# YichengDWu/NeuralGraphPDE.jl

Hardware: AMD Instinct MI355X
Metric: ODE-steps/sec (fwd+bwd) on 16k-node graph, 64-d feats (higher is better)
Workload: dtype f32; 1 GPU; C2: 16384-node / 131072-edge closest-pairs radius graph, 64-d feats, RHS = 2 x GCNConv(64=>64, relu, self-loops), Tsit5 fixed dt=1/50 x 50 steps, forward + discrete adjoint of sum(u(T)); rhs_evals_per_ode_step=6, parallelism=dp1 (independent trajectories, all-reduce of 8320-float grads)

## Files before the change

### include/ngpde.h

```cpp
#ifndef NGPDE_H
#define NGPDE_H

#include <stddef.h>
#include <stdint.h>

#ifdef __cplusplus
extern "C" {
#endif

#define NGPDE_VERSION_STRING "0.1.0"

typedef struct ngpde_graph ngpde_graph_t;
typedef struct ngpde_node ngpde_node_t;
typedef struct ngpde_node_gat ngpde_node_gat_t;
typedef struct ngpde_node_vmh ngpde_node_vmh_t;
typedef void *ngpde_stream_t;

typedef enum {
  NGPDE_OK = 0,
  NGPDE_ERR_INVALID_ARGUMENT = -1,
  NGPDE_ERR_DIMENSION_MISMATCH = -2,
  NGPDE_ERR_HIP = -3,
  NGPDE_ERR_UNSUPPORTED = -4,
  NGPDE_ERR_WORKSPACE = -5,
// ... 274 lines not shown

int32_t ngpde_gat_layer_supported(const ngpde_graph_t *g, int32_t din, int32_t heads, int32_t c);
size_t ngpde_gat_layer_workspace_bytes(const ngpde_graph_t *g, int32_t heads, int32_t c);
int32_t ngpde_gat_layer_forward(const ngpde_graph_t *g, int32_t din, int32_t heads, int32_t c, float negative_slope, int32_t act,
                                const float *x, const float *weight, const float *a, const float *bias, float *y,
                                float *save_alpha, float *save_z, ngpde_stream_t stream);
int32_t ngpde_gat_layer_backward(const ngpde_graph_t *g, int32_t din, int32_t heads, int32_t c, float negative_slope, int32_t act,
                                 const float *x, const float *weight, const float *a, const float *y_or_z, const float *save_alpha,
                                 const float *dy, float *dx, float *dweight, float *da, float *dbias, void *workspace,
                                 size_t workspace_bytes, ngpde_stream_t stream);

int32_t ngpde_bias_act_forward(int64_t n, int32_t d, int32_t act, const float *a, const float *addend, const float *bias, float *y,
                               float *save_z, ngpde_stream_t stream);
size_t ngpde_bias_act_workspace_bytes(int32_t d);
int32_t ngpde_bias_act_backward(int64_t n, int32_t d, int32_t act, const float *dy, const float *z, float *dz, float *dbias,
                                void *workspace, size_t workspace_bytes, ngpde_stream_t stream);

int32_t ngpde_edge_mlp_supported(const ngpde_graph_t *g, int32_t h1, int32_t n_tail, const int32_t *tail_dout);
int32_t ngpde_edge_mlp_forward(const ngpde_graph_t *g, int32_t h1, int32_t act1, const float *p_target,
                               const float *q_source, const float *e_term, int32_t n_tail, const int32_t *tail_dout,
                               const int32_t *tail_act, const float *const *tail_weight, const float *const *tail_bias,
                               int32_t aggr, float *out, float *const *save_z, ngpde_stream_t stream);
int32_t ngpde_edge_mlp_backward_supported(const ngpde_graph_t *g, int32_t h1, int32_t n_tail, const int32_t *tail_dout, int32_t aggr);
int32_t ngpde_edge_mlp_backward_needs_edge_buffer(const ngpde_graph_t *g, int32_t h1, int32_t act1, int32_t has_e_term, int32_t n_tail,
                                                   const int32_t *tail_dout, const int32_t *tail_act, int32_t aggr);
size_t ngpde_edge_mlp_backward_workspace_bytes(const ngpde_graph_t *g, int32_t h1, int32_t n_tail, const int32_t *tail_dout);
int32_t ngpde_edge_mlp_backward(const ngpde_graph_t *g, int32_t h1, int32_t act1, const float *p_target, const float *q_source,
                                const float *e_term, int32_t n_tail, const int32_t *tail_dout, const int32_t *tail_act,
                                const float *const *tail_weight, const float *const *tail_bias, int32_t aggr, const float *dout,
                                float *dp_target, float *dq_source, float *de_term, float *const *dtail_weight,
                                float *const *dtail_bias, void *workspace, size_t workspace_bytes, ngpde_stream_t stream);
int32_t ngpde_activation_forward(int64_t count, int32_t act, const float *z, float *a, ngpde_stream_t stream);

int32_t ngpde_spectral_weights(int64_t n_edges, int32_t n, const float *e, float *w, ngpde_stream_t stream);

int32_t ngpde_node_gcn2_create(const ngpde_graph_t *g, int32_t d, int32_t act, int32_t tableau,
                               int32_t n_steps, float dt, int32_t with_backward, ngpde_node_t **out);
int32_t ngpde_node_gcn2_create_batch(const ngpde_graph_t *member, int32_t members, int32_t d, int32_t act, int32_t tableau,
                                     int32_t n_steps, float dt, int32_t with_backward, ngpde_node_t **out);
int32_t ngpde_node_destroy(ngpde_node_t *plan);
size_t ngpde_node_tape_bytes(const ngpde_node_t *plan);
int32_t ngpde_node_gcn2_forward(ngpde_node_t *plan, const float *u0, const float *w1, const float *b1,
                                const float *w2, const float *b2, float *uT, ngpde_stream_t stream);
int32_t ngpde_node_gcn2_backward(ngpde_node_t *plan, const float *duT, float *du0, float *dw1,
                                 float *db1, float *dw2, float *db2, ngpde_stream_t stream);
int32_t ngpde_node_generation(const ngpde_node_t *plan, uint64_t *generation, int32_t *backward_pending);
int32_t ngpde_node_expect_generation(const ngpde_node_t *plan, uint64_t generation);
int32_t ngpde_node_launch_count(const ngpde_node_t *plan, int32_t *forward, int32_t *backward);
enum { NGPDE_NODE_PRESCALED = 1, NGPDE_NODE_SIGN_MASKS = 2,  NGPDE_NODE_PERSISTENT_FWD = 8,
       NGPDE_NODE_PERSISTENT_BWD = 16, NGPDE_NODE_TILE_PAIRS = 32 ,
       NGPDE_NODE_TILE_ROUNDS = 64 ,
       NGPDE_NODE_WIDENED = 128 ,
       NGPDE_NODE_HUB_GEOMETRY = 256 ,
       NGPDE_NODE_OWN_FIRST = 512  };
int32_t ngpde_node_flags(const ngpde_node_t *plan, int32_t *flags);
int32_t ngpde_batch_pad_host(int32_t n_members, const int64_t *sizes, int64_t *padded_offsets, int64_t *index, const int32_t *order,
                             int32_t *order_padded);
int32_t ngpde_hub_partition_host(int64_t n_nodes, const int32_t *rowptr_by_target, const int32_t *col_by_target,
                                 const int32_t *rowptr_by_source, const int32_t *col_by_source, int32_t *order, int32_t *tile_rows);
int32_t ngpde_node_fault(ngpde_node_t *plan, ngpde_stream_t stream, int32_t *fault);
int32_t ngpde_node_pipeline_stats(ngpde_node_t *plan, ngpde_stream_t stream, int64_t *ahead_forward, int64_t *ahead_backward,
                                  int64_t *slot_phases);
int32_t ngpde_node_gat_supported(const ngpde_graph_t *g, int32_t din, int32_t heads, int32_t c);
int32_t ngpde_node_gat_create(const ngpde_graph_t *g, int32_t heads, int32_t c, float negative_slope, int32_t act, int32_t tableau,
                              int32_t n_steps, double dt, int32_t with_backward, ngpde_node_gat_t **out);
int32_t ngpde_node_gat_create_batch(const ngpde_graph_t *g, int32_t members, int32_t heads, int32_t c, float negative_slope,
                                    int32_t act, int32_t tableau, int32_t n_steps, double dt, int32_t with_backward,
                                    ngpde_node_gat_t **out);
int32_t ngpde_node_gat_destroy(ngpde_node_gat_t *plan);
size_t ngpde_node_gat_tape_bytes(const ngpde_node_gat_t *plan);
int32_t ngpde_node_gat_fault(ngpde_node_gat_t *plan, ngpde_stream_t stream, int32_t *fault);
int32_t ngpde_node_gat_forward(ngpde_node_gat_t *plan, const float *u0, const float *weight, const float *a, const float *bias,
                               float *uT, ngpde_stream_t stream);
int32_t ngpde_node_gat_backward(ngpde_node_gat_t *plan, const float *weight, const float *a, const float *duT, float *du0,
                                float *dweight, float *da, float *dbias, ngpde_stream_t stream);
int32_t ngpde_node_vmh_supported(const ngpde_graph_t *g, int32_t hd, int32_t pd, int32_t n_phi, const int32_t *phi_dims, const int32_t *phi_acts,
                                 int32_t n_gamma, const int32_t *gamma_dims, const int32_t *gamma_acts, int32_t aggr);
int32_t ngpde_node_vmh_create(const ngpde_graph_t *g, int32_t hd, int32_t pd, const float *pos, int32_t n_phi, const int32_t *phi_dims,
                              const int32_t *phi_acts, int32_t n_gamma, const int32_t *gamma_dims, const int32_t *gamma_acts, int32_t aggr,
                              int32_t tableau, int32_t n_steps, double dt, int32_t with_backward, ngpde_node_vmh_t **out);
int32_t ngpde_node_vmh_destroy(ngpde_node_vmh_t *plan);
size_t ngpde_node_vmh_tape_bytes(const ngpde_node_vmh_t *plan);
size_t ngpde_release_cached_memory(void);
int32_t ngpde_node_vmh_fault(ngpde_node_vmh_t *plan, ngpde_stream_t stream, int32_t *fault);
int32_t ngpde_node_vmh_forward(ngpde_node_vmh_t *plan, const float *u0, const float *const *phi_weight, const float *const *phi_bias,
                               const float *const *gamma_weight, const float *const *gamma_bias, float *uT, ngpde_stream_t stream);
int32_t ngpde_node_vmh_backward(ngpde_node_vmh_t *plan, const float *const *phi_weight, const float *const *gamma_weight, const float *duT,
                                float *du0, float *const *dphi_weight, float *const *dphi_bias, float *const *dgamma_weight,
                                float *const *dgamma_bias, ngpde_stream_t stream);
int32_t ngpde_node_vmh_forward_saveat(ngpde_node_vmh_t *plan, const float *u0, const float *const *phi_weight, const float *const *phi_bias,
                                      const float *const *gamma_weight, const float *const *gamma_bias, int32_t save_every,
                                      int32_t save_start, float *usave, ngpde_stream_t stream);
int32_t ngpde_node_vmh_backward_saveat(ngpde_node_vmh_t *plan, const float *const *phi_weight, const float *const *gamma_weight,
                                       int32_t save_every, int32_t save_start, const float *dusave, float *du0, float *const *dphi_weight,
                                       float *const *dphi_bias, float *const *dgamma_weight, float *const *dgamma_bias,
                                       ngpde_stream_t stream);

int32_t ngpde_node_profile(ngpde_node_t *plan, int32_t stride, float *out_us, int32_t *out_count,
                           ngpde_stream_t stream);

int32_t ngpde_rk_stage_combine(int64_t count, float c_self, const float *base, int32_t n_terms, const float *const *terms,
                               const float *coefs, float *out, ngpde_stream_t stream);

int32_t ngpde_accumulate_many(int32_t n_arrays, float *const *acc, const float *const *g, const int64_t *counts, ngpde_stream_t stream);

size_t ngpde_rk_error_norm_workspace_bytes(int64_t count);
int32_t ngpde_rk_error_norm(int64_t count, int32_t n_terms, const float *const *terms, const float *coefs, const float *u_prev,
                            const float *u_new, double abstol, double reltol, void *workspace, double *out ,
                            ngpde_stream_t stream);

typedef enum { NGPDE_RK_REJECT = 0, NGPDE_RK_ACCEPT = 1, NGPDE_RK_DONE = 2 } ngpde_rk_action_t;
typedef struct ngpde_rk_control {
  double t0, t, t_end;
  double dt;
  double dtmax, dtmin;
// ... 144 lines not shown
```

### neuralgraphpde.jl_amd/_lib.py

```python
from __future__ import annotations

import ctypes as C
import os

_HERE = os.path.dirname(os.path.abspath(__file__))
LIB_PATH = os.path.join(_HERE, "libngpde_hip.so")


class NgpdeError(RuntimeError):

    def __init__(self, code, msg):
        super().__init__(f"[ngpde status {code}] {msg}")
        self.code = code
        self.msg = msg


class DimensionMismatch(NgpdeError, ValueError):
    """Mirrors Julia's DimensionMismatch (status NGPDE_ERR_DIMENSION_MISMATCH)."""


class ArgumentError(NgpdeError, ValueError):
    """Mirrors Julia's ArgumentError / AssertionError (status NGPDE_ERR_INVALID_ARGUMENT)."""


# ... 184 lines not shown
    "ngpde_rk_control_init": (_i32, [C.POINTER(RkControl), C.c_double, C.c_double, C.c_double, C.c_double, C.c_double, _i64]),
    "ngpde_rk_control_trial_dt": (_i32, [C.POINTER(RkControl), C.c_double, C.c_double, C.POINTER(C.c_double)]),
    "ngpde_rk_control_initial_dt": (_i32, [C.POINTER(RkControl), C.c_double, C.c_double, C.c_double]),
    "ngpde_rk_control_step": (_i32, [C.POINTER(RkControl), C.c_double, C.POINTER(_i32)]),
    "ngpde_rk_tsit5_interp_coefs": (_i32, [C.c_double, C.c_double, C.POINTER(C.c_double)]),
    "ngpde_rk_dense_output": (_i32, [_i64, _vp, _i32, _vp, _i32, _vp, _vp, _vp]),
    "ngpde_rk_dense_output_pullback": (_i32, [_i64, _i32, _vp, _i32, _vp, _vp, _vp, _vp]),
    "ngpde_gno_message_supported": (_i32, [_i32, _i32]),
    "ngpde_gno_message_backward_from_nodes": (_i32, [_vp, _i32, _i32, _i32, _i32, _vp, _vp, _vp, _vp, _vp, _vp, _vp, _vp]),
    "ngpde_gno_message_forward": (_i32, [_vp, _i32, _i32, _i32, _vp, _vp, _vp, _vp, _vp, _vp, _vp, _vp]),
    "ngpde_ode_create": (_i32, [_vp, C.POINTER(OdeDesc), C.POINTER(_vp), C.POINTER(_i32)]),
    "ngpde_ode_destroy": (_i32, [_vp]),
    "ngpde_ode_tape_bytes": (_sz, [_vp]),
    "ngpde_ode_fault": (_i32, [_vp, _vp, C.POINTER(_i32)]),
    "ngpde_ode_forward": (_i32, [_vp, _vp, C.POINTER(OdeParams), _i32, _i32, _vp, _vp]),
    "ngpde_ode_backward": (_i32, [_vp, C.POINTER(OdeParams), _i32, _i32, _vp, _vp, C.POINTER(OdeGrads), _vp]),
    "ngpde_gno_gform_supported": (_i32, [_i32, _i32]),
    "ngpde_gno_gform_preferred": (_i32, [_i64, _i64, _i32, _i32, _i32, _i32]),
    "ngpde_gno_gform_splits": (_i32, [_i64, _i32, _i32, _i32]),
    "ngpde_gno_gform_aggregate": (_i32, [_vp, _i32, _i32, _i32, _i32, _vp, _vp, _vp, _vp, _vp, _vp, _vp, _vp]),
    "ngpde_gno_gform_transform": (_i32, [_i64, _i32, _i32, _i32, _i32, _vp, _vp, _vp, _vp, _vp, _vp, _vp, _vp, _vp, _vp, _i32, _vp]),
    "ngpde_gat_layer_supported": (_i32, [_vp, _i32, _i32, _i32]),
    "ngpde_gat_layer_workspace_bytes": (_sz, [_vp, _i32, _i32]),
    "ngpde_gat_layer_forward": (_i32, [_vp, _i32, _i32, _i32, _f32, _i32, _vp, _vp, _vp, _vp, _vp, _vp, _vp, _vp]),
    "ngpde_gat_layer_backward": (_i32, [_vp, _i32, _i32, _i32, _f32, _i32, _vp, _vp, _vp, _vp, _vp, _vp, _vp, _vp, _vp, _vp, _vp, _sz, _vp]),
    "ngpde_bias_act_forward": (_i32, [_i64, _i32, _i32, _vp, _vp, _vp, _vp, _vp, _vp]),
    "ngpde_bias_act_workspace_bytes": (_sz, [_i32]),
    "ngpde_bias_act_backward": (_i32, [_i64, _i32, _i32, _vp, _vp, _vp, _vp, _vp, _sz, _vp]),
    "ngpde_edge_mlp_supported": (_i32, [_vp, _i32, _i32, _vp]),
    "ngpde_edge_mlp_forward": (_i32, [_vp, _i32, _i32, _vp, _vp, _vp, _i32, _vp, _vp, _vp, _vp, _i32, _vp, _vp, _vp]),
    "ngpde_edge_mlp_backward_supported": (_i32, [_vp, _i32, _i32, _vp, _i32]),
    "ngpde_edge_mlp_backward_needs_edge_buffer": (_i32, [_vp, _i32, _i32, _i32, _i32, _vp, _vp, _i32]),
    "ngpde_edge_mlp_backward_workspace_bytes": (_sz, [_vp, _i32, _i32, _vp]),
    "ngpde_edge_mlp_backward": (_i32, [_vp, _i32, _i32, _vp, _vp, _vp, _i32, _vp, _vp, _vp, _vp, _i32, _vp, _vp, _vp, _vp, _vp, _vp,
                                        _vp, _sz, _vp]),
    "ngpde_activation_forward": (_i32, [_i64, _i32, _vp, _vp, _vp]),
    "ngpde_spectral_weights": (_i32, [_i64, _i32, _vp, _vp, _vp]),
    "ngpde_node_gcn2_create": (_i32, [_vp, _i32, _i32, _i32, _i32, _f32, _i32, C.POINTER(_vp)]),
    "ngpde_node_gcn2_create_batch": (_i32, [_vp, _i32, _i32, _i32, _i32, _i32, _f32, _i32, C.POINTER(_vp)]),
    "ngpde_node_destroy": (_i32, [_vp]),
    "ngpde_node_tape_bytes": (_sz, [_vp]),
    "ngpde_node_gcn2_forward": (_i32, [_vp, _vp, _vp, _vp, _vp, _vp, _vp, _vp]),
    "ngpde_node_gcn2_backward": (_i32, [_vp, _vp, _vp, _vp, _vp, _vp, _vp, _vp]),
    "ngpde_node_launch_count": (_i32, [_vp, C.POINTER(_i32), C.POINTER(_i32)]),
    "ngpde_node_flags": (_i32, [_vp, C.POINTER(_i32)]),
    "ngpde_hub_partition_host": (_i32, [_i64, _vp, _vp, _vp, _vp, _vp, _vp]),
    "ngpde_batch_pad_host": (_i32, [_i32, _vp, _vp, _vp, _vp, _vp]),
    "ngpde_node_fault": (_i32, [_vp, _vp, C.POINTER(_i32)]),
    "ngpde_row_blocks_gather": (_i32, [_i32, _i32, _vp, _i32, _vp, _vp, _vp, _vp, _vp, _i32, _vp, _vp, _vp]),
    "ngpde_row_blocks_scatter": (_i32, [_i32, _i32, _vp, _i32, _vp, _vp, _vp, _vp, _vp, _i32, _vp, _vp, _vp]),
    "ngpde_transpose": (_i32, [_i32, _i32, _vp, _vp, _vp]),
    "ngpde_rows_scale": (_i32, [_i64, _i32, _vp, _vp, _vp, _vp]),
    "ngpde_node_pipeline_stats": (_i32, [_vp, _vp, C.POINTER(_i64), C.POINTER(_i64), C.POINTER(_i64)]),
    "ngpde_node_generation": (_i32, [_vp, C.POINTER(C.c_uint64), C.POINTER(_i32)]),
    "ngpde_node_expect_generation": (_i32, [_vp, C.c_uint64]),
    "ngpde_node_profile": (_i32, [_vp, _i32, C.POINTER(_f32), C.POINTER(_i32), _vp]),
    "ngpde_node_gat_supported": (_i32, [_vp, _i32, _i32, _i32]),
    "ngpde_node_gat_create": (_i32, [_vp, _i32, _i32, _f32, _i32, _i32, _i32, C.c_double, _i32, C.POINTER(_vp)]),
    "ngpde_node_gat_create_batch": (_i32, [_vp, _i32, _i32, _i32, _f32, _i32, _i32, _i32, C.c_double, _i32, C.POINTER(_vp)]),
    "ngpde_node_gat_destroy": (_i32, [_vp]),
    "ngpde_node_gat_tape_bytes": (_sz, [_vp]),
    "ngpde_node_gat_fault": (_i32, [_vp, _vp, C.POINTER(_i32)]),
    "ngpde_node_gat_forward": (_i32, [_vp, _vp, _vp, _vp, _vp, _vp, _vp]),
    "ngpde_node_gat_backward": (_i32, [_vp, _vp, _vp, _vp, _vp, _vp, _vp, _vp, _vp]),
}

_lib = None


def load():
    global _lib
    if _lib is not None:
        return _lib
    if not os.path.exists(LIB_PATH):
        raise ImportError(
            f"{LIB_PATH} is missing: build it with `python -c 'import __graft_entry__ as g; g.build()'` "
            "or `make -C neuralgraphpde.jl_amd/csrc`.  There is no CPU fallback for the hot path.")
    import torch
    lib = C.CDLL(LIB_PATH, mode=C.RTLD_GLOBAL)
    for name, (res, args) in SIGNATURES.items():
        try:
            fn = getattr(lib, name)
        except AttributeError as e:
            raise ImportError(f"{LIB_PATH} does not export {name}; rebuild the library") from e
        fn.restype = res
        fn.argtypes = args
    _lib = lib
    return lib


def check(status):
    if status == OK:
        return
    msg = load().ngpde_last_error().decode("utf-8", "replace")
    if status == ERR_DIMENSION_MISMATCH:
        raise DimensionMismatch(status, msg)
    if status == ERR_INVALID_ARGUMENT:
        raise ArgumentError(status, msg)
    raise NgpdeError(status, msg)


def ptr(t):
    if t is None:
        return None
    if hasattr(t, "data_ptr"):
        return t.data_ptr()
# ... 42 lines not shown
```

### neuralgraphpde.jl_amd/csrc/common.h

```cpp
#pragma once

#include <hip/hip_runtime.h>

#include <cstdarg>
#include <cstdint>
#include <cstdio>
#include <mutex>
#include <string>
#include <vector>

#include "../../include/ngpde.h"

namespace ngpde {

std::string &last_error();
int32_t fail(int32_t code, const char *fmt, ...);

#define NGPDE_LAUNCH_CHECK(name)                                                                    \
  do {                                                                                              \
    hipError_t _le = hipGetLastError();                                                             \
    if (_le != hipSuccess)                                                                          \
      return ::ngpde::fail(NGPDE_ERR_HIP, "%s launch failed: %s", name, hipGetErrorString(_le));    \
  } while (0)

// ... 85 lines not shown
  const float *wt = nullptr;
  const float *bias = nullptr;
  float *y = nullptr;
  float *save_agg = nullptr;
  float *save_z = nullptr;
  uint8_t *save_mask = nullptr;
  bool pre = false;
  const OwnFirst *of = nullptr;
  bool has_comb = false;
  Comb comb;
  float *comb_out = nullptr;
  hipEvent_t ev_start = nullptr, ev_stop = nullptr;
};
bool fused_supported(int din, int dout);
bool fused_prescaled_supported(const ngpde_graph *g, int d);
int32_t launch_fused_fwd(const FusedFwdArgs &a, hipStream_t stream);

struct FusedBwdArgs {
  const ngpde_graph *g = nullptr;
  int d = 0, act = 0;
  bool aggregate = false;
  const float *g_in = nullptr;
  bool has_comb = false;
  Comb comb;
  float *store_t = nullptr;
  float *store_v = nullptr;
  float v_scale = 1.f;
  bool do_dense = true;
  const float *z = nullptr;
  const uint8_t *mask = nullptr;
  bool pre = false;
  const float *saved_agg = nullptr;
  const float *wt = nullptr;
  float *g_out = nullptr;
  float *slab_dw = nullptr;
  float *slab_db = nullptr;
  hipEvent_t ev_start = nullptr, ev_stop = nullptr;
};
int fused_tile_rows();
int fused_num_blocks(int64_t n_nodes);
size_t fused_mask_bytes(int64_t n_nodes, int d);
int fused_num_slabs(int64_t n_nodes, int d);
int32_t launch_fused_bwd(const FusedBwdArgs &a, hipStream_t stream);
int32_t launch_reduce_slabs(const float *slab, int n_slabs, int len, int ct, float *out, hipStream_t stream);
int32_t launch_zero(void *ptr, size_t bytes, hipStream_t stream);
struct OwnFirst {
  uint8_t *slots = nullptr;
  int4 *sched = nullptr;
  float *slot_w = nullptr;
  uint8_t *pre = nullptr;
};
int32_t own_first_tables_build(const ngpde_graph *g, OwnFirst *of, hipStream_t stream);
void own_first_tables_free(OwnFirst *of);

struct NodePersist {
  int n_tiles = 0;
  int pair_wgs = 0;
  int *nbr = nullptr;
  unsigned *sync = nullptr;
  size_t sync_bytes = 0;
  unsigned *fault = nullptr;
  volatile unsigned *fault_host = nullptr;
  int *stats = nullptr;
  float *coef = nullptr;
  bool hub = false;
  struct HubLists {
    int32_t *halo = nullptr;
    uint8_t *slots = nullptr;
    int2 *rows = nullptr;
    int4 *info = nullptr;
    uint8_t *longs = nullptr;
    float *w = nullptr;
    int4 *sched = nullptr;
  } hub_lists[2];
};
struct NodePersistFwd {
  const ngpde_graph *g = nullptr;
  const NodePersist *ps = nullptr;
  int n_steps = 0, S = 0, act = 0, n_members = 1;
  const float *u_in = nullptr;
  float *u_out = nullptr, *bufA = nullptr, *bufB = nullptr;
  const float *w1 = nullptr, *b1 = nullptr, *w2 = nullptr, *b2 = nullptr;
  float *tape = nullptr;
  uint8_t *masks = nullptr;
  float *ztape = nullptr;
  size_t row_elems = 0, mask_bytes = 0;
  bool interleave = false;
  bool pair = false;
  int k_tiles = 0;
  float *state = nullptr;
  hipEvent_t ev_start = nullptr, ev_stop = nullptr;
  bool no_latch = false;
  const OwnFirst *of = nullptr;
};
struct NodePersistBwd {
  const ngpde_graph *g = nullptr;
  const NodePersist *ps = nullptr;
  int n_steps = 0, S = 0, n_members = 1, act = NGPDE_ACT_RELU;
  float *lam = nullptr, *g1 = nullptr, *g2 = nullptr;
  const float *w1 = nullptr, *w2 = nullptr, *tape = nullptr, *ztape = nullptr;
  const uint8_t *masks = nullptr;
  size_t row_elems = 0, mask_bytes = 0;
  float *slab_dw1 = nullptr, *slab_db1 = nullptr, *slab_dw2 = nullptr, *slab_db2 = nullptr;
  bool interleave = false;
  bool pair = false;
  int k_tiles = 0;
  float *ubar = nullptr;
  hipEvent_t ev_start = nullptr, ev_stop = nullptr;
  bool no_latch = false;
};
const unsigned *node_persistent_abort_word(const NodePersist *ps);
bool node_persistent_interleave_env();
bool node_persistent_disabled_env();
bool node_persistent_supported(const ngpde_graph *g, int d, int act, bool with_bwd);
int node_persistent_mode(const ngpde_graph *g, int d, int act, bool with_bwd);
bool node_persistent_hub_possible(const ngpde_graph *g, int d);
int node_persistent_rounds(const ngpde_graph *g);
int32_t node_persistent_setup(const ngpde_graph *g, const float *coef_host , NodePersist *ps, bool pair = false, bool hub = false);
bool node_wait_lists_fit(const ngpde_graph *g);
void node_persistent_free(NodePersist *ps);
int32_t launch_node_fwd_persistent(const NodePersistFwd &a, hipStream_t stream);
int32_t launch_node_bwd_persistent(const NodePersistBwd &a, hipStream_t stream);
struct PersistentTurn {
  int dev = -1;
  bool held = false;
  hipStream_t stream = nullptr;
  const NodePersist *ps = nullptr;
  int32_t enter(const NodePersist &p, hipStream_t s);
  int32_t latch();
  int32_t leave();
  ~PersistentTurn();
  PersistentTurn() = default;
  PersistentTurn(const PersistentTurn &) = delete;
  PersistentTurn &operator=(const PersistentTurn &) = delete;
};
struct GatNodeFwd {
  const ngpde_graph *g = nullptr;
  const NodePersist *ps = nullptr;
  int heads = 0, act = 0, n_steps = 0, S = 0;
  float slope = 0.2f;
  bool taped = false;
  const float *u_in = nullptr, *wt = nullptr, *a = nullptr, *bias = nullptr;
  float *u_out = nullptr, *xs = nullptr, *yz = nullptr, *alpha = nullptr, *kbuf = nullptr;
  const float *cf = nullptr;
  int n_members = 1;
  size_t xs_stride = 0, yz_stride = 0, alpha_stride = 0;
  hipEvent_t ev_start = nullptr, ev_stop = nullptr;
};
struct GatNodeBwd {
  const ngpde_graph *g = nullptr;
  const NodePersist *ps = nullptr;
  int heads = 0, act = 0, n_steps = 0, S = 0;
  float slope = 0.2f;
  const float *wt = nullptr, *a = nullptr, *xs = nullptr, *yz = nullptr, *alpha = nullptr, *duT = nullptr;
  float *lam = nullptr, *ubar = nullptr, *dzbuf = nullptr, *dscore = nullptr, *dal = nullptr;
  float *slab_db = nullptr, *slab_dw = nullptr, *slab_u = nullptr;
  const int *xpad = nullptr;
  const float *cb = nullptr;
  float *dwt = nullptr, *da = nullptr, *db = nullptr;
  int n_members = 1;
  size_t xs_stride = 0, yz_stride = 0, alpha_stride = 0;
  hipEvent_t ev_start = nullptr, ev_stop = nullptr;
// ... 214 lines not shown
```

### neuralgraphpde.jl_amd/csrc/node.hip

```cpp
#include <cstdlib>
#include <new>
#include <vector>

#include "common.h"

using namespace ngpde;

namespace {

struct Tableau {
  int S;
  std::vector<std::vector<double>> a;
  std::vector<double> b;
};

Tableau make_tableau(int which) {
  Tableau t;
  if (which == NGPDE_TABLEAU_EULER) {
    t.S = 1;
    t.a = {{}};
    t.b = {1.0};
    return t;
  }
  t.S = 6;
// ... 125 lines not shown
    }
  }
}

int32_t copy_block(float *dst, int dpitch, const float *src, int spitch, int w, int h, hipStream_t stream) {
  NGPDE_HIP_CHECK(hipMemcpy2DAsync(dst, (size_t)dpitch * sizeof(float), src, (size_t)spitch * sizeof(float), (size_t)w * sizeof(float),
                                   (size_t)h, hipMemcpyDeviceToDevice, stream));
  return NGPDE_OK;
}

bool act_needs_z(int act) {
  return !(act == NGPDE_ACT_IDENTITY || act == NGPDE_ACT_RELU || act == NGPDE_ACT_LEAKYRELU);
}

}

struct ngpde_node {
  const ngpde_graph *g = nullptr;
  int d = 0, act = 0, n_steps = 0;
  int du = 0;
  float dt = 0.f;
  bool with_bwd = false, needs_z = false;
  Tableau tb;
  int64_t n = 0;
  size_t row_elems = 0;
  int members = 1;
  size_t all_elems = 0;
  int nb = 0;
  int slots = 0;

  float *u = nullptr, *ustage = nullptr, *u0keep = nullptr;
  float *w1 = nullptr, *b1 = nullptr, *w2 = nullptr, *b2 = nullptr;
  float *tape = nullptr;
  size_t tape_bytes = 0;
  bool mask_mode = false;
  bool pre = false;
  float *ybuf = nullptr;
  uint8_t *masks = nullptr;
  size_t mask_bytes = 0;
  float *lam = nullptr, *g1 = nullptr, *g2 = nullptr;
  std::vector<float *> ubar;
  float *slabs = nullptr;
  size_t slab_bytes = 0;
  float *slab_dw1 = nullptr, *slab_db1 = nullptr, *slab_dw2 = nullptr, *slab_db2 = nullptr;
  float *dw1 = nullptr, *db1 = nullptr, *dw2 = nullptr, *db2 = nullptr;

  bool persistent = false;
  bool hub = false;
  bool ztape_mode = false;
  float *ztape = nullptr;
  NodePersist persist;
  OwnFirst of;
  bool has_of = false;
  float *pbuf = nullptr;
  bool interleave = false;
  bool pair = false;
  int ktiles = 0;
  float *kstate = nullptr;
  float *pubar = nullptr;

  hipStream_t cap_stream = nullptr;
  hipGraph_t fwd_graph = nullptr, bwd_graph = nullptr;
  hipGraphExec_t fwd_exec = nullptr, bwd_exec = nullptr;
  bool forward_done = false;
  uint64_t generation = 0;
  bool backward_pending = false;
  int fwd_launches = 0, bwd_launches = 0;

  float *slot(int step, int stage, int k) const {
    const int s = with_bwd ? step : 0;
    if (mask_mode) {
      if (k == 1 || k == 3) return ybuf + ((size_t)stage * 2 + (k == 3 ? 1 : 0)) * row_elems;
      return tape + ((size_t)(s * tb.S + stage) * 2 + (k == 2 ? 1 : 0)) * row_elems;
    }
    return tape + ((size_t)(s * tb.S + stage) * slots + k) * row_elems;
  }
  uint8_t *mask_slot(int step, int stage, int layer) const {
    return masks + ((size_t)(step * tb.S + stage) * 2 + (layer - 1)) * mask_bytes;
  }
};

namespace {

struct Prof {
  int stride = 1, counter = 0;
  std::vector<hipEvent_t> ev0, ev1;
  std::vector<int> role;
  bool want(int r, hipEvent_t *a, hipEvent_t *b) {
    if ((counter++ % stride) != 0) return false;
    hipEvent_t e0 = nullptr, e1 = nullptr;
    if (hipEventCreate(&e0) != hipSuccess || hipEventCreate(&e1) != hipSuccess) return false;
    ev0.push_back(e0); ev1.push_back(e1); role.push_back(r);
    *a = e0; *b = e1;
    return true;
  }
  ~Prof() {
    for (hipEvent_t e : ev0) (void)hipEventDestroy(e);
    for (hipEvent_t e : ev1) (void)hipEventDestroy(e);
  }
};

int32_t dev_alloc(float **p, size_t elems) {
  *p = nullptr;
  NGPDE_HIP_CHECK(hipMalloc((void **)p, std::max<size_t>(elems, 1) * sizeof(float)));
  return NGPDE_OK;
}
// ... 97 lines not shown
        for (int j = i + 1; j < S; ++j) {
          if (tb.a[j][i - 1] == 0.0) continue;
          e.comb.ptr[e.comb.n] = p->ubar[j];
          e.comb.coef[e.comb.n++] = (float)(p->dt * tb.a[j][i - 1]);
        }
        e.comb.coef_self = (float)(p->dt * tb.a[i][i - 1]);
        fill_dense(p, e, 2, n, i - 1);
      } else {
        e.comb.ptr[e.comb.n] = p->lam;
        e.comb.coef[e.comb.n++] = 1.0f;
        for (int j = 1; j < S; ++j) {
          e.comb.ptr[e.comb.n] = p->ubar[j];
          e.comb.coef[e.comb.n++] = 1.0f;
        }
        e.comb.coef_self = 1.0f;
        e.store_v = p->lam;
        if (n > 0) {
          e.v_scale = (float)(p->dt * tb.b[S - 1]);
          fill_dense(p, e, 2, n - 1, S - 1);
        } else {
          e.do_dense = false;
          e.pre = p->pre;
        }
      }
      if (prof && e.do_dense) prof->want(3, &e.ev_start, &e.ev_stop);
      if ((st = launch_fused_bwd(e, stream))) return st;
      count += 2;
    }
  }
  const int dd = p->d * p->d;
  const int ns = fused_num_slabs(p->n, p->d);
  if ((st = launch_reduce_slabs(p->slab_dw1, ns, dd, p->d / 16, p->dw1, stream))) return st;
  if ((st = launch_reduce_slabs(p->slab_db1, ns, p->d, 0, p->db1, stream))) return st;
  if ((st = launch_reduce_slabs(p->slab_dw2, ns, dd, p->d / 16, p->dw2, stream))) return st;
  if ((st = launch_reduce_slabs(p->slab_db2, ns, p->d, 0, p->db2, stream))) return st;
  count += 4;
  if (launches) *launches = count;
  return NGPDE_OK;
}

int32_t enqueue_forward_persistent(ngpde_node *p, hipStream_t stream, hipEvent_t ev0 = nullptr, hipEvent_t ev1 = nullptr, bool fold_latch = false) {
  NodePersistFwd a;
  a.no_latch = fold_latch;
  a.g = p->g; a.ps = &p->persist; a.n_steps = p->n_steps; a.S = p->tb.S; a.act = p->act; a.n_members = p->members;
  a.u_in = p->u; a.u_out = p->u;
  a.bufA = p->ustage; a.bufB = p->pbuf;
  a.w1 = p->w1; a.b1 = p->b1; a.w2 = p->w2; a.b2 = p->b2;
  a.row_elems = p->row_elems;
  if (p->with_bwd) {
    a.tape = p->tape; a.masks = p->masks; a.mask_bytes = p->mask_bytes; a.ztape = p->ztape;
  }
  a.interleave = p->interleave; a.pair = p->pair; a.k_tiles = p->ktiles; a.state = p->kstate;
  a.of = p->has_of ? &p->of : nullptr;
  a.ev_start = ev0; a.ev_stop = ev1;
  return launch_node_fwd_persistent(a, stream);
}

int32_t enqueue_backward_persistent(ngpde_node *p, hipStream_t stream, hipEvent_t ev0 = nullptr, hipEvent_t ev1 = nullptr,
                                    float *const *out = nullptr) {
  NodePersistBwd a;
  a.no_latch = true;
  a.g = p->g; a.ps = &p->persist; a.n_steps = p->n_steps; a.S = p->tb.S; a.n_members = p->members; a.act = p->act;
  a.lam = p->lam; a.g1 = p->g1; a.g2 = p->g2; a.w1 = p->w1; a.w2 = p->w2;
  a.tape = p->tape; a.masks = p->masks; a.row_elems = p->row_elems; a.mask_bytes = p->mask_bytes; a.ztape = p->ztape;
  a.slab_dw1 = p->slab_dw1; a.slab_db1 = p->slab_db1; a.slab_dw2 = p->slab_dw2; a.slab_db2 = p->slab_db2;
  a.interleave = p->interleave; a.pair = p->pair; a.ubar = p->pubar; a.k_tiles = p->ktiles;
  a.ev_start = ev0; a.ev_stop = ev1;
  int32_t st;
  if ((st = launch_node_bwd_persistent(a, stream))) return st;
  const int dd = p->d * p->d;
  Reduce4 r;
  r.n_slabs = (p->pair || p->ktiles) ? p->persist.pair_wgs : p->persist.n_tiles;
  r.slab[0] = p->slab_dw1; r.slab[1] = p->slab_db1; r.slab[2] = p->slab_dw2; r.slab[3] = p->slab_db2;
  r.len[0] = r.len[2] = dd; r.len[1] = r.len[3] = p->d;
  r.ct[0] = r.ct[2] = p->d / 16; r.ct[1] = r.ct[3] = 0;
  if (out) {
    for (int j = 0; j < 4; ++j) r.out[j] = out[j];
    r.du = p->du;
  } else {
    r.out[0] = p->dw1; r.out[1] = p->db1; r.out[2] = p->dw2; r.out[3] = p->db2;
    r.du = p->d;
  }
  r.abort_word = node_persistent_abort_word(&p->persist); r.fault = p->persist.fault;
  hipLaunchKernelGGL(reduce4_slabs_kernel, dim3((dd + 63) / 64, 4), dim3(1024), 0, stream, r);
  NGPDE_LAUNCH_CHECK("reduce4_slabs_kernel");
  return NGPDE_OK;
}

int32_t capture(ngpde_node *p, bool backward) {
  hipGraph_t graph = nullptr;
  NGPDE_HIP_CHECK(hipStreamBeginCapture(p->cap_stream, hipStreamCaptureModeRelaxed));
  int count = 0;
  int32_t st = backward ? enqueue_backward(p, p->cap_stream, &count) : enqueue_forward(p, p->cap_stream, &count);
  hipError_t e = hipStreamEndCapture(p->cap_stream, &graph);
  if (st) {
    if (graph) (void)hipGraphDestroy(graph);
    return st;
  }
  if (e != hipSuccess) {
    if (graph) (void)hipGraphDestroy(graph);
    return fail(NGPDE_ERR_HIP, "hipStreamEndCapture failed: %s", hipGetErrorString(e));
  }
  hipGraphExec_t exec = nullptr;
  e = hipGraphInstantiate(&exec, graph, nullptr, nullptr, 0);
  if (e != hipSuccess) {
    (void)hipGraphDestroy(graph);
    return fail(NGPDE_ERR_HIP, "hipGraphInstantiate failed: %s", hipGetErrorString(e));
  }
  if (backward) {
    p->bwd_graph = graph; p->bwd_exec = exec; p->bwd_launches = count;
  } else {
    p->fwd_graph = graph; p->fwd_exec = exec; p->fwd_launches = count;
  }
  return NGPDE_OK;
}

}

extern "C" {

int32_t ngpde_node_destroy(ngpde_node_t *p) {
  NGPDE_RANGE();
  if (!p) return NGPDE_OK;
  if (p->fwd_exec) (void)hipGraphExecDestroy(p->fwd_exec);
  if (p->bwd_exec) (void)hipGraphExecDestroy(p->bwd_exec);
  if (p->fwd_graph) (void)hipGraphDestroy(p->fwd_graph);
  if (p->bwd_graph) (void)hipGraphDestroy(p->bwd_graph);
  if (p->cap_stream) (void)hipStreamDestroy(p->cap_stream);
  float *bufs[] = {p->u0keep, p->u, p->ustage, p->w1, p->b1, p->w2, p->b2, p->tape, p->lam, p->g1, p->g2, p->slabs,
                   p->dw1, p->db1, p->dw2, p->db2};
  for (float *b : bufs)
    if (b) (void)hipFree(b);
  for (float *b : p->ubar)
    if (b) (void)hipFree(b);
  if (p->ybuf) (void)hipFree(p->ybuf);
  if (p->masks) (void)hipFree(p->masks);
  if (p->pbuf) (void)hipFree(p->pbuf);
  if (p->pubar) (void)hipFree(p->pubar);
  if (p->kstate) (void)hipFree(p->kstate);
  node_persistent_free(&p->persist);
  own_first_tables_free(&p->of);
  delete p;
  return NGPDE_OK;
}

int32_t ngpde_node_gcn2_create(const ngpde_graph_t *g, int32_t d, int32_t act, int32_t tableau, int32_t n_steps,
                               float dt, int32_t with_backward, ngpde_node_t **out) {
  NGPDE_RANGE();
  return ngpde_node_gcn2_create_batch(g, 1, d, act, tableau, n_steps, dt, with_backward, out);
}

static int32_t node_create(const ngpde_graph_t *g, int32_t members, int32_t d, int32_t du, int32_t act, int32_t tableau,
                           int32_t n_steps, float dt, int32_t with_backward, ngpde_node_t **out) {
  NGPDE_REQUIRE(out != nullptr, NGPDE_ERR_INVALID_ARGUMENT, "ngpde_node_gcn2_create: out is NULL");
  NGPDE_REQUIRE(members >= 1, NGPDE_ERR_INVALID_ARGUMENT, "ngpde_node_gcn2_create_batch: members must be >= 1");
  *out = nullptr;
  NGPDE_REQUIRE(g != nullptr, NGPDE_ERR_INVALID_ARGUMENT, "ngpde_node_gcn2_create: graph is NULL");
  NGPDE_REQUIRE(g->has_norm, NGPDE_ERR_STATE, "ngpde_node_gcn2_create: GCN normalisation not set");
  NGPDE_REQUIRE(fused_supported(d, d), NGPDE_ERR_UNSUPPORTED,
                "ngpde_node_gcn2_create: d must be one of 16, 32, 64, 128 (got %d)", d);
  NGPDE_REQUIRE(act >= NGPDE_ACT_IDENTITY && act <= NGPDE_ACT_SOFTPLUS, NGPDE_ERR_INVALID_ARGUMENT,
                "ngpde_node_gcn2_create: unknown activation code %d", act);
  NGPDE_REQUIRE(tableau == NGPDE_TABLEAU_EULER || tableau == NGPDE_TABLEAU_TSIT5, NGPDE_ERR_INVALID_ARGUMENT,
                "ngpde_node_gcn2_create: unknown tableau %d", tableau);
  NGPDE_REQUIRE(n_steps >= 1, NGPDE_ERR_INVALID_ARGUMENT, "ngpde_node_gcn2_create: n_steps must be >= 1");
  NGPDE_REQUIRE(g->n_nodes >= 1, NGPDE_ERR_INVALID_ARGUMENT, "ngpde_node_gcn2_create: empty graph");
  ngpde_node *p = new (std::nothrow) ngpde_node();
  NGPDE_REQUIRE(p != nullptr, NGPDE_ERR_INVALID_ARGUMENT, "out of host memory");
  p->g = g; p->d = d; p->du = du; p->act = act; p->n_steps = n_steps; p->dt = dt;
  p->with_bwd = with_backward != 0;
  p->needs_z = p->with_bwd && act_needs_z(act);
  p->tb = make_tableau(tableau);
  p->n = g->n_nodes;
  p->members = members;
  p->row_elems = (size_t)p->n * d;
  p->all_elems = (size_t)members * p->row_elems;
  p->nb = fused_num_blocks(p->n);
  p->mask_mode = p->with_bwd && act == NGPDE_ACT_RELU && std::getenv("NGPDE_NO_MASK") == nullptr;
  p->pre = fused_prescaled_supported(g, d) && std::getenv("NGPDE_NO_PRESCALE") == nullptr;
  int pmode = p->pre ? node_persistent_mode(g, d, act, p->with_bwd) : 0;
  bool hub = !p->pre && pmode == 0 && std::getenv("NGPDE_NO_PRESCALE") == nullptr && node_persistent_hub_possible(g, d) &&
             (!p->with_bwd || p->mask_mode || act != NGPDE_ACT_RELU);
  if (hub) {
    pmode = 4;
    p->pre = true;
  }
  p->pair = pmode == 2 && members == 1 && (!p->with_bwd || p->mask_mode);
  p->ktiles = (pmode == 3 && members == 1) ? node_persistent_rounds(g) : 0;
  bool want_persist = (pmode == 1 && (!p->with_bwd || p->mask_mode || (act != NGPDE_ACT_RELU && members == 1))) || p->pair || p->ktiles > 0 || hub;
  const int S = p->tb.S;
  int32_t st = NGPDE_OK;
  if (want_persist) {
    p->persistent = true;
    float coef[90] = {0};
    const Tableau &tb = p->tb;
    for (int i = 0; i < S; ++i) {
      const std::vector<double> &row = (i == S - 1) ? tb.b : tb.a[i + 1];
      for (int j = 0; j < i; ++j) coef[i * 6 + j] = (float)(dt * row[j]);
      coef[36 + i] = (float)(dt * row[i]);
      coef[42 + i] = (float)(dt * tb.b[i]);
    }
    for (int i = 1; i < S; ++i) {
      for (int j = i + 1; j < S; ++j) coef[48 + i * 6 + j] = (float)(dt * tb.a[j][i - 1]);
      coef[84 + i] = (float)(dt * tb.a[i][i - 1]);
    }
    st = node_persistent_setup(g, coef, &p->persist, p->pair, hub);
    if (st == NGPDE_ERR_UNSUPPORTED) {
      st = NGPDE_OK;
      p->persistent = false;
    }
    if (p->persistent && p->ktiles > 0) p->persist.pair_wgs = (p->persist.n_tiles + p->ktiles - 1) / p->ktiles;
  }
  if (!p->persistent) {
    p->pair = false;
    p->ktiles = 0;
  }
  if (hub && !p->persistent) {
    p->pre = false;
    hub = false;
    node_persistent_free(&p->persist);
  }
  p->hub = hub;
  int dev_ = 0, cus_ = 0;
  const bool one_wave = hipGetDevice(&dev_) == hipSuccess && hipDeviceGetAttribute(&cus_, hipDeviceAttributeMultiprocessorCount, dev_) == hipSuccess &&
                        p->nb <= 2 * cus_;
  if (st == NGPDE_OK && p->pre && !hub && one_wave) {
    const char *nof = std::getenv("NGPDE_NO_OWN_FIRST");
    if (!(nof && nof[0] == '1')) {
      st = own_first_tables_build(g, &p->of, nullptr);
      p->has_of = st == NGPDE_OK;
    }
  }
  p->ztape_mode = p->with_bwd && !p->mask_mode && p->persistent;
  p->slots = p->mask_mode ? 2 : (p->ztape_mode ? 4 : (p->with_bwd ? (p->needs_z ? 6 : 4) : 4));
  p->mask_bytes = p->mask_mode ? fused_mask_bytes(p->n, d) : 0;
  p->interleave = members > 1 && !hub && node_persistent_interleave_env();
  const size_t xslots = p->interleave ? 2 : 1;
  auto A = [&](float **ptr, size_t elems) {
    if (st == NGPDE_OK) st = dev_alloc(ptr, elems);
  };
  A(&p->u, p->all_elems);
  A(&p->ustage, xslots * p->row_elems);
  A(&p->u0keep, (size_t)members * p->n * du);
  A(&p->w1, (size_t)d * d); A(&p->b1, d); A(&p->w2, (size_t)d * d); A(&p->b2, d);
  if (st == NGPDE_OK && du != d) {
    for (float *w : {p->w1, p->w2})
      if (hipMemset(w, 0, (size_t)d * d * sizeof(float)) != hipSuccess) st = fail(NGPDE_ERR_HIP, "hipMemset failed");
    for (float *b : {p->b1, p->b2})
      if (hipMemset(b, 0, (size_t)d * sizeof(float)) != hipSuccess) st = fail(NGPDE_ERR_HIP, "hipMemset failed");
  }
  const size_t tape_elems = (size_t)(p->with_bwd ? n_steps : 1) * S * p->slots * p->all_elems;
  p->tape_bytes = tape_elems * sizeof(float);
  A(&p->tape, tape_elems);
  if (p->mask_mode) {
    A(&p->ybuf, (size_t)S * 2 * p->row_elems);
    if (st == NGPDE_OK) {
      const size_t mb = (size_t)members * n_steps * S * 2 * p->mask_bytes;
      if (hipMalloc((void **)&p->masks, std::max<size_t>(mb, 1)) != hipSuccess) st = fail(NGPDE_ERR_HIP, "hipMalloc of the sign-bit masks failed");
      else p->tape_bytes += mb + (size_t)S * 2 * p->row_elems * sizeof(float);
    }
  }
  if (p->with_bwd) {
    A(&p->lam, p->all_elems); A(&p->g1, xslots * p->row_elems); A(&p->g2, xslots * p->row_elems);
    if (p->interleave || p->pair || p->ktiles) A(&p->pubar, 2 * 5 * p->row_elems);
    p->ubar.assign(S, nullptr);
    for (int j = 1; j < S; ++j) A(&p->ubar[j], p->row_elems);
    const size_t dd = (size_t)d * d;
    const size_t per = (size_t)p->nb * (dd + d);
    p->slab_bytes = 2 * per * sizeof(float);
    A(&p->slabs, 2 * per);
    if (st == NGPDE_OK) {
      p->slab_dw1 = p->slabs;
      p->slab_db1 = p->slab_dw1 + (size_t)p->nb * dd;
      p->slab_dw2 = p->slab_db1 + (size_t)p->nb * d;
      p->slab_db2 = p->slab_dw2 + (size_t)p->nb * dd;
    }
    A(&p->dw1, dd); A(&p->db1, d); A(&p->dw2, dd); A(&p->db2, d);
  }
  if (st == NGPDE_OK && p->persistent) A(&p->pbuf, xslots * p->row_elems);
  if (st == NGPDE_OK && p->ktiles) A(&p->kstate, 7 * p->row_elems);
  if (st == NGPDE_OK && p->ztape_mode) p->ztape = p->tape + (size_t)n_steps * S * 2 * p->all_elems;
  if (st == NGPDE_OK && members > 1 && !p->persistent)
    st = fail(NGPDE_ERR_UNSUPPORTED, "ngpde_node_gcn2_create_batch: the member-by-member solve exists for the persistent plan only "
                                     "(d = 64, relu, unweighted, at most two 32-row tiles per CU); batch the graphs into one handle instead");
  if (st == NGPDE_OK && !p->persistent) {
    hipError_t e = hipStreamCreateWithFlags(&p->cap_stream, hipStreamNonBlocking);
    if (e != hipSuccess) st = fail(NGPDE_ERR_HIP, "hipStreamCreate failed: %s", hipGetErrorString(e));
    if (st == NGPDE_OK) st = capture(p, false);
    if (st == NGPDE_OK && p->with_bwd) st = capture(p, true);
  }
  if (p->persistent) {
    p->fwd_launches = 2;
    p->bwd_launches = p->with_bwd ? 3 : 0;
  }
  if (st != NGPDE_OK) {
    std::string keep = last_error();
    ngpde_node_destroy(p);
    last_error() = keep;
    return st;
  }
  *out = p;
  return NGPDE_OK;
}

int32_t ngpde_node_gcn2_create_batch(const ngpde_graph_t *g, int32_t members, int32_t d, int32_t act, int32_t tableau,
                                     int32_t n_steps, float dt, int32_t with_backward, ngpde_node_t **out) {
  NGPDE_RANGE();
  const char *nw = std::getenv("NGPDE_NO_WIDEN");
  if (out && g && (d == 16 || d == 32) && !(nw && nw[0] == '1') && g->has_norm && g->n_nodes >= 1 &&
      (node_persistent_mode(g, 64, act, with_backward != 0) != 0 || node_persistent_hub_possible(g, 64))) {
    ngpde_node_t *w = nullptr;
    if (node_create(g, members, 64, d, act, tableau, n_steps, dt, with_backward, &w) == NGPDE_OK) {
      if (w->persistent) {
        *out = w;
        return NGPDE_OK;
      }
      ngpde_node_destroy(w);
    }
  }
  return node_create(g, members, d, d, act, tableau, n_steps, dt, with_backward, out);
}

size_t ngpde_node_tape_bytes(const ngpde_node_t *p) { return p ? p->tape_bytes : 0; }

int32_t ngpde_node_launch_count(const ngpde_node_t *p, int32_t *forward, int32_t *backward) {
  NGPDE_RANGE();
  NGPDE_REQUIRE(p != nullptr, NGPDE_ERR_INVALID_ARGUMENT, "ngpde_node_launch_count: plan is NULL");
  if (forward) *forward = p->fwd_launches;
  if (backward) *backward = p->bwd_launches;
  return NGPDE_OK;
}

int32_t ngpde_node_flags(const ngpde_node_t *p, int32_t *flags) {
  NGPDE_RANGE();
  NGPDE_REQUIRE(p != nullptr && flags != nullptr, NGPDE_ERR_INVALID_ARGUMENT, "ngpde_node_flags: NULL argument");
  *flags = (p->pre ? NGPDE_NODE_PRESCALED : 0) | (p->mask_mode ? NGPDE_NODE_SIGN_MASKS : 0) |
           (p->persistent ? NGPDE_NODE_PERSISTENT_FWD : 0) | (p->persistent && p->with_bwd ? NGPDE_NODE_PERSISTENT_BWD : 0) |
           (p->pair ? NGPDE_NODE_TILE_PAIRS : 0) | (p->ktiles ? NGPDE_NODE_TILE_ROUNDS : 0) | (p->du != p->d ? NGPDE_NODE_WIDENED : 0) |
           (p->hub ? NGPDE_NODE_HUB_GEOMETRY : 0) | (p->has_of ? NGPDE_NODE_OWN_FIRST : 0);
  return NGPDE_OK;
}

int32_t ngpde_node_fault(ngpde_node_t *p, ngpde_stream_t stream_, int32_t *fault) {
  NGPDE_RANGE();
  NGPDE_REQUIRE(p != nullptr && fault != nullptr, NGPDE_ERR_INVALID_ARGUMENT, "ngpde_node_fault: NULL argument");
  *fault = 0;
  if (!p->persist.fault_host) return NGPDE_OK;
  NGPDE_HIP_CHECK(hipStreamSynchronize((hipStream_t)stream_));
  *fault = *p->persist.fault_host ? 1 : 0;
  return NGPDE_OK;
}

int32_t ngpde_node_pipeline_stats(ngpde_node_t *p, ngpde_stream_t stream_, int64_t *ahead_forward, int64_t *ahead_backward,
                                  int64_t *slot_phases) {
  NGPDE_RANGE();
  NGPDE_REQUIRE(p != nullptr, NGPDE_ERR_INVALID_ARGUMENT, "ngpde_node_pipeline_stats: plan is NULL");
  if (ahead_forward) *ahead_forward = 0;
  if (ahead_backward) *ahead_backward = 0;
  if (slot_phases) *slot_phases = 0;
  if (!p->persist.stats) return NGPDE_OK;
  const int nt = p->persist.n_tiles;
  std::vector<int> h((size_t)nt * 2);
  NGPDE_HIP_CHECK(hipMemcpyAsync(h.data(), p->persist.stats, h.size() * sizeof(int), hipMemcpyDeviceToHost, (hipStream_t)stream_));
  NGPDE_HIP_CHECK(hipStreamSynchronize((hipStream_t)stream_));
  int64_t f = 0, b = 0;
  for (int t = 0; t < nt; ++t) f += h[2 * t], b += h[2 * t + 1];
  if (ahead_forward) *ahead_forward = f;
  if (ahead_backward) *ahead_backward = b;
  if (slot_phases) *slot_phases = (int64_t)nt * p->members * p->n_steps * p->tb.S * 2;
  return NGPDE_OK;
}

int32_t ngpde_node_gcn2_forward(ngpde_node_t *p, const float *u0, const float *w1, const float *b1, const float *w2,
                                const float *b2, float *uT, ngpde_stream_t stream_) {
  NGPDE_RANGE();
  NGPDE_REQUIRE(p != nullptr, NGPDE_ERR_INVALID_ARGUMENT, "ngpde_node_gcn2_forward: plan is NULL");
  NGPDE_REQUIRE(u0 && w1 && w2 && uT, NGPDE_ERR_INVALID_ARGUMENT, "ngpde_node_gcn2_forward: NULL argument");
  NGPDE_REQUIRE(!(p->persist.fault_host && *p->persist.fault_host), NGPDE_ERR_STATE,
                "ngpde_node_gcn2_forward: an earlier persistent launch of this plan gave up waiting for its neighbours (its outputs are NaN): "
                "another kernel held the device's compute units, or two persistent solves of different processes shared the device; "
                "create a new plan (NGPDE_NO_PERSISTENT=1 selects the replayed plan)");
  hipStream_t stream = (hipStream_t)stream_;
  const size_t user_bytes = (size_t)p->members * p->n * p->du * sizeof(float);
  if (p->pre) {
    RowsExtra x;
    x.keep = reinterpret_cast<float4 *>(p->u0keep);
    int32_t st = launch_scale_rows_width(u0, p->du, p->g->c, p->u, p->d, p->n, false, stream, p->members, x);
    if (st) return st;
  } else {
    NGPDE_HIP_CHECK(hipMemcpyAsync(p->u, u0, p->all_elems * sizeof(float), hipMemcpyDeviceToDevice, stream));
    NGPDE_HIP_CHECK(hipMemcpyAsync(p->u0keep, u0, user_bytes, hipMemcpyDeviceToDevice, stream));
  }
  {
    int32_t st = launch_pack_params(w1, b1, w2, b2, p->du, p->d, p->w1, p->b1, p->w2, p->b2, stream);
    if (st) return st;
  }
  const bool fold_latch = p->persistent && p->pre;
  if (p->persistent) {
    int32_t st = enqueue_forward_persistent(p, stream, nullptr, nullptr, fold_latch);
    if (st) return st;
  } else {
    NGPDE_HIP_CHECK(hipGraphLaunch(p->fwd_exec, stream));
  }
  if (p->pre) {
    RowsExtra x;
    if (fold_latch) { x.abort_word = node_persistent_abort_word(&p->persist); x.fault = p->persist.fault; }
    int32_t st = launch_scale_rows_width(p->u, p->d, p->g->c, uT, p->du, p->n, true, stream, p->members, x);
    if (st) return st;
  } else {
    NGPDE_HIP_CHECK(hipMemcpyAsync(uT, p->u, p->all_elems * sizeof(float), hipMemcpyDeviceToDevice, stream));
  }
  p->forward_done = true;
  ++p->generation;
  p->backward_pending = p->with_bwd;
  return NGPDE_OK;
}

int32_t ngpde_node_generation(const ngpde_node_t *p, uint64_t *generation, int32_t *backward_pending) {
  NGPDE_RANGE();
  NGPDE_REQUIRE(p != nullptr, NGPDE_ERR_INVALID_ARGUMENT, "ngpde_node_generation: plan is NULL");
  if (generation) *generation = p->generation;
  if (backward_pending) *backward_pending = p->backward_pending ? 1 : 0;
// ... 611 lines not shown
```

### neuralgraphpde.jl_amd/csrc/node_persistent.hip

```cpp

#include <algorithm>
#include <cstdlib>
#include <cstring>
#include <mutex>
#include <type_traits>

#include "common.h"
#include "persistent_gcn_tile.h"
#include "stamps.h"

namespace ngpde {

namespace {


template <int ACT, bool TAPE, bool WGT = false, bool HUB = false>
__global__ __launch_bounds__(kThreads, HUB ? 2 : 4) void node_fwd_persistent_kernel(const PFwdK p) {
  static_assert(!(HUB && WGT), "hub geometry: its own weight lists (HubCtx::hw), not the WGT form");
  constexpr int XH = HUB ? kHubXhF : kXhF, MF = HUB ? kHubMetaF : kMetaF;
  __shared__ __attribute__((aligned(16))) float lds[XH + 2 * kTileF + (WGT ? kWF + kSlotWF : 2 * kWF) + 2 * PD + MF + 48 + 4];
  static_assert(!HUB || sizeof(lds) <= 160 * 1024 - 64, "one workgroup per CU");
  float *ldsXh = lds, *ldsT = lds + XH, *ldsZ = ldsT + kTileF, *ldsW1 = ldsZ + kTileF, *ldsW2 = WGT ? ldsW1 : ldsW1 + kWF;
  float *ldsSW = ldsW2 + kWF, *ldsB = WGT ? ldsSW + kSlotWF : ldsSW;
  float *ldsMeta = ldsB + 2 * PD, *ldsC = ldsMeta + MF;
  int *s_ok = reinterpret_cast<int *>(ldsC + 48);
  typename std::conditional<HUB, HubCtx, TileCtx>::type c;
  if constexpr (HUB) hub_ctx_init(p.m, c, ldsMeta);
  else tile_ctx_init(p.m, c, ldsMeta);
  coef_to_lds(ldsC, p.cf, 42, c.tid);
  const int act = ACT >= 0 ? ACT : p.act;
  float4 *Xh4 = reinterpret_cast<float4 *>(ldsXh);
  float bw1[16];
  if constexpr (WGT) {
    reinterpret_cast<float2 *>(ldsSW)[c.tid] = reinterpret_cast<const float2 *>(p.m.slot_w + (size_t)c.tile * kSlotWF)[c.tid];
    c.lds_w = ldsSW;
    const int i16 = c.lane & 15, kq = c.lane >> 4, ct = c.wave_u / PG::RT;
#pragma unroll
    for (int kb = 0; kb < 4; ++kb)
#pragma unroll
      for (int r = 0; r < 4; ++r) bw1[4 * kb + r] = p.w1[(16 * kb + 4 * kq + r) * PD + 16 * ct + i16];
  } else {
    load_weight_lds(p.w1, ldsW1, c.tid, true);
  }
  load_weight_lds(p.w2, ldsW2, c.tid, true);
  biases_to_lds(ldsB, p.b1, p.b2, c.tid);
  if (!HUB) zero_halo_row(ldsXh, c.grp == 0, c.q);
  if (c.tid == 0) *s_ok = 1;
  const unsigned own = own_row_offset(c);
  __syncthreads();
  int of_pre = 0;
  if constexpr (!HUB && !WGT) {
    if (p.m.of_pre) of_pre = __builtin_amdgcn_readfirstlane((int)p.m.of_pre[(size_t)c.tile * 8 + c.wave_u]);
  }
  const float4 bias1 = reinterpret_cast<const float4 *>(ldsB)[c.q], bias2 = reinterpret_cast<const float4 *>(ldsB + PD)[c.q];
  bool ok = true;
  int ph = 0;
  for (int mb = 0; mb < p.n_members; ++mb) {
  const float *u_in = p.u_in + (size_t)mb * p.row_elems;
  const size_t ev0 = (size_t)mb * p.n_steps * p.S * 2;
  float4 u = f4_sel(c.valid && ok, ld4_g(u_in, own), f4_zero());
  float4 k0 = f4_zero(), k1 = f4_zero(), k2 = f4_zero(), k3 = f4_zero(), k4 = f4_zero(), k5 = f4_zero();
  Xh4[c.grp * PG::LPR + c.q] = u;
  if constexpr (!HUB && !WGT) __syncthreads();
  for (int n = 0; n < p.n_steps && ok; ++n) {
    for (int i = 0; i < p.S && ok; ++i) {
#pragma unroll
      for (int layer = 0; layer < 2; ++layer) {
        ++ph;
        const float *X = layer == 0 ? ((n == 0 && i == 0) ? u_in : p.bufA) : p.bufB;
        NGPDE_PHASE_STAMP(p.m.stamps, ph, 0);
        float4 agg;
        if constexpr (HUB) {
          unsigned sw[8];
          hub_slot_words(c, sw);
          if (!hub_wait(p.m, c, ph, s_ok)) { ok = false; break; }
          NGPDE_PHASE_STAMP(p.m.stamps, ph, 1);
          hub_gather_foreign(c, X, ldsXh);
          NGPDE_PHASE_STAMP(p.m.stamps, ph, 2);
          agg = hub_aggregate(c, sw, ldsXh, ldsZ);
        } else if constexpr (!WGT) {
          unsigned sw[8], swf[8];
          tile_slot_words(c, sw);
          tile_slot_words_from(c, of_pre, swf);
          unsigned goff[2];
          tile_gather_offsets(c, goff);
          const float4 self = Xh4[c.grp * PG::LPR + c.q];
          float4 a = tile_aggregate_rounds(c, sw, ldsXh, f4_zero(), of_pre);
          tile_wait_arrive(p.m, c, ph, s_ok, p.m.flags);
          NGPDE_PHASE_STAMP(p.m.stamps, ph, 1);
          if (!tile_gather_foreign_checked(c, X, ldsXh, goff, s_ok)) { ok = false; break; }
          NGPDE_PHASE_STAMP(p.m.stamps, ph, 2);
          a = tile_aggregate_rounds(c, swf, ldsXh, a, ((c.wmax + 3) >> 2) - of_pre);
          agg = f4_add(a, self);
        } else {
          unsigned sw[8];
          tile_slot_words(c, sw);
          if (!tile_wait(p.m, c, ph, s_ok)) { ok = false; break; }
          NGPDE_PHASE_STAMP(p.m.stamps, ph, 1);
          tile_gather_foreign(c, X, ldsXh);
          NGPDE_PHASE_STAMP(p.m.stamps, ph, 2);
          agg = tile_aggregate_weighted(c, ldsXh);
        }
        float4 acc = f4_scale(c.ci, agg);
        tile_row_store(ldsT, c, acc);
        const size_t ev = ev0 + (size_t)(n * p.S + i) * 2 + layer;
        __syncthreads();
        NGPDE_PHASE_STAMP(p.m.stamps, ph, 3);
        if (WGT && layer == 0) mfma_rows_times_bfrag64(ldsT, bw1, ldsZ, c.wave_u, c.lane);
        else mfma_rows_times_bt<PD>(ldsT, layer == 0 ? ldsW1 : ldsW2, ldsZ, c.wave_u, c.lane);
        __syncthreads();
        NGPDE_PHASE_STAMP(p.m.stamps, ph, 4);
        const float4 z = fwd_preact(ldsZ, c, layer == 0 ? bias1 : bias2);
        const uint8_t sign_bits = relu_sign_bits(z);
        float4 yv = fwd_output(c, act, z);
        if (layer == 0) {
          if (c.valid) store_sc1(p.bufB, own, yv);
          Xh4[c.grp * PG::LPR + c.q] = yv;
        } else {
          k0 = f4_sel(i == 0, yv, k0); k1 = f4_sel(i == 1, yv, k1); k2 = f4_sel(i == 2, yv, k2);
          k3 = f4_sel(i == 3, yv, k3); k4 = f4_sel(i == 4, yv, k4); k5 = f4_sel(i == 5, yv, k5);
          const float4 v = rk_combine<false>(RkCoefInPlace{ldsC, i}, i, yv, u, k0, k1, k2, k3, k4);
          if (i == p.S - 1) u = v;
          if (c.valid) store_sc1(p.bufA, own, v);
          Xh4[c.grp * PG::LPR + c.q] = v;
        }
        NGPDE_PHASE_STAMP(p.m.stamps, ph, 5);
        tile_publish(p.m, c, ph);
        NGPDE_PHASE_STAMP(p.m.stamps, ph, 6);
        if constexpr (TAPE && ACT == NGPDE_ACT_RELU) stu8_g(p.masks + ev * p.mask_bytes + (size_t)c.tile * kThreads, (unsigned)c.tid, sign_bits);
        else if (TAPE && c.valid) st4_stream_g(p.ztape + ev * p.row_elems, own, z);
        if (TAPE && c.valid) st4_stream_g(p.tape + ev * p.row_elems, own, tile_row(ldsT, c));
      }
    }
  }
  if (c.valid) st4_g(p.u_out + (size_t)mb * p.row_elems, own, f4_sel(ok, u, f4_nan()));
  }
}


template <int ACT, bool TAPE>
__global__ __launch_bounds__(kThreads, 4) void node_fwd_persistentK_kernel(const PFwdK p) {
  constexpr int kMS = meta_stride<true>(), kMT = meta_tiles<true>();
  __shared__ __attribute__((aligned(16))) float lds[kXhF + 2 * kTileF + kWF + 2 * PD + kMT * kMS + 48 + 4];
  static_assert(sizeof(lds) <= 80 * 1024 - 64, "two workgroups per CU");
  float *ldsXh = lds, *ldsT = lds + kXhF, *ldsZ = ldsT + kTileF, *ldsW = ldsZ + kTileF, *ldsB = ldsW + kWF;
  float *ldsMeta = ldsB + 2 * PD, *ldsC = ldsMeta + kMT * kMS;
  int *s_ok = reinterpret_cast<int *>(ldsC + 48);
  const int tid = threadIdx.x, q = tid & 15;
  coef_to_lds(ldsC, p.cf, 42, tid);
  const int act = ACT >= 0 ? ACT : p.act;
  biases_to_lds(ldsB, p.b1, p.b2, tid);
  zero_halo_row(ldsXh, tid < PG::LPR, tid & 15);
  if (tid == 0) *s_ok = 1;
  const int W = p.pair_wgs, K = min(p.k_tiles, kMT);
  const int t0 = xcd_tile(blockIdx.x, W);
  const unsigned rowb = (unsigned)(p.row_elems * sizeof(float));
  tile_round_tables<true>(p.m, t0, W, K, ldsMeta);
  const int KT = tile_round_count(p.m, t0, W, K);
  __syncthreads();
  const float4 bias1 = reinterpret_cast<const float4 *>(ldsB)[q], bias2 = reinterpret_cast<const float4 *>(ldsB + PD)[q];
  bool ok = true;
  int ph = 0;
  for (int n = 0; n < p.n_steps && ok; ++n) {
    for (int i = 0; i < p.S && ok; ++i) {
#pragma unroll 1
      for (int layer = 0; layer < 2 && ok; ++layer) {
        ++ph;
        const float *X = layer == 0 ? ((n == 0 && i == 0) ? p.u_in : p.bufA) : p.bufB;
        const size_t ev = (size_t)(n * p.S + i) * 2 + layer;
        const bool last_phase = (n == p.n_steps - 1 && i == p.S - 1 && layer == 1);
        load_weight_lds(layer == 0 ? p.w1 : p.w2, ldsW, tid, true);
        for (int s = 0; s < K; ++s) {
          const int tile = t0 + s * W;
          if (tile >= p.m.n_tiles) break;
          TileCtx c;
          tile_ctx_from_lds<true>(c, tile, ldsMeta + s * kMS);
          const unsigned own = own_row_offset(c);
          if (!tile_wait(p.m, c, ph, s_ok)) { ok = false; break; }
          halo_fill_all(c, X, ldsXh);
          float4 su = f4_zero(), sk0 = f4_zero(), sk1 = f4_zero(), sk2 = f4_zero(), sk3 = f4_zero(), sk4 = f4_zero();
          if (layer == 1) {
            su = (n == 0) ? f4_sel(c.valid, ld4_g(p.u_in, own), f4_zero()) : ld4_g(p.state, own);
            sk0 = i > 0 ? ld4_g(p.state, own + rowb) : f4_zero(); sk1 = i > 1 ? ld4_g(p.state, own + 2 * rowb) : f4_zero();
            sk2 = i > 2 ? ld4_g(p.state, own + 3 * rowb) : f4_zero(); sk3 = i > 3 ? ld4_g(p.state, own + 4 * rowb) : f4_zero();
// ... 285 lines not shown
  int pend_ph = 0;
  const int NP = p.n_steps * p.S * 2;
  for (int mb = 0; mb < p.n_members && ok; mb += 2) {
    const bool two = PAIR ? has1 : mb + 1 < p.n_members;
    const float *u_in0 = p.u_in + (size_t)mb * p.row_elems, *u_in1 = u_in0 + ((two && !PAIR) ? p.row_elems : 0);
    const size_t ev00 = (size_t)mb * NP, ev01 = PAIR ? ev00 : ev00 + NP;
    const size_t boff1 = PAIR ? 0 : p.row_elems;
    unsigned *flags1 = p.m.flags + (PAIR ? 0 : p.flag_stride);
    FSlot s0, s1;
    s0.u = f4_sel(c.valid, ld4_g(u_in0, own), f4_zero());
    s1.u = f4_sel(c1.valid && two, ld4_g(u_in1, own1), f4_zero());
    s0.k0 = s0.k1 = s0.k2 = s0.k3 = s0.k4 = s0.k5 = f4_zero();
    s1.k0 = s1.k1 = s1.k2 = s1.k3 = s1.k4 = s1.k5 = f4_zero();
    s0.xown = s0.u;
    s1.xown = s1.u;
    int n = 0, i = 0;
    for (int P = 0; P < NP && ok; P += 2) {
#pragma unroll
      for (int layer = 0; layer < 2; ++layer) {
        ++ph;
        const float *ldsW = layer == 0 ? ldsW1 : ldsW2, *ldsBias = layer == 0 ? ldsB : ldsB + PD;
        const float *X0 = layer == 0 ? (P == 0 ? u_in0 : p.bufA) : p.bufB;
        const float *X1 = layer == 0 ? (P == 0 ? u_in1 : p.bufA + boff1) : p.bufB + boff1;
        FNext nx0, nx1;
        nx0.exists = two; nx0.ph = ph; nx0.X = X1; nx0.flags = flags1;
        nx1.exists = P + layer + 1 < NP; nx1.ph = ph + 1; nx1.X = layer == 0 ? p.bufB : p.bufA; nx1.flags = p.m.flags;
        if (!fwd_slot_phase<ACT, TAPE, PAIR>(p, c, c1, s0, s1, 0, ph, n, i, layer, X0, ev00, act, own, pre, n_ahead, pend_flags, pend_ph, nx0, ldsXh,
                                             ldsT, ldsZ, ldsW, ldsBias, ldsC, s_ok, s_pre)) { ok = false; break; }
        if (two && !fwd_slot_phase<ACT, TAPE, PAIR>(p, c1, c, s1, s0, 1, ph, n, i, layer, X1, ev01, act, own1, pre, n_ahead, pend_flags, pend_ph, nx1,
                                                    ldsXh, ldsT, ldsZ, ldsW, ldsBias, ldsC, s_ok, s_pre)) { ok = false; break; }
      }
      if (++i == p.S) i = 0, ++n;
    }
    wait_vmcnt0();
    __syncthreads();
    if (ok && pend_flags && c.tid == 0) __hip_atomic_store(pend_flags, (unsigned)pend_ph, __ATOMIC_RELAXED, __HIP_MEMORY_SCOPE_AGENT);
    pend_flags = nullptr;
    if (c.valid) st4_g(p.u_out + (size_t)mb * p.row_elems, own, f4_sel(ok, s0.u, f4_nan()));
    if (two && c1.valid) st4_g(p.u_out + (PAIR ? 0 : (size_t)(mb + 1) * p.row_elems), own1, f4_sel(ok, s1.u, f4_nan()));
    if (PAIR) break;
  }
  if (!ok) {
    poison_members(p.u_out, p.n_members, p.row_elems, c.valid, own);
    poison_members(p.u_out, p.n_members, p.row_elems, PAIR && has1 && c1.valid, own1);
  }
  if (c.tid == 0 && p.m.stats) p.m.stats[2 * c.tile] = n_ahead;
}


template <int ACT, bool WGT = false, bool HUB = false>
__global__ __launch_bounds__(kThreads, HUB ? 2 : 4) void node_bwd_persistent_kernel(const PBwdK p) {
  static_assert(!(HUB && WGT), "hub geometry: its own weight lists (HubCtx::hw), not the WGT form");
  constexpr bool RELU = (ACT == NGPDE_ACT_RELU);
  using Aux = typename std::conditional<RELU, unsigned, float4>::type;
  constexpr int XH = HUB ? kHubXhF : kXhF, MF = HUB ? kHubMetaF : kMetaF;
  __shared__ __attribute__((aligned(16))) float lds[XH + 2 * kTileF + (WGT ? PD * PD + kWF + kSlotWF : 2 * kWF) + MF + 48 + 4];
  static_assert(sizeof(lds) <= (HUB ? 160 : 80) * 1024 - 64, "two workgroups per CU (hub geometry: one)");
  float *ldsXh = lds, *ldsG = lds, *ldsDZ = lds + XH, *ldsX = ldsDZ + kTileF, *ldsW1 = ldsX + kTileF, *ldsW2 = ldsW1 + (WGT ? PD * PD : kWF);
  float *ldsSW = ldsW2 + kWF;
  float *ldsMeta = WGT ? ldsSW + kSlotWF : ldsSW, *ldsC = ldsMeta + MF;
  int *s_ok = reinterpret_cast<int *>(ldsC + 48);
  typename std::conditional<HUB, HubCtx, TileCtx>::type c;
  if constexpr (HUB) hub_ctx_init(p.m, c, ldsMeta);
  else tile_ctx_init(p.m, c, ldsMeta);
  coef_to_lds(ldsC, p.cb, 48, c.tid);
  float4 *Xh4 = reinterpret_cast<float4 *>(ldsXh);
  if constexpr (WGT) {
    reinterpret_cast<float2 *>(ldsSW)[c.tid] = reinterpret_cast<const float2 *>(p.m.slot_w + (size_t)c.tile * kSlotWF)[c.tid];
    c.lds_w = ldsSW;
#pragma unroll
    for (int k = 0; k < PG::W4; ++k) {
      const int idx = c.tid + k * kThreads;
      if (idx < PD * PD / 4) {
        const int wi = (idx * 4) / PD, w4 = ((idx * 4) % PD) / 4;
        *reinterpret_cast<float4 *>(&ldsW1[wi * PD + 4 * (w4 ^ (wi & 15))]) = reinterpret_cast<const float4 *>(p.w1)[idx];
      }
    }
  } else {
    load_weight_lds(p.w1, ldsW1, c.tid, false);
  }
  load_weight_lds(p.w2, ldsW2, c.tid, false);
  if (!HUB) zero_halo_row(ldsXh, c.grp == 0, c.q);
  if (c.tid == 0) *s_ok = 1;
  const unsigned own = own_row_offset(c);
  f32x4 dw1[PG::DWT], dw2[PG::DWT];
#pragma unroll
  for (int mm = 0; mm < PG::DWT; ++mm) dw1[mm] = dw2[mm] = (f32x4){0.f, 0.f, 0.f, 0.f};
  float db1 = 0.f, db2 = 0.f;
  const int dbc = c.tid / PG::DBP, dbpart = c.tid % PG::DBP;
  const int S = p.S;
  __syncthreads();

  auto tape_row = [&](size_t ev) { return ld4_stream_g(p.tape + ev * p.row_elems, own); };
  auto mask_of = [&](size_t ev) -> Aux {
    if constexpr (RELU) return ldu8_g(p.masks + ev * p.mask_bytes + (size_t)c.tile * kThreads, (unsigned)c.tid);
    else return ld4_stream_g(p.ztape + ev * p.row_elems, own);
  };
  Aux mk_n{};
  float4 xrow_n = f4_zero();
  unsigned f_next = 0;
  auto dense = [&](int ph, const float *ldsW, f32x4 (&dwl)[PG::DWT], float &dbl, float4 kbar, Aux mk, float4 xrow, float *gout, bool pf, size_t ev_n) {
    const float4 dz = adjoint_dz<RELU>(c, p.act, kbar, mk);
    tile_row_store(ldsDZ, c, dz);
    __syncthreads();
    NGPDE_PHASE_STAMP(p.m.stamps, ph, 3);
    if (WGT && ldsW == ldsW1) mfma_rows_times_bswz64(ldsDZ, ldsW, ldsG, c.wave_u, c.lane);
    else mfma_rows_times_bt<PD>(ldsDZ, ldsW, ldsG, c.wave_u, c.lane);
    __syncthreads();
    NGPDE_PHASE_STAMP(p.m.stamps, ph, 4);
    const float4 gv = adjoint_g_row(ldsG, c);
    if (c.valid) store_sc1(gout, own, gv);
    adjoint_x_store(ldsX, c, xrow);
    NGPDE_PHASE_STAMP(p.m.stamps, ph, 5);
    tile_publish(p.m, c, ph);
    NGPDE_PHASE_STAMP(p.m.stamps, ph, 6);
    Xh4[c.grp * PG::LPR + c.q] = gv;
    if constexpr (!HUB) {
      if (c.wave_u == 0) f_next = poll_issue(p.m, c, p.m.flags);
    }
    if (pf) {
      mk_n = mask_of(ev_n);
      xrow_n = tape_row(ev_n);
    }
    param_grad_products(ldsX, ldsDZ, c.wave_u, c.lane, dbc, dbpart, dwl, dbl);
    NGPDE_PHASE_STAMP(p.m.stamps, ph, 7);
  };

  bool ok = true;
  int ph = 0;
  for (int mb = 0; mb < p.n_members; ++mb) {
  float *lam_g = p.lam + (size_t)mb * p.row_elems;
  const size_t ev0 = (size_t)mb * p.n_steps * S * 2;
  float4 lam = f4_sel(c.valid && ok, ld4_g(lam_g, own), f4_zero());
  float4 ub1 = f4_zero(), ub2 = f4_zero(), ub3 = f4_zero(), ub4 = f4_zero(), ub5 = f4_zero();
  if (ok) {
    ++ph;
    const size_t ev = ev0 + (size_t)((p.n_steps - 1) * S + (S - 1)) * 2 + 1;
    dense(ph, ldsW2, dw2, db2, adjoint_kbar_last(ldsC, S, lam), mask_of(ev), tape_row(ev), p.g2, true,
          ev0 + (size_t)((p.n_steps - 1) * S + (S - 1)) * 2);
  }
  for (int n = p.n_steps - 1; n >= 0 && ok; --n) {
    for (int i = S - 1; i >= 0 && ok; --i) {
      {
        ++ph;
        NGPDE_PHASE_STAMP(p.m.stamps, ph, 0);
        const Aux mk = mk_n;
        const float4 xrow = xrow_n;
        const bool last_next = (i == 0 && n == 0);
        const size_t ev_next = ev0 + ((i >= 1) ? (size_t)(n * S + i - 1) * 2 + 1 : (size_t)((max(n, 1) - 1) * S + (S - 1)) * 2 + 1);
        float4 t;
        if constexpr (HUB) {
          unsigned sw[8];
          hub_slot_words(c, sw);
          if (!hub_wait(p.m, c, ph, s_ok)) { ok = false; break; }
          NGPDE_PHASE_STAMP(p.m.stamps, ph, 1);
          hub_gather_foreign(c, p.g2, ldsXh);
          NGPDE_PHASE_STAMP(p.m.stamps, ph, 2);
          t = hub_aggregate(c, sw, ldsXh, ldsDZ);
        } else if constexpr (WGT) {
          if (!tile_wait_primed(p.m, c, ph, s_ok, p.m.flags, f_next)) { ok = false; break; }
          NGPDE_PHASE_STAMP(p.m.stamps, ph, 1);
          tile_gather_foreign(c, p.g2, ldsXh);
          NGPDE_PHASE_STAMP(p.m.stamps, ph, 2);
          t = tile_aggregate_weighted(c, ldsXh);
        } else {
          unsigned sw[8], goff[2];
          tile_slot_words(c, sw);
          if constexpr (RELU) tile_gather_offsets(c, goff);
          if constexpr (RELU) {
            tile_wait_primed_arrive(p.m, c, ph, s_ok, p.m.flags, f_next);
            NGPDE_PHASE_STAMP(p.m.stamps, ph, 1);
            if (!tile_gather_foreign_checked(c, p.g2, ldsXh, goff, s_ok)) { ok = false; break; }
          } else {
            if (!tile_wait_primed(p.m, c, ph, s_ok, p.m.flags, f_next)) { ok = false; break; }
            NGPDE_PHASE_STAMP(p.m.stamps, ph, 1);
            tile_gather_foreign(c, p.g2, ldsXh);
          }
          NGPDE_PHASE_STAMP(p.m.stamps, ph, 2);
          float4 self;
          if constexpr (RELU) self = Xh4[c.grp * PG::LPR + c.q];
          t = tile_aggregate_rounds_rolling(c, sw, ldsXh, f4_zero(), (c.wmax + 3) >> 2);
          if constexpr (!RELU) self = Xh4[c.grp * PG::LPR + c.q];
          t = f4_add(t, self);
        }
        dense(ph, ldsW1, dw1, db1, t, mk, xrow, p.g1, !last_next, ev_next);
      }
      {
        ++ph;
        const bool last = (i == 0 && n == 0);
        NGPDE_PHASE_STAMP(p.m.stamps, ph, 0);
        const Aux mk = mk_n;
        const float4 xrow = xrow_n;
        const size_t ev_next = ev0 + (size_t)(i >= 1 ? n * S + i - 1 : (max(n, 1) - 1) * S + (S - 1)) * 2;
        float4 t;
        if constexpr (HUB) {
          unsigned sw[8];
          hub_slot_words(c, sw);
          if (!hub_wait(p.m, c, ph, s_ok)) { ok = false; break; }
          NGPDE_PHASE_STAMP(p.m.stamps, ph, 1);
          hub_gather_foreign(c, p.g1, ldsXh);
          NGPDE_PHASE_STAMP(p.m.stamps, ph, 2);
          t = hub_aggregate(c, sw, ldsXh, ldsDZ);
        } else if constexpr (WGT) {
          if (!tile_wait_primed(p.m, c, ph, s_ok, p.m.flags, f_next)) { ok = false; break; }
          NGPDE_PHASE_STAMP(p.m.stamps, ph, 1);
          tile_gather_foreign(c, p.g1, ldsXh);
          NGPDE_PHASE_STAMP(p.m.stamps, ph, 2);
          t = tile_aggregate_weighted(c, ldsXh);
        } else {
          unsigned sw[8], goff[2];
          tile_slot_words(c, sw);
          if constexpr (RELU) tile_gather_offsets(c, goff);
          if constexpr (RELU) {
            tile_wait_primed_arrive(p.m, c, ph, s_ok, p.m.flags, f_next);
            NGPDE_PHASE_STAMP(p.m.stamps, ph, 1);
            if (!tile_gather_foreign_checked(c, p.g1, ldsXh, goff, s_ok)) { ok = false; break; }
          } else {
            if (!tile_wait_primed(p.m, c, ph, s_ok, p.m.flags, f_next)) { ok = false; break; }
            NGPDE_PHASE_STAMP(p.m.stamps, ph, 1);
            tile_gather_foreign(c, p.g1, ldsXh);
          }
          NGPDE_PHASE_STAMP(p.m.stamps, ph, 2);
          float4 self;
          if constexpr (RELU) self = Xh4[c.grp * PG::LPR + c.q];
          t = tile_aggregate_rounds_rolling(c, sw, ldsXh, f4_zero(), (c.wmax + 3) >> 2);
          if constexpr (!RELU) self = Xh4[c.grp * PG::LPR + c.q];
          t = f4_add(t, self);
        }
        float4 kbar;
        if (i >= 1) {
          ub1 = f4_sel(i == 1, t, ub1); ub2 = f4_sel(i == 2, t, ub2); ub3 = f4_sel(i == 3, t, ub3);
          ub4 = f4_sel(i == 4, t, ub4); ub5 = f4_sel(i == 5, t, ub5);
          kbar = adjoint_kbar_stage(ldsC, i, t, lam, ub2, ub3, ub4, ub5);
        } else {
          const float4 v = adjoint_lambda_update(t, lam, ub1, ub2, ub3, ub4, ub5);
          lam = v;
          kbar = adjoint_kbar_last(ldsC, S, v);
        }
        if (last) break;
        dense(ph, ldsW2, dw2, db2, kbar, mk, xrow, p.g2, true, ev_next);
      }
    }
  }
  if (c.valid) st4_g(lam_g, own, f4_sel(ok, lam, f4_nan()));
  }
  write_slab(dw1, db1, p.slab_dw1, p.slab_db1, c.wave_u, c.lane, dbc, dbpart, ok);
  write_slab(dw2, db2, p.slab_dw2, p.slab_db2, c.wave_u, c.lane, dbc, dbpart, ok);
}


struct BNext {
  bool gather;
  int ph;
  const float *X;
  const unsigned *flags;
  bool tape;
  size_t ev;
};

template <bool PAIR>
__global__ __launch_bounds__(kThreads, 4) void node_bwd_persistent2_kernel(const PBwdK p) {
  __shared__ __attribute__((aligned(16))) float lds[kXhF + 2 * kTileF + 2 * kWF + (PAIR ? 2 : 1) * kMetaF + 48 + 4];
  float *ldsXh = lds, *ldsG = lds, *ldsDZ = lds + kXhF, *ldsX = ldsDZ + kTileF, *ldsW1 = ldsX + kTileF, *ldsW2 = ldsW1 + kWF;
  float *ldsMeta = ldsW2 + kWF, *ldsC = ldsMeta + (PAIR ? 2 : 1) * kMetaF;
  int *s_ok = reinterpret_cast<int *>(ldsC + 48), *s_pre = s_ok + 1;
  TileCtx c, c1s;
  tile_ctx_init(p.m, c, ldsMeta, PAIR ? xcd_tile(blockIdx.x, p.pair_wgs) : -1);
  const bool has1 = !PAIR || c.tile + p.pair_wgs < p.m.n_tiles;
  if (PAIR) tile_ctx_init(p.m, c1s, ldsMeta + kMetaF, has1 ? c.tile + p.pair_wgs : c.tile);
  const TileCtx &c1 = PAIR ? c1s : c;
  coef_to_lds(ldsC, p.cb, 48, c.tid);
  load_weight_lds(p.w1, ldsW1, c.tid, false);
  load_weight_lds(p.w2, ldsW2, c.tid, false);
  zero_halo_row(ldsXh, c.grp == 0, c.q);
  if (c.tid == 0) *s_ok = 1, *s_pre = 0;
  const unsigned own = own_row_offset(c);
  const unsigned own1 = row_offset(c1.node, c.q);
  f32x4 dw1[PG::DWT], dw2[PG::DWT];
#pragma unroll
// ... 869 lines not shown
  pre = max(pre, __shfl_xor(pre, 1));
  pre = max(pre, __shfl_xor(pre, 2));
  int fits = (4 * pre + nf <= kSlotWidth) ? 1 : 0;
  fits = min(fits, __shfl_xor(fits, 1));
  fits = min(fits, __shfl_xor(fits, 2));
  if (!fits) pre = 0;
  if (row) {
    uint8_t *ob = o_slots + pos * kSlotWidth;
    float *ow = o_w ? o_w + pos * kSlotWidth : nullptr;
    const float *iw = slot_w ? slot_w + pos * kSlotWidth : nullptr;
    if (fits) {
      int k = 0;
      for (int j = 0; j < deg; ++j)
        if (b[j] < kTileRows) { ob[k] = b[j]; if (ow) ow[k] = iw[j]; ++k; }
      for (; k < 4 * pre; ++k) { ob[k] = (uint8_t)kHaloCap; if (ow) ow[k] = 0.f; }
      for (int j = 0; j < deg; ++j)
        if (b[j] >= kTileRows) { ob[k] = b[j]; if (ow) ow[k] = iw[j]; ++k; }
      const int len = k;
      for (; k < kSlotWidth; ++k) { ob[k] = (uint8_t)kHaloCap; if (ow) ow[k] = 0.f; }
      if (sc.x >= 0) sc.z = len;
    } else {
      for (int j = 0; j < kSlotWidth; ++j) { ob[j] = b[j]; if (ow) ow[j] = iw[j]; }
    }
    o_sched[pos] = sc;
    if ((r & 3) == 0) o_pre[(size_t)tile * 8 + (r >> 2)] = (uint8_t)pre;
  }
}
}

int32_t own_first_tables_build(const ngpde_graph *g, OwnFirst *of, hipStream_t stream) {
  const int nt = g->n_sched / kTileRows;
  const Csr &c = g->by_t;
  if (c.halo_ok && c.slots && c.sched) {
    NGPDE_HIP_CHECK(hipMalloc((void **)&of->slots, (size_t)g->n_sched * kSlotWidth));
    NGPDE_HIP_CHECK(hipMalloc((void **)&of->sched, (size_t)g->n_sched * sizeof(int4)));
    NGPDE_HIP_CHECK(hipMalloc((void **)&of->pre, (size_t)nt * 8));
    if (c.slot_w) NGPDE_HIP_CHECK(hipMalloc((void **)&of->slot_w, (size_t)g->n_sched * kSlotWidth * sizeof(float)));
    hipLaunchKernelGGL(own_first_tables_kernel, dim3(nt), dim3(64), 0, stream, nt, c.slots, c.sched, c.slot_w, of->slots, of->sched,
                       of->slot_w, of->pre);
    NGPDE_LAUNCH_CHECK("own_first_tables_kernel");
  }
  NGPDE_HIP_CHECK(hipStreamSynchronize(stream));
  return NGPDE_OK;
}

void own_first_tables_free(OwnFirst *of) {
  if (of->slots) (void)hipFree(of->slots);
  if (of->sched) (void)hipFree(of->sched);
  if (of->slot_w) (void)hipFree(of->slot_w);
  if (of->pre) (void)hipFree(of->pre);
  *of = OwnFirst();
}

int32_t node_persistent_setup(const ngpde_graph *g, const float *coef_host, NodePersist *ps, bool pair, bool hub) {
  std::vector<int> lists;
  const int nt = g->n_sched / kTileRows;
  ps->hub = false;
  if (hub) {
    NGPDE_REQUIRE(!pair && nt <= kHubNbr, NGPDE_ERR_UNSUPPORTED, "persistent solver, hub geometry: at most %d tiles, one per workgroup", kHubNbr);
    std::vector<int32_t> rp[2], cl[2];
    NGPDE_REQUIRE(host_csr(g, g->by_t, rp[0], cl[0]) && host_csr(g, g->by_s, rp[1], cl[1]), NGPDE_ERR_HIP, "download of the CSR lists failed");
    std::vector<int32_t> order = hub_partition(g->n_nodes, rp, cl, true);
    if ((int64_t)order.size() != g->n_nodes) order = hub_partition(g->n_nodes, rp, cl, false);
    NGPDE_REQUIRE((int64_t)order.size() == g->n_nodes, NGPDE_ERR_UNSUPPORTED,
                  "persistent solver, hub geometry: no partition into 32-row tiles of at most %d referenced rows each (a node of more than %d distinct in+out neighbours, or tiles that do not close)",
                  kHubHalo, kHubHalo - kTileRows);
    std::vector<float> wcsr[2];
    if (g->w_coo && g->n_edges > 0) {
      std::vector<float> wc((size_t)g->n_edges);
      NGPDE_HIP_CHECK(hipMemcpy(wc.data(), g->w_coo, wc.size() * sizeof(float), hipMemcpyDeviceToHost));
      const Csr *cs[2] = {&g->by_t, &g->by_s};
      for (int dir = 0; dir < 2; ++dir) {
        std::vector<int32_t> eid = cs[dir]->h_eid;
        if (eid.empty()) {
          eid.resize((size_t)g->n_edges);
          NGPDE_HIP_CHECK(hipMemcpy(eid.data(), cs[dir]->eid, eid.size() * sizeof(int32_t), hipMemcpyDeviceToHost));
        }
        wcsr[dir].resize((size_t)g->n_edges);
        for (int64_t e = 0; e < g->n_edges; ++e) wcsr[dir][(size_t)e] = wc[(size_t)eid[(size_t)e]];
      }
    }
    HubHost hh[2];
    NGPDE_REQUIRE(build_hub_lists(g->n_nodes, nt, rp[0], cl[0], order, hh[0], wcsr[0].empty() ? nullptr : wcsr[0].data()) &&
                      build_hub_lists(g->n_nodes, nt, rp[1], cl[1], order, hh[1], wcsr[1].empty() ? nullptr : wcsr[1].data()),
                  NGPDE_ERR_UNSUPPORTED,
                  "persistent solver, hub geometry: a tile references more than %d distinct rows or holds more than %d entries", kHubHalo, kHubList);
    std::vector<float> cnode((size_t)g->n_nodes);
    NGPDE_HIP_CHECK(hipMemcpy(cnode.data(), g->c, cnode.size() * sizeof(float), hipMemcpyDeviceToHost));
    std::vector<int4> hsched((size_t)nt * kTileRows, make_int4(-1, 0, 0, 0));
    for (int64_t pos = 0; pos < g->n_nodes; ++pos) {
      int4 e = make_int4(order[pos], 0, 0, 0);
      std::memcpy(&e.w, &cnode[order[pos]], 4);
      hsched[(size_t)pos] = e;
    }
    std::vector<int32_t> tile_of((size_t)g->n_nodes, 0);
    for (int64_t pos = 0; pos < g->n_nodes; ++pos) tile_of[order[pos]] = (int32_t)(pos / kTileRows);
    std::vector<std::vector<int>> nb(nt);
    for (const HubHost &h : hh)
      for (int t = 0; t < nt; ++t)
        for (int k = kTileRows; k < h.info[t].x; ++k) {
          const int u = tile_of[h.halo[(size_t)t * kHubHalo + k]];
          if (u == t) continue;
          nb[t].push_back(u);
          nb[u].push_back(t);
        }
    lists.assign((size_t)nt * kHubNbr, -1);
// ... 38 lines not shown
  NGPDE_HIP_CHECK(hipMemset(ps->sync, 0, ps->sync_bytes));
  NGPDE_HIP_CHECK(hipMalloc((void **)&ps->coef, 90 * sizeof(float)));
  NGPDE_HIP_CHECK(hipMemcpy(ps->coef, coef_host, 90 * sizeof(float), hipMemcpyHostToDevice));
  NGPDE_HIP_CHECK(hipHostMalloc((void **)&ps->fault_host, 128, hipHostMallocMapped));
  *ps->fault_host = 0u;
  NGPDE_HIP_CHECK(hipHostGetDevicePointer((void **)&ps->fault, const_cast<unsigned *>(ps->fault_host), 0));
  NGPDE_HIP_CHECK(hipMalloc((void **)&ps->stats, (size_t)nt * 2 * sizeof(int)));
  NGPDE_HIP_CHECK(hipMemset(ps->stats, 0, (size_t)nt * 2 * sizeof(int)));
  return NGPDE_OK;
}

void node_persistent_free(NodePersist *ps) {
  if (ps->nbr) (void)hipFree(ps->nbr);
  if (ps->sync) (void)hipFree(ps->sync);
  if (ps->fault_host) (void)hipHostFree(const_cast<unsigned *>(ps->fault_host));
  ps->fault_host = nullptr;
  if (ps->coef) (void)hipFree(ps->coef);
  if (ps->stats) (void)hipFree(ps->stats);
  ps->stats = nullptr;
  for (NodePersist::HubLists &L : ps->hub_lists) {
    if (L.halo) (void)hipFree(L.halo);
    if (L.slots) (void)hipFree(L.slots);
    if (L.rows) (void)hipFree(L.rows);
    if (L.info) (void)hipFree(L.info);
    if (L.longs) (void)hipFree(L.longs);
    if (L.sched) (void)hipFree(L.sched);
    if (L.w) (void)hipFree(L.w);
    L = NodePersist::HubLists();
  }
  ps->hub = false;
  ps->nbr = nullptr; ps->sync = nullptr; ps->fault = nullptr; ps->coef = nullptr;
}

namespace {
__global__ void set_word_kernel(unsigned *w, unsigned v) {
  if (threadIdx.x == 0) *w = v;
}
__global__ void latch_fault_kernel(const unsigned *abort_word, unsigned *fault) {
  if (threadIdx.x == 0 && *abort_word != 0) *fault = 1u;
}
}
const unsigned *node_persistent_abort_word(const NodePersist *ps) { return ps->sync ? sync_abort_word(ps->sync, ps->n_tiles) : nullptr; }
namespace {
TileMeta make_meta(const Csr &c, const NodePersist &ps, int dir, const OwnFirst *of = nullptr) {
  TileMeta m;
  m.halo = c.halo; m.slots = c.slots; m.sched = c.sched; m.tile_info = c.tile_info; m.nbr = ps.nbr; m.slot_w = c.slot_w;
  m.of_pre = nullptr;
  if (of && of->slots && !ps.hub) {
    m.slots = of->slots; m.sched = of->sched; m.of_pre = of->pre;
    if (m.slot_w) m.slot_w = of->slot_w;
  }
  const NodePersist::HubLists &L = ps.hub_lists[dir];
  m.hub_halo = L.halo; m.hub_slots = L.slots; m.hub_rows = L.rows; m.hub_info = L.info; m.hub_long = L.longs; m.hub_sched = L.sched;
  m.hub_w = L.w;
  if (ps.hub) m.slot_w = nullptr;
  m.flags = ps.sync; m.abort_word = sync_abort_word(ps.sync, ps.n_tiles); m.n_tiles = ps.n_tiles;
  m.stats = ps.stats;
  NGPDE_STAMP_SET(m, kStampPersistent, 0);
  return m;
}
}

namespace {
struct Turnstile {
  std::mutex mu;
  hipEvent_t last[16] = {};
  bool used[16] = {};
};
Turnstile &turnstile() {
  static Turnstile t;
  return t;
}
}

int32_t PersistentTurn::enter(const NodePersist &p, hipStream_t s) {
  ps = &p;
  stream = s;
  NGPDE_HIP_CHECK(hipGetDevice(&dev));
  if (dev >= 0 && dev < 16) {
    Turnstile &t = turnstile();
    t.mu.lock();
    held = true;
    hipStreamCaptureStatus cs = hipStreamCaptureStatusNone;
    if (hipStreamIsCapturing(stream, &cs) != hipSuccess) cs = hipStreamCaptureStatusNone;
    if (cs == hipStreamCaptureStatusNone && t.used[dev]) NGPDE_HIP_CHECK(hipStreamWaitEvent(stream, t.last[dev], 0));
  }
  int32_t st;
  if ((st = launch_zero(p.sync, p.sync_bytes, stream))) return st;
  const char *fa = std::getenv("NGPDE_DEBUG_FORCE_ABORT");
  if (fa && fa[0] == '1') hipLaunchKernelGGL(set_word_kernel, dim3(1), dim3(64), 0, stream, sync_abort_word(p.sync, p.n_tiles), 1u);
  return NGPDE_OK;
}
int32_t PersistentTurn::latch() {
  hipLaunchKernelGGL(latch_fault_kernel, dim3(1), dim3(64), 0, stream, sync_abort_word(ps->sync, ps->n_tiles), ps->fault);
  NGPDE_LAUNCH_CHECK("latch_fault_kernel");
  return NGPDE_OK;
}
int32_t PersistentTurn::leave() {
  if (!held) return NGPDE_OK;
  Turnstile &t = turnstile();
  int32_t st = NGPDE_OK;
  hipStreamCaptureStatus cs = hipStreamCaptureStatusNone;
  if (hipStreamIsCapturing(stream, &cs) != hipSuccess) cs = hipStreamCaptureStatusNone;
  if (cs == hipStreamCaptureStatusNone) {
    if (!t.last[dev] && hipEventCreateWithFlags(&t.last[dev], hipEventDisableTiming) != hipSuccess) st = fail(NGPDE_ERR_HIP, "hipEventCreate failed");
    if (st == NGPDE_OK && hipEventRecord(t.last[dev], stream) != hipSuccess) st = fail(NGPDE_ERR_HIP, "hipEventRecord failed");
// ... 17 lines not shown
  PersistentTurn turn;
  if ((st = turn.enter(ps, stream))) return st;
  PFwdK k;
  k.m = make_meta(g->by_t, ps, 0, a.of);
  k.n_steps = a.n_steps; k.S = a.S; k.act = a.act; k.n_members = a.n_members;
  k.u_in = a.u_in; k.u_out = a.u_out; k.bufA = a.bufA; k.bufB = a.bufB;
  k.w1 = a.w1; k.b1 = a.b1; k.w2 = a.w2; k.b2 = a.b2;
  k.tape = a.tape; k.masks = a.masks; k.row_elems = a.row_elems; k.mask_bytes = a.mask_bytes;
  k.flag_stride = sync_slot_stride(ps.n_tiles);
  k.pair_wgs = a.pair ? ps.pair_wgs : 0;
  k.cf = ps.coef;
  NGPDE_REQUIRE(!a.pair || (ps.pair_wgs > 0 && !a.interleave && a.n_members == 1), NGPDE_ERR_STATE, "tile-pair launch without its setup");
  k.k_tiles = a.k_tiles; k.state = a.state;
  const auto launch = [&](auto kernel, dim3 grid) { launch_timed(kernel, grid, dim3(kThreads), 0, stream, a.ev_start, a.ev_stop, k); };
  if (a.k_tiles > 0) {
    NGPDE_REQUIRE(ps.pair_wgs > 0 && a.n_members == 1 && a.state, NGPDE_ERR_STATE, "tile-round launch without its setup");
    NGPDE_REQUIRE(a.k_tiles <= kMaxTileRounds, NGPDE_ERR_STATE, "tile rounds: at most %d tiles per workgroup", kMaxTileRounds);
    k.pair_wgs = ps.pair_wgs; k.ztape = a.ztape;
    if ((st = launch_zero(a.state + a.row_elems, 6 * a.row_elems * sizeof(float), stream))) return st;
    const dim3 gridk(ps.pair_wgs);
    NGPDE_REQUIRE(!k.m.slot_w || a.k_tiles <= kMaxTileRoundsW, NGPDE_ERR_STATE, "weighted tile rounds: at most %d tiles per workgroup", kMaxTileRoundsW);
#define NGPDE_PFK_LAUNCH(AA, TT) \
    launch(k.m.slot_w ? node_fwd_persistentK_kernel<AA, TT> : node_fwd_persistentKP_kernel<AA, TT>, gridk);
    if (a.tape && a.act == NGPDE_ACT_RELU) { NGPDE_PFK_LAUNCH(NGPDE_ACT_RELU, true) }
    else if (a.tape) { NGPDE_PFK_LAUNCH(-1, true) }
    else if (a.act == NGPDE_ACT_RELU) { NGPDE_PFK_LAUNCH(NGPDE_ACT_RELU, false) }
    else { NGPDE_PFK_LAUNCH(-1, false) }
#undef NGPDE_PFK_LAUNCH
    NGPDE_LAUNCH_CHECK("node_fwd_persistentK_kernel");
    if (!a.no_latch && (st = turn.latch())) return st;
    return turn.leave();
  }
  NGPDE_REQUIRE(!k.m.slot_w || (!a.pair && !a.interleave && a.n_members == 1), NGPDE_ERR_STATE,
                "weighted graphs: one tile per workgroup or tile rounds, one member");
  const dim3 grid(a.pair ? ps.pair_wgs : ps.n_tiles);
  if (ps.hub) {
    NGPDE_REQUIRE(!a.pair && !a.interleave, NGPDE_ERR_STATE, "hub geometry: one tile per workgroup, the members of a batch one after the other");
    k.ztape = a.ztape;
    NGPDE_REQUIRE(!a.tape || (a.act == NGPDE_ACT_RELU ? a.masks != nullptr : a.ztape != nullptr), NGPDE_ERR_INVALID_ARGUMENT,
                  "persistent forward with a tape needs the sign-bit masks (relu) or the pre-activation tape");
    if (a.tape && a.act == NGPDE_ACT_RELU) launch(node_fwd_persistent_kernel<NGPDE_ACT_RELU, true, false, true>, grid);
    else if (a.tape) launch(node_fwd_persistent_kernel<-1, true, false, true>, grid);
    else if (a.act == NGPDE_ACT_RELU) launch(node_fwd_persistent_kernel<NGPDE_ACT_RELU, false, false, true>, grid);
    else launch(node_fwd_persistent_kernel<-1, false, false, true>, grid);
    NGPDE_LAUNCH_CHECK("node_fwd_persistent_kernel (hub geometry)");
    if (!a.no_latch && (st = turn.latch())) return st;
    return turn.leave();
  }
#define NGPDE_PF_LAUNCH(AA, TT)                                                                                  \
  launch(k.m.slot_w ? node_fwd_persistent_kernel<AA, TT, true>                                                   \
         : a.pair ? node_fwd_persistent2_kernel<AA, TT, true>                                                    \
         : a.interleave ? node_fwd_persistent2_kernel<AA, TT, false> : node_fwd_persistent_kernel<AA, TT>, grid);
  k.ztape = a.ztape;
  if (a.tape && a.act == NGPDE_ACT_RELU) {
    NGPDE_REQUIRE(a.masks != nullptr, NGPDE_ERR_INVALID_ARGUMENT, "persistent forward with a relu tape needs the sign-bit masks");
    NGPDE_PF_LAUNCH(NGPDE_ACT_RELU, true)
  } else if (a.tape) {
    NGPDE_REQUIRE(a.ztape != nullptr && !a.interleave && !a.pair, NGPDE_ERR_INVALID_ARGUMENT,
                  "persistent forward with a tape: activations other than relu keep the pre-activations (one member at a time)");
    NGPDE_PF_LAUNCH(-1, true)
  } else if (a.act == NGPDE_ACT_RELU) {
    NGPDE_PF_LAUNCH(NGPDE_ACT_RELU, false)
  } else {
    NGPDE_PF_LAUNCH(-1, false)
  }
#undef NGPDE_PF_LAUNCH
  NGPDE_LAUNCH_CHECK("node_fwd_persistent_kernel");
  if (!a.no_latch && (st = turn.latch())) return st;
  return turn.leave();
}

int32_t launch_node_bwd_persistent(const NodePersistBwd &a, hipStream_t stream) {
  const ngpde_graph *g = a.g;
  const NodePersist &ps = *a.ps;
  int32_t st;
  PersistentTurn turn;
  if ((st = turn.enter(ps, stream))) return st;
  PBwdK k;
  k.m = make_meta(g->by_s, ps, 1);
  k.n_steps = a.n_steps; k.S = a.S; k.n_members = a.n_members; k.act = a.act; k.ztape = a.ztape;
  k.lam = a.lam; k.g1 = a.g1; k.g2 = a.g2; k.w1 = a.w1; k.w2 = a.w2;
  k.tape = a.tape; k.masks = a.masks; k.row_elems = a.row_elems; k.mask_bytes = a.mask_bytes;
  k.slab_dw1 = a.slab_dw1; k.slab_db1 = a.slab_db1; k.slab_dw2 = a.slab_dw2; k.slab_db2 = a.slab_db2;
  k.cb = ps.coef + 42;
  k.flag_stride = sync_slot_stride(ps.n_tiles);
  k.pair_wgs = a.pair ? ps.pair_wgs : 0;
  k.ubar = a.ubar;
  NGPDE_REQUIRE(!a.pair || (ps.pair_wgs > 0 && !a.interleave && a.n_members == 1 && a.act == NGPDE_ACT_RELU), NGPDE_ERR_STATE,
                "tile-pair launch without its setup");
  k.k_tiles = a.k_tiles;
  const auto launch = [&](auto kernel, dim3 grid) { launch_timed(kernel, grid, dim3(kThreads), 0, stream, a.ev_start, a.ev_stop, k); };
  if (a.k_tiles > 0) {
    NGPDE_REQUIRE(ps.pair_wgs > 0 && a.n_members == 1 && a.ubar, NGPDE_ERR_STATE, "tile-round launch without its setup");
    NGPDE_REQUIRE(a.k_tiles <= kMaxTileRounds, NGPDE_ERR_STATE, "tile rounds: at most %d tiles per workgroup", kMaxTileRounds);
    NGPDE_REQUIRE(a.act == NGPDE_ACT_RELU || a.ztape, NGPDE_ERR_INVALID_ARGUMENT, "persistent adjoint: activations other than relu need the saved pre-activations");
    k.pair_wgs = ps.pair_wgs;
    if ((st = launch_zero(a.ubar, 5 * a.row_elems * sizeof(float), stream))) return st;
    const dim3 gridk(ps.pair_wgs);
    NGPDE_REQUIRE(!k.m.slot_w || a.k_tiles <= kMaxTileRoundsW, NGPDE_ERR_STATE, "weighted tile rounds: at most %d tiles per workgroup", kMaxTileRoundsW);
    if (a.act == NGPDE_ACT_RELU) launch(k.m.slot_w ? node_bwd_persistentK_kernel<NGPDE_ACT_RELU> : node_bwd_persistentKP_kernel<NGPDE_ACT_RELU>, gridk);
    else launch(k.m.slot_w ? node_bwd_persistentK_kernel<-1> : node_bwd_persistentKP_kernel<-1>, gridk);
    NGPDE_LAUNCH_CHECK("node_bwd_persistentK_kernel");
    if (!a.no_latch && (st = turn.latch())) return st;
    return turn.leave();
  }
  NGPDE_REQUIRE(!k.m.slot_w || (!a.pair && !a.interleave && a.n_members == 1), NGPDE_ERR_STATE,
                "weighted graphs: one tile per workgroup or tile rounds, one member");
  const dim3 grid(a.pair ? ps.pair_wgs : ps.n_tiles);
  if (ps.hub) {
    NGPDE_REQUIRE(!a.pair && !a.interleave, NGPDE_ERR_STATE, "hub geometry: one tile per workgroup, the members of a batch one after the other");
    NGPDE_REQUIRE(a.act == NGPDE_ACT_RELU || a.ztape, NGPDE_ERR_INVALID_ARGUMENT, "persistent adjoint: activations other than relu need the saved pre-activations");
    launch(a.act == NGPDE_ACT_RELU ? node_bwd_persistent_kernel<NGPDE_ACT_RELU, false, true> : node_bwd_persistent_kernel<-1, false, true>, grid);
  } else if (k.m.slot_w) {
    NGPDE_REQUIRE(a.act == NGPDE_ACT_RELU || a.ztape, NGPDE_ERR_INVALID_ARGUMENT, "persistent adjoint: activations other than relu need the saved pre-activations");
    launch(a.act == NGPDE_ACT_RELU ? node_bwd_persistent_kernel<NGPDE_ACT_RELU, true> : node_bwd_persistent_kernel<-1, true>, grid);
  } else if (a.pair) {
    NGPDE_REQUIRE(a.ubar != nullptr, NGPDE_ERR_INVALID_ARGUMENT, "tile-pair persistent adjoint without its stage-adjoint scratch");
    launch(node_bwd_persistent2_kernel<true>, grid);
  } else if (a.interleave) {
    NGPDE_REQUIRE(a.ubar != nullptr, NGPDE_ERR_INVALID_ARGUMENT, "interleaved persistent adjoint without its stage-adjoint scratch");
    launch(node_bwd_persistent2_kernel<false>, grid);
  } else if (a.act != NGPDE_ACT_RELU) {
    NGPDE_REQUIRE(a.ztape != nullptr, NGPDE_ERR_INVALID_ARGUMENT, "persistent adjoint: activations other than relu need the saved pre-activations");
    launch(node_bwd_persistent_kernel<-1>, grid);
  } else {
    launch(node_bwd_persistent_kernel<NGPDE_ACT_RELU>, grid);
  }
  NGPDE_LAUNCH_CHECK("node_bwd_persistent_kernel");
  if (!a.no_latch && (st = turn.latch())) return st;
  return turn.leave();
}

}
```

### neuralgraphpde.jl_amd/csrc/persistent_gcn_tile.h

```cpp
#pragma once

#include "common.h"
#include "device_utils.h"
#include "gcn_tile.h"
#include "persistent_mem.h"
#include "persistent_sync.h"
#include "stamps.h"

namespace ngpde {

namespace {

constexpr int PD = 64;
using PG = Geo<PD>;
static_assert(PG::R == 1 && PG::GROUPS == kTM && PG::LPR == 16, "one 16-lane group per tile row");
constexpr int kXhF = (kHaloCap + 1) * PD;
constexpr int kTileF = kTM * PG::TS;
constexpr int kWF = PD * PG::TS;
constexpr int kMaxTileRounds = 8;

struct TileCtx {
  int tid, lane, wave_u, grp, q, tile, node, hcount, wmax, my_nbr;
  bool valid;
  float ci;
  const unsigned *lds_slots;
  const int *lds_hnode;
  const float *lds_w;
};
constexpr int kMetaF = kTM * 8 + 2 * kTM;

struct TileMeta {
  const int2 *halo;
  const uint8_t *slots;
  const int4 *sched;
  const int2 *tile_info;
  const int *nbr;
  const float *slot_w;
  unsigned *flags, *abort_word;
  int n_tiles;
  const uint8_t *of_pre;
  int *stats;
  const int *hub_halo;
  const uint8_t *hub_slots;
  const int2 *hub_rows;
  const int4 *hub_info;
  const int4 *hub_sched;
  const uint8_t *hub_long;
  const float *hub_w;
  NGPDE_STAMP_FIELD
};

__device__ __forceinline__ void tile_ctx_init(const TileMeta &m, TileCtx &c, float *lds_meta, int tile = -1) {
  c.tid = threadIdx.x;
  c.lane = c.tid & 63;
  c.wave_u = __builtin_amdgcn_readfirstlane(c.tid >> 6);
  c.grp = c.tid >> 4;
  c.q = c.tid & 15;
  c.tile = tile >= 0 ? tile : xcd_tile(blockIdx.x, m.n_tiles);
  const size_t pos = (size_t)c.tile * kTM + c.grp;
  const int4 sc = m.sched[pos];
  c.valid = sc.x >= 0;
  c.node = max(sc.x, 0);
  c.ci = c.valid ? __int_as_float(sc.w) : 0.f;
  unsigned *ls = reinterpret_cast<unsigned *>(lds_meta);
  int *lh = reinterpret_cast<int *>(lds_meta + kTM * 8);
  if (c.q < 8) ls[c.grp * 8 + c.q] = reinterpret_cast<const unsigned *>(m.slots)[pos * 8 + c.q];
  if (c.q >= 8 && c.q < 10) lh[c.grp + 32 * (c.q - 8)] = m.halo[(size_t)c.tile * kHaloCap + c.grp + 32 * (c.q - 7)].x;
  c.lds_slots = ls;
  c.lds_hnode = lh;
  c.hcount = __builtin_amdgcn_readfirstlane(m.tile_info[c.tile].x);
  int wm = c.valid ? sc.z : 0;
  wm = max(wm, __shfl_xor(wm, 16));
  wm = max(wm, __shfl_xor(wm, 32));
  c.wmax = __builtin_amdgcn_readfirstlane(wm);
  c.my_nbr = m.nbr[(size_t)c.tile * kNbrStride + c.lane];
}

constexpr int kMetaKF = kMetaF + kTM * 4 + kNbrStride + 4;
constexpr int kMaxTileRoundsW = 3;
constexpr int kSlotWF = kTM * kSlotWidth;
template <bool WGT> constexpr int meta_stride() { return kMetaKF + (WGT ? kSlotWF : 0); }
template <bool WGT> constexpr int meta_tiles() { return WGT ? kMaxTileRoundsW : kMaxTileRounds; }
template <bool WGT = false>
__device__ __forceinline__ void tile_tables_to_lds(const TileMeta &m, int tile, float *base) {
  const int tid = threadIdx.x, grp = tid >> 4, q = tid & 15;
  const size_t pos = (size_t)tile * kTM + grp;
  unsigned *ls = reinterpret_cast<unsigned *>(base);
  int *lh = reinterpret_cast<int *>(base + kTM * 8);
  int4 *lsc = reinterpret_cast<int4 *>(base + kMetaF);
  int *ln = reinterpret_cast<int *>(base + kMetaF + kTM * 4);
  if (q < 8) ls[grp * 8 + q] = reinterpret_cast<const unsigned *>(m.slots)[pos * 8 + q];
  if (q >= 8 && q < 10) lh[grp + 32 * (q - 8)] = m.halo[(size_t)tile * kHaloCap + grp + 32 * (q - 7)].x;
  if (q == 10) lsc[grp] = m.sched[pos];
  if (tid < kNbrStride) ln[tid] = m.nbr[(size_t)tile * kNbrStride + tid];
  if (tid == kNbrStride) ln[kNbrStride] = m.tile_info[tile].x;
  if constexpr (WGT) {
    float2 *lw = reinterpret_cast<float2 *>(base + kMetaKF);
    lw[tid] = reinterpret_cast<const float2 *>(m.slot_w + (size_t)tile * kSlotWF)[tid];
  }
}
template <bool WGT = false>
__device__ __forceinline__ void tile_ctx_from_lds(TileCtx &c, int tile, const float *base) {
  c.tid = threadIdx.x;
  c.lane = c.tid & 63;
  c.wave_u = __builtin_amdgcn_readfirstlane(c.tid >> 6);
  c.grp = c.tid >> 4;
  c.q = c.tid & 15;
  c.tile = tile;
  const int4 sc = reinterpret_cast<const int4 *>(base + kMetaF)[c.grp];
  const int *ln = reinterpret_cast<const int *>(base + kMetaF + kTM * 4);
  c.valid = sc.x >= 0;
  c.node = max(sc.x, 0);
  c.ci = c.valid ? __int_as_float(sc.w) : 0.f;
  c.lds_slots = reinterpret_cast<const unsigned *>(base);
  c.lds_hnode = reinterpret_cast<const int *>(base + kTM * 8);
  c.hcount = __builtin_amdgcn_readfirstlane(ln[kNbrStride]);
  int wm = c.valid ? sc.z : 0;
  wm = max(wm, __shfl_xor(wm, 16));
  wm = max(wm, __shfl_xor(wm, 32));
  c.wmax = __builtin_amdgcn_readfirstlane(wm);
  c.my_nbr = ln[c.lane];
  c.lds_w = WGT ? base + kMetaKF : nullptr;
}

__device__ __forceinline__ void tile_wait_arrive(const TileMeta &m, const TileCtx &c, int ph, int *s_ok, const unsigned *flags) {
  if (ph <= 1) return;
  if (c.wave_u == 0) {
    const unsigned *const a[1] = {watch_first(m.abort_word, flags, c.lane, c.my_nbr)};
    flag_poll<1>(a, m.abort_word, c.lane, (unsigned)(ph - 1), s_ok);
  }
  __syncthreads();
}
__device__ __forceinline__ bool tile_wait(const TileMeta &m, const TileCtx &c, int ph, int *s_ok, const unsigned *flags) {
  if (ph <= 1) return true;
  tile_wait_arrive(m, c, ph, s_ok, flags);
  return *s_ok != 0;
}
__device__ __forceinline__ bool tile_wait(const TileMeta &m, const TileCtx &c, int ph, int *s_ok) { return tile_wait(m, c, ph, s_ok, m.flags); }
__device__ __forceinline__ void tile_wait_primed_arrive(const TileMeta &m, const TileCtx &c, int ph, int *s_ok, const unsigned *flags, unsigned f) {
  if (c.wave_u == 0) {
    const unsigned need = (unsigned)(ph - 1);
    const unsigned *addr = watch_first(m.abort_word, flags, c.lane, c.my_nbr);
    const unsigned long long t0 = __builtin_amdgcn_s_memrealtime();
    bool ok = true;
    for (unsigned it = 1;; ++it) {
      if (__any((int)(c.lane == 63 && f != 0))) { ok = false; break; }
      if (__all((int)(c.lane == 63 || f >= need))) break;
      if ((it & 1023u) == 0 && __builtin_amdgcn_s_memrealtime() - t0 > kWaitTicks) {
        if (c.lane == 0) __hip_atomic_store(m.abort_word, 1u, __ATOMIC_RELAXED, __HIP_MEMORY_SCOPE_AGENT);
        ok = false;
        break;
      }
      __builtin_amdgcn_s_sleep(1);
      f = (c.lane == 63) ? 0u : need;
      if (addr) f = __hip_atomic_load(addr, __ATOMIC_RELAXED, __HIP_MEMORY_SCOPE_AGENT);
    }
    if (c.lane == 0) *s_ok = ok ? 1 : 0;
  }
  __syncthreads();
}
__device__ __forceinline__ bool tile_wait_primed(const TileMeta &m, const TileCtx &c, int ph, int *s_ok, const unsigned *flags, unsigned f) {
  tile_wait_primed_arrive(m, c, ph, s_ok, flags, f);
  return *s_ok != 0;
}

__device__ __forceinline__ void tile_publish(const TileCtx &c, int ph, unsigned *flags) { flag_publish(flags, c.tid, (unsigned)ph, c.tile); }
__device__ __forceinline__ void tile_publish(const TileMeta &m, const TileCtx &c, int ph) { tile_publish(c, ph, m.flags); }

__device__ __forceinline__ void tile_gather_foreign(const TileCtx &c, const float *X, float *ldsXh) {
  float4 *Xh4 = reinterpret_cast<float4 *>(ldsXh);
#pragma unroll
  for (int k = 0; k < 2; ++k) {
    if (4 * c.wave_u + 32 * (k + 1) < c.hcount) {
      const unsigned off = (unsigned)c.lds_hnode[c.grp + 32 * k] * (unsigned)(PD * 4) + (unsigned)(c.q * 16);
      __builtin_amdgcn_global_load_lds((const __attribute__((address_space(1))) void *)(reinterpret_cast<const char *>(X) + off),
                                       (__attribute__((address_space(3))) void *)(Xh4 + (c.grp + 32 * (k + 1)) * PG::LPR + c.q), 16, 0, 16);
    }
  }
  wait_vmcnt0();
  __syncthreads();
}

__device__ __forceinline__ void tile_gather_offsets(const TileCtx &c, unsigned (&off)[2]) {
#pragma unroll
  for (int k = 0; k < 2; ++k) off[k] = (unsigned)c.lds_hnode[c.grp + 32 * k] * (unsigned)(PD * 4) + (unsigned)(c.q * 16);
}
__device__ __forceinline__ bool tile_gather_foreign_checked(const TileCtx &c, const float *X, float *ldsXh, const unsigned (&off)[2], const int *s_ok) {
  float4 *Xh4 = reinterpret_cast<float4 *>(ldsXh);
#pragma unroll
  for (int k = 0; k < 2; ++k) {
    if (4 * c.wave_u + 32 * (k + 1) < c.hcount) {
      __builtin_amdgcn_global_load_lds((const __attribute__((address_space(1))) void *)(reinterpret_cast<const char *>(X) + off[k]),
                                       (__attribute__((address_space(3))) void *)(Xh4 + (c.grp + 32 * (k + 1)) * PG::LPR + c.q), 16, 0, 16);
    }
  }
  const int verdict = *s_ok;
  wait_vmcnt0();
  __syncthreads();
  return verdict != 0;
}

__device__ __forceinline__ void tile_slot_words(const TileCtx &c, unsigned (&w)[8]) {
  const uint4 a = reinterpret_cast<const uint4 *>(c.lds_slots)[c.grp * 2], b = reinterpret_cast<const uint4 *>(c.lds_slots)[c.grp * 2 + 1];
  w[0] = a.x; w[1] = a.y; w[2] = a.z; w[3] = a.w; w[4] = b.x; w[5] = b.y; w[6] = b.z; w[7] = b.w;
}

__device__ __forceinline__ void tile_round_rows(const float4 *Xh4, unsigned w, int q, float4 (&v)[4]) {
#pragma unroll
  for (int jb = 0; jb < 4; ++jb) v[jb] = Xh4[((w >> (8 * jb)) & 0xff) * PG::LPR + q];
}
__device__ __forceinline__ float4 tile_aggregate_rounds(const TileCtx &c, const unsigned (&w)[8], const float *ldsXh, float4 a, int n) {
  const float4 *Xh4 = reinterpret_cast<const float4 *>(ldsXh);
  if (n <= 0) return a;
  float4 v[4];
  tile_round_rows(Xh4, w[0], c.q, v);
#pragma unroll
  for (int jw = 0; jw < 8; ++jw) {
    if (jw == 7 || jw + 1 >= n) {
      a = f4_add(a, f4_add(f4_add(v[0], v[1]), f4_add(v[2], v[3])));
      break;
    }
    float4 nx[4];
    tile_round_rows(Xh4, w[jw + 1], c.q, nx);
    __builtin_amdgcn_sched_barrier(0);
    a = f4_add(a, f4_add(f4_add(v[0], v[1]), f4_add(v[2], v[3])));
#pragma unroll
    for (int jb = 0; jb < 4; ++jb) v[jb] = nx[jb];
  }
  return a;
}
__device__ __forceinline__ float4 tile_aggregate_rounds_rolling(const TileCtx &c, const unsigned (&w)[8], const float *ldsXh, float4 a, int n) {
  const float4 *Xh4 = reinterpret_cast<const float4 *>(ldsXh);
  if (n <= 0) return a;
  auto row = [&](unsigned wd, int jb) { return Xh4[((wd >> (8 * jb)) & 0xff) * PG::LPR + c.q]; };
  float4 v0 = row(w[0], 0), v1 = row(w[0], 1), v2 = row(w[0], 2), v3 = row(w[0], 3);
#pragma unroll
  for (int jw = 0; jw < 8; ++jw) {
    if (jw == 7 || jw + 1 >= n) {
      a = f4_add(a, f4_add(f4_add(v0, v1), f4_add(v2, v3)));
      break;
    }
    const float4 p = f4_add(v0, v1);
    __builtin_amdgcn_sched_barrier(0);
    v0 = row(w[jw + 1], 0); v1 = row(w[jw + 1], 1);
    __builtin_amdgcn_sched_barrier(0);
    const float4 s2 = f4_add(v2, v3);
    __builtin_amdgcn_sched_barrier(0);
    v2 = row(w[jw + 1], 2); v3 = row(w[jw + 1], 3);
    __builtin_amdgcn_sched_barrier(0);
    a = f4_add(a, f4_add(p, s2));
  }
  return a;
}

__device__ __forceinline__ float4 tile_aggregate(const TileCtx &c, const unsigned (&sw)[8], const float *ldsXh) {
  const float4 *Xh4 = reinterpret_cast<const float4 *>(ldsXh);
  float4 a = f4_zero();
#pragma unroll
  for (int jw = 0; jw < 8; ++jw) {
    if (jw * 4 < c.wmax) {
      const unsigned w = sw[jw];
      float4 v[4];
#pragma unroll
      for (int jb = 0; jb < 4; ++jb) v[jb] = Xh4[((w >> (8 * jb)) & 0xff) * PG::LPR + c.q];
      a = f4_add(a, f4_add(f4_add(v[0], v[1]), f4_add(v[2], v[3])));
    }
  }
  return f4_add(a, Xh4[c.grp * PG::LPR + c.q]);
}
__device__ __forceinline__ float4 tile_aggregate_lean(const TileCtx &c, const float *ldsXh) {
  const float4 *Xh4 = reinterpret_cast<const float4 *>(ldsXh);
  float4 a = f4_zero();
#pragma unroll 1
  for (int jw = 0; jw * 4 < c.wmax; ++jw) {
    const unsigned w = c.lds_slots[c.grp * 8 + jw];
    float4 v[4];
#pragma unroll
    for (int jb = 0; jb < 4; ++jb) v[jb] = Xh4[((w >> (8 * jb)) & 0xff) * PG::LPR + c.q];
    a = f4_add(a, f4_add(f4_add(v[0], v[1]), f4_add(v[2], v[3])));
  }
  return f4_add(a, Xh4[c.grp * PG::LPR + c.q]);
}

__device__ __forceinline__ float4 tile_aggregate_weighted(const TileCtx &c, const float *ldsXh) {
  const float4 *Xh4 = reinterpret_cast<const float4 *>(ldsXh);
  float4 a = f4_zero();
#pragma unroll 1
  for (int jw = 0; jw * 4 < c.wmax; ++jw) {
    const unsigned w = c.lds_slots[c.grp * 8 + jw];
    const float4 wv = *reinterpret_cast<const float4 *>(c.lds_w + c.grp * kSlotWidth + 4 * jw);
    float4 v[4];
#pragma unroll
    for (int jb = 0; jb < 4; ++jb) v[jb] = Xh4[((w >> (8 * jb)) & 0xff) * PG::LPR + c.q];
    a = f4_fma(wv.x, v[0], a); a = f4_fma(wv.y, v[1], a); a = f4_fma(wv.z, v[2], a); a = f4_fma(wv.w, v[3], a);
  }
  return f4_add(a, Xh4[c.grp * PG::LPR + c.q]);
}


__device__ __forceinline__ void tile_slot_words_from(const TileCtx &c, int r0, unsigned (&w)[8]) {
#pragma unroll
  for (int k = 0; k < 8; ++k) w[k] = c.lds_slots[c.grp * 8 + min(r0 + k, 7)];
}
constexpr int kHubHalo = 256;
constexpr int kHubList = 4096;
constexpr int kHubNbr = 256;
constexpr int kHubXhF = kHubHalo * PD;
constexpr int kHubMetaF = kHubList / 4 + (kHubHalo - kTM) + 2 * kTM + kTM / 4 + kHubList;

struct HubCtx : TileCtx {
  const uint8_t *hs;
  const int2 *hrows;
  const uint8_t *hlong;
  const float *hw;
  int start, len;
  int n_long;
  int nb1, nb2, nb3;
};

__device__ __forceinline__ void hub_ctx_init(const TileMeta &m, HubCtx &c, float *lds_meta) {
  c.tid = threadIdx.x;
  c.lane = c.tid & 63;
  c.wave_u = __builtin_amdgcn_readfirstlane(c.tid >> 6);
  c.grp = c.tid >> 4;
  c.q = c.tid & 15;
  c.tile = xcd_tile(blockIdx.x, m.n_tiles);
  const size_t pos = (size_t)c.tile * kTM + c.grp;
  const int4 sc = m.hub_sched[pos];
  c.valid = sc.x >= 0;
  c.node = max(sc.x, 0);
  c.ci = c.valid ? __int_as_float(sc.w) : 0.f;
  const int4 info = m.hub_info[c.tile];
  uint4 *ls = reinterpret_cast<uint4 *>(lds_meta);
  int *lh = reinterpret_cast<int *>(lds_meta + kHubList / 4);
  int2 *lr = reinterpret_cast<int2 *>(lds_meta + kHubList / 4 + (kHubHalo - kTM));
  unsigned *ll = reinterpret_cast<unsigned *>(lds_meta + kHubList / 4 + (kHubHalo - kTM) + 2 * kTM);
  if (c.tid * 16 < info.y) ls[c.tid] = reinterpret_cast<const uint4 *>(m.hub_slots + (size_t)c.tile * kHubList)[c.tid];
  if (c.tid < kHubHalo - kTM) lh[c.tid] = m.hub_halo[(size_t)c.tile * kHubHalo + kTM + c.tid];
  if (c.tid >= 256 && c.tid < 256 + kTM) lr[c.tid - 256] = m.hub_rows[(size_t)c.tile * kTM + (c.tid - 256)];
  if (c.tid >= 320 && c.tid < 320 + kTM / 4) ll[c.tid - 320] = reinterpret_cast<const unsigned *>(m.hub_long + (size_t)c.tile * kTM)[c.tid - 320];
  c.hs = reinterpret_cast<const uint8_t *>(ls);
  c.lds_hnode = lh;
  c.lds_slots = nullptr;
  c.lds_w = nullptr;
  c.hrows = lr;
  c.hlong = reinterpret_cast<const uint8_t *>(ll);
  c.hw = nullptr;
  if (m.hub_w) {
    float4 *lw = reinterpret_cast<float4 *>(lds_meta + kHubList / 4 + (kHubHalo - kTM) + 2 * kTM + kTM / 4);
    const float4 *gw = reinterpret_cast<const float4 *>(m.hub_w + (size_t)c.tile * kHubList);
#pragma unroll
    for (int k = 0; k < kHubList / 4 / kThreads; ++k)
      if ((c.tid + k * kThreads) * 4 < info.y) lw[c.tid + k * kThreads] = gw[c.tid + k * kThreads];
    c.hw = reinterpret_cast<const float *>(lw);
  }
  c.hcount = __builtin_amdgcn_readfirstlane(info.x);
  c.n_long = __builtin_amdgcn_readfirstlane(info.z);
  const int2 mine = m.hub_rows[pos];
  c.start = mine.x;
  c.len = (c.valid && mine.y <= kSlotWidth) ? mine.y : 0;
  int wm = c.len;
  wm = max(wm, __shfl_xor(wm, 16));
  wm = max(wm, __shfl_xor(wm, 32));
  c.wmax = __builtin_amdgcn_readfirstlane(wm);
  const int *nb = m.nbr + (size_t)c.tile * kHubNbr;
  c.my_nbr = nb[c.lane]; c.nb1 = nb[c.lane + 64]; c.nb2 = nb[c.lane + 128]; c.nb3 = nb[c.lane + 192];
}

__device__ __forceinline__ bool hub_wait(const TileMeta &m, const HubCtx &c, int ph, int *s_ok) {
  if (ph <= 1) return true;
  if (c.wave_u == 0) {
    const unsigned need = (unsigned)(ph - 1);
    const unsigned *a0 = (c.lane == 63) ? m.abort_word : (c.my_nbr >= 0 ? m.flags + kFlagLine * c.my_nbr : nullptr);
    const unsigned *a1 = c.nb1 >= 0 ? m.flags + kFlagLine * c.nb1 : nullptr, *a2 = c.nb2 >= 0 ? m.flags + kFlagLine * c.nb2 : nullptr,
                   *a3 = c.nb3 >= 0 ? m.flags + kFlagLine * c.nb3 : nullptr;
    const unsigned long long t0 = __builtin_amdgcn_s_memrealtime();
    bool ok = true;
// ... 136 lines not shown
  }
}
__device__ __forceinline__ void halo_fill_all(const TileCtx &c, const float *X, float *__restrict__ halo) {
  float4 *Xh4 = reinterpret_cast<float4 *>(halo);
#pragma unroll
  for (int k = 0; k < 3; ++k) {
    if (k == 0 || 4 * c.wave_u + 32 * k < c.hcount) {
      const unsigned row = k == 0 ? (unsigned)c.node : (unsigned)c.lds_hnode[c.grp + 32 * (k - 1)];
      const unsigned off = row * (unsigned)(PD * 4) + (unsigned)(c.q * 16);
      __builtin_amdgcn_global_load_lds((const __attribute__((address_space(1))) void *)(reinterpret_cast<const char *>(X) + off),
                                       (__attribute__((address_space(3))) void *)(Xh4 + (c.grp + 32 * k) * PG::LPR + c.q), 16, 0, 16);
    }
  }
}

struct PFwdK {
  TileMeta m;
  int n_steps, S, act;
  int n_members;
  const float *u_in;
  float *u_out;
  float *bufA, *bufB;
  const float *w1, *b1, *w2, *b2;
  float *tape;
  uint8_t *masks;
  float *ztape;
  size_t row_elems, mask_bytes;
  size_t flag_stride;
  int pair_wgs;
  int k_tiles;
  float *state;
  const float *cf;
};

struct PBwdK {
  TileMeta m;
  int n_steps, S, n_members, act;
  const float *ztape;
  float *lam;
  float *g1, *g2;
  const float *w1, *w2;
  const float *tape;
  const uint8_t *masks;
  size_t row_elems, mask_bytes;
  float *slab_dw1, *slab_db1, *slab_dw2, *slab_db2;
  int pair_wgs;
  int k_tiles;
  size_t flag_stride;
  float *ubar;
  const float *cb;
};


__device__ __forceinline__ float4 tile_row(const float *tile, const TileCtx &c) { return *reinterpret_cast<const float4 *>(&tile[c.grp * PG::TS + 4 * c.q]); }
__device__ __forceinline__ void tile_row_store(float *tile, const TileCtx &c, float4 v) { *reinterpret_cast<float4 *>(&tile[c.grp * PG::TS + 4 * c.q]) = v; }

__device__ __forceinline__ unsigned row_offset(int node, int q) { return (unsigned)node * (unsigned)(PD * 4) + (unsigned)(q * 16); }
__device__ __forceinline__ unsigned own_row_offset(const TileCtx c) { return row_offset(c.node, c.q); }

__device__ __forceinline__ void coef_to_lds(float *ldsC, const float *table, int n, int tid) {
  if (tid < n) ldsC[tid] = table[tid];
}
__device__ __forceinline__ void biases_to_lds(float *ldsB, const float *b1, const float *b2, int tid) {
  if (tid < PD) ldsB[tid] = b1 ? b1[tid] : 0.f;
  else if (tid < 2 * PD) ldsB[tid] = b2 ? b2[tid - PD] : 0.f;
}
__device__ __forceinline__ void zero_halo_row(float *ldsXh, bool first_group, int q) {
  if (first_group) reinterpret_cast<float4 *>(ldsXh)[kHaloCap * PG::LPR + q] = f4_zero();
}
template <bool WEIGHTED>
__device__ __forceinline__ void tile_round_tables(const TileMeta &m, int t0, int W, int K, float *ldsMeta) {
  for (int s = 0; s < K && t0 + s * W < m.n_tiles; ++s) tile_tables_to_lds<WEIGHTED>(m, t0 + s * W, ldsMeta + s * meta_stride<WEIGHTED>());
}
__device__ __forceinline__ int tile_round_count(const TileMeta &m, int t0, int W, int K) {
  int n = 0;
  for (int s = 0; s < K && t0 + s * W < m.n_tiles; ++s) n = s + 1;
  return n;
}

__device__ __forceinline__ void poison_tile_rounds(const TileMeta &m, float *out, int t0, int W, int n, int tid) {
  for (int s = 0; s < n; ++s) {
    const int4 sc = m.sched[(size_t)(t0 + s * W) * kTM + (tid >> 4)];
    if (sc.x >= 0) st4_g(out, row_offset(sc.x, tid & 15), f4_nan());
  }
}
__device__ __forceinline__ void poison_members(float *out, int n_members, size_t row_elems, bool valid, unsigned own) {
  for (int mb = 0; mb < n_members; ++mb)
    if (valid) st4_g(out + (size_t)mb * row_elems, own, f4_nan());
}

__device__ __forceinline__ float4 fwd_preact(const float *ldsZ, const TileCtx &c, float4 bias) { return f4_add(tile_row(ldsZ, c), bias); }
__device__ __forceinline__ uint8_t relu_sign_bits(float4 z) {
  return (uint8_t)((z.x > 0.f ? 1 : 0) | (z.y > 0.f ? 2 : 0) | (z.z > 0.f ? 4 : 0) | (z.w > 0.f ? 8 : 0));
}
__device__ __forceinline__ float4 fwd_output(const TileCtx &c, int act, float4 z) { return f4_sel(c.valid, f4_scale(c.ci, f4_act(act, z)), f4_zero()); }

struct RkCoef {
  float s, c0, c1, c2, c3, c4;
  __device__ __forceinline__ float self() const { return s; }
  __device__ __forceinline__ float k0() const { return c0; }
  __device__ __forceinline__ float k1() const { return c1; }
  __device__ __forceinline__ float k2() const { return c2; }
  __device__ __forceinline__ float k3() const { return c3; }
  __device__ __forceinline__ float k4() const { return c4; }
};
__device__ __forceinline__ RkCoef rk_coef(const float *ldsC, int i) {
  return RkCoef{ldsC[36 + i], ldsC[i * 6 + 0], ldsC[i * 6 + 1], ldsC[i * 6 + 2], ldsC[i * 6 + 3], ldsC[i * 6 + 4]};
}
struct RkCoefInPlace {
  const float *ldsC;
  int i;
  __device__ __forceinline__ float self() const { return ldsC[36 + i]; }
  __device__ __forceinline__ float k0() const { return ldsC[i * 6 + 0]; }
  __device__ __forceinline__ float k1() const { return ldsC[i * 6 + 1]; }
  __device__ __forceinline__ float k2() const { return ldsC[i * 6 + 2]; }
  __device__ __forceinline__ float k3() const { return ldsC[i * 6 + 3]; }
  __device__ __forceinline__ float k4() const { return ldsC[i * 6 + 4]; }
};
template <bool KI_IS_YV>
__device__ __forceinline__ float4 rk_stage_row(int i, int j, float4 yv, float4 kj) {
  if constexpr (KI_IS_YV) return f4_sel(i == j, yv, kj);
  else return kj;
}
template <bool KI_IS_YV, class Coef>
__device__ __forceinline__ float4 rk_combine(Coef cf, int i, float4 yv, float4 u, float4 k0, float4 k1, float4 k2, float4 k3, float4 k4) {
  float4 v = f4_scale(cf.self(), yv);
  v = f4_fma(1.0f, u, v);
  v = f4_fma(cf.k0(), rk_stage_row<KI_IS_YV>(i, 0, yv, k0), v); v = f4_fma(cf.k1(), rk_stage_row<KI_IS_YV>(i, 1, yv, k1), v);
  v = f4_fma(cf.k2(), rk_stage_row<KI_IS_YV>(i, 2, yv, k2), v); v = f4_fma(cf.k3(), rk_stage_row<KI_IS_YV>(i, 3, yv, k3), v);
  v = f4_fma(cf.k4(), rk_stage_row<KI_IS_YV>(i, 4, yv, k4), v);
  return v;
}

template <bool RELU, class Aux>
__device__ __forceinline__ float4 adjoint_dz(const TileCtx &c, int act, float4 kbar, Aux mk) {
  kbar = f4_scale(c.ci, kbar);
  if constexpr (RELU) {
    return c.valid ? make_float4((mk & 1u) ? kbar.x : 0.f, (mk & 2u) ? kbar.y : 0.f, (mk & 4u) ? kbar.z : 0.f, (mk & 8u) ? kbar.w : 0.f)
                   : f4_zero();
  } else {
    return f4_sel(c.valid, f4_mul(kbar, f4_dact(act, mk)), f4_zero());
  }
}
__device__ __forceinline__ float4 adjoint_kbar_last(const float *ldsC, int S, float4 lam) { return f4_scale(ldsC[S - 1], lam); }
__device__ __forceinline__ void adjoint_x_store(float *ldsX, const TileCtx &c, float4 xrow) { tile_row_store(ldsX, c, f4_sel(c.valid, xrow, f4_zero())); }
__device__ __forceinline__ float4 adjoint_g_row(const float *ldsG, const TileCtx &c) { return f4_sel(c.valid, f4_scale(c.ci, tile_row(ldsG, c)), f4_zero()); }

__device__ __forceinline__ void param_grad_products(const float *tX, const float *tDZ, int wave_u, int lane, int dbc, int dbpart,
                                                    f32x4 (&dwl)[PG::DWT], float &dbl) {
  constexpr int NT = PG::CT * PG::CT;
  const int i16 = lane & 15, kq = lane >> 4;
#pragma unroll
  for (int mm = 0; mm < PG::DWT; ++mm) {
    const int tt = wave_u + PG::WAVES * mm;
    if (tt < NT) {
      const int mt = tt / PG::CT, nt = tt % PG::CT;
#pragma unroll
      for (int kh = 0; kh < 2; ++kh) {
        float a[kTM / 8], b[kTM / 8];
#pragma unroll
        for (int ks = 0; ks < kTM / 8; ++ks) {
          a[ks] = tX[(4 * (ks + 4 * kh) + kq) * PG::TS + mt * 16 + i16];
          b[ks] = tDZ[(4 * (ks + 4 * kh) + kq) * PG::TS + nt * 16 + i16];
        }
#pragma unroll
        for (int ks = 0; ks < kTM / 8; ++ks) dwl[mm] = mfma16(a[ks], b[ks], dwl[mm]);
      }
    }
  }
  float sdb = 0.f;
#pragma unroll
  for (int nn = dbpart; nn < kTM; nn += PG::DBP) sdb += tDZ[nn * PG::TS + dbc];
#pragma unroll
  for (int o = 1; o < PG::DBP; o <<= 1) sdb += __shfl_xor(sdb, o);
  dbl += sdb;
}
__device__ __forceinline__ void param_grad_products_beside_dma(const float *__restrict__ tX, const float *__restrict__ tDZ, int wave_u, int lane, int dbc,
                                                               int dbpart, f32x4 (&dwl)[PG::DWT], float &dbl) {
  param_grad_products(tX, tDZ, wave_u, lane, dbc, dbpart, dwl, dbl);
}

__device__ __forceinline__ float4 adjoint_kbar_stage(const float *ldsC, int i, float4 t, float4 lam, float4 ub2, float4 ub3, float4 ub4, float4 ub5) {
  float4 v = f4_scale(ldsC[42 + i], t);
  v = f4_fma(ldsC[i - 1], lam, v);
  v = f4_fma(ldsC[6 + i * 6 + 2], ub2, v); v = f4_fma(ldsC[6 + i * 6 + 3], ub3, v);
  v = f4_fma(ldsC[6 + i * 6 + 4], ub4, v); v = f4_fma(ldsC[6 + i * 6 + 5], ub5, v);
  return v;
}
__device__ __forceinline__ float4 adjoint_lambda_update(float4 t, float4 lam, float4 ub1, float4 ub2, float4 ub3, float4 ub4, float4 ub5) {
  float4 v = f4_scale(1.0f, t);
  v = f4_fma(1.0f, lam, v);
  v = f4_fma(1.0f, ub1, v); v = f4_fma(1.0f, ub2, v); v = f4_fma(1.0f, ub3, v);
  v = f4_fma(1.0f, ub4, v); v = f4_fma(1.0f, ub5, v);
  return v;
}

__device__ __forceinline__ void write_slab(const f32x4 (&dwl)[PG::DWT], float dbl, float *slab_dw, float *slab_db, int wave_u, int lane,
                                           int dbc, int dbpart, bool ok) {
  float4 *slab4 = reinterpret_cast<float4 *>(slab_dw + (size_t)blockIdx.x * PD * PD);
// ... 12 lines not shown
```

### neuralgraphpde.jl_amd/plans.py

```python
from __future__ import annotations

import ctypes as C
import weakref

import torch

from . import _lib

class _Token:
    __slots__ = ("__weakref__",)


class _RowsIndexFn(torch.autograd.Function):

    @staticmethod
    def forward(ctx, x, index, n_rows, scatter):
        x = x.contiguous()
        outer = 1 if x.dim() == 1 else x.shape[0]
        n_idx = int(index.numel())
        out = torch.empty((n_rows if scatter else n_idx,) if x.dim() == 1 else (outer, n_rows if scatter else n_idx), dtype=torch.float32, device=x.device)
        _lib.check(_lib.load().ngpde_rows_index(outer, n_rows, n_idx, 1, _lib.ptr(index), _lib.ptr(x), _lib.ptr(out), int(scatter), _lib.current_stream()))
        ctx.meta = (index, n_rows, scatter)
        return out

# ... 58 lines not shown


class _Recent(dict):

    def put(self, key, value, limit):
        self[key] = value
        while len(self) > limit:
            del self[next(iter(self))]
        return value


class _PlanPool(_Recent):

    def acquire(self, key, with_backward, make, limits):
        pool = self.get(key)
        if pool is None:
            pool = self.put(key, [], limits.max_plans)
        else:
            self[key] = self.pop(key)
        for plan in pool:
            if not (with_backward and plan.busy()):
                return plan
        if len(pool) >= limits.max_outstanding:
            raise _lib.NgpdeError(_lib.ERR_STATE, f"NeuralODE: {len(pool)} solves await their backward pass on this graph; "
                                                  "each holds a tape -- run backward (or raise NeuralODE.max_outstanding)")
        try:
            pool.append(make())
        finally:
            if not pool:
                self.pop(key, None)
        return pool[-1]


class _Plan(_ResidentPlan):
    _entries = "ngpde_node"

    def __init__(self, handle, d, act, tableau, n_steps, dt, with_backward, members=1):
        super().__init__(handle, members)
        out = C.c_void_p()
        _lib.check(self.lib.ngpde_node_gcn2_create_batch(handle.ptr, self.members, d, act, _lib.TABLEAU[tableau], n_steps, dt,
                                                         int(with_backward), C.byref(out)))
        self.ptr = out

    def launch_count(self):
        f, b = C.c_int32(), C.c_int32()
        _lib.check(self.lib.ngpde_node_launch_count(self.ptr, C.byref(f), C.byref(b)))
        return f.value, b.value

    def flags(self):
        f = C.c_int32()
        _lib.check(self.lib.ngpde_node_flags(self.ptr, C.byref(f)))
        return {name for bit, name in _FLAG_NAMES if f.value & bit}

    def generation(self):
        gen, pend = C.c_uint64(), C.c_int32()
        _lib.check(self.lib.ngpde_node_generation(self.ptr, C.byref(gen), C.byref(pend)))
        return gen.value, bool(pend.value)

    def _backward_pending(self):
        return self.generation()[1]


class _NodeGCN2Fn(torch.autograd.Function):
    @staticmethod
    def forward(ctx, u, w1t, b1, w2t, b2, plan):
        lib = _lib.load()
        u, w1t, w2t = u.contiguous(), w1t.contiguous(), w2t.contiguous()
        uT = torch.empty_like(u)
        _lib.check(lib.ngpde_node_gcn2_forward(plan.ptr, _lib.ptr(u), _lib.ptr(w1t), _lib.ptr(b1), _lib.ptr(w2t),
                                               _lib.ptr(b2), _lib.ptr(uT), _lib.current_stream()))
        ctx.plan = plan
        ctx.token = plan.claim()
        ctx.generation = plan.generation()[0]
        ctx.shapes = (u.shape, w1t.shape, None if b1 is None else b1.shape, None if b2 is None else b2.shape)
        ctx.dev = u.device
        return uT

    @staticmethod
    def backward(ctx, duT):
        lib = _lib.load()
        us, ws, b1s, b2s = ctx.shapes
        mk = lambda s: None if s is None else torch.empty(s, dtype=torch.float32, device=ctx.dev)
        du0, dw1, dw2, db1, db2 = mk(us), mk(ws), mk(ws), mk(b1s), mk(b2s)
        duT = duT.contiguous()
        _lib.check(lib.ngpde_node_expect_generation(ctx.plan.ptr, ctx.generation))
        _lib.check(lib.ngpde_node_gcn2_backward(ctx.plan.ptr, _lib.ptr(duT), _lib.ptr(du0), _lib.ptr(dw1), _lib.ptr(db1),
                                                _lib.ptr(dw2), _lib.ptr(db2), _lib.current_stream()))
        return du0, dw1, db1, dw2, db2, None


_FLAG_NAMES = ((1, "prescaled"), (2, "sign_masks"), (8, "persistent_fwd"), (16, "persistent_bwd"), (32, "tile_pairs"),
               (64, "tile_rounds"), (128, "widened"), (256, "hub_geometry"), (512, "own_first"))


class _OdePlan(_ResidentPlan):
    _entries = "ngpde_ode"

    def __init__(self, handle, desc, kind):
        super().__init__(handle, desc.members)
        self.gen, self._pending = 0, False
        self.kind = kind
        self.n_first, self.n_steps = int(desc.n_phi), int(desc.n_steps)
        out, fl = C.c_void_p(), C.c_int32()
        _lib.check(self.lib.ngpde_ode_create(handle.ptr, C.byref(desc), C.byref(out), C.byref(fl)))
        self.ptr, self._flags = out, fl.value

    def flags(self):
        return {name for bit, name in _FLAG_NAMES if self._flags & bit} | {self.kind}

    def _backward_pending(self):
        return self._pending


def _ode_desc(rhs, tableau, n_steps, dt, with_backward, members=1, **kw):
    d = _lib.OdeDesc()
    d.rhs, d.tableau, d.n_steps, d.dt, d.with_backward, d.members = rhs, _lib.TABLEAU[tableau], int(n_steps), float(dt), int(with_backward), int(members)
    for k, v in kw.items():
        if k in ("phi_dims", "phi_acts", "gamma_dims", "gamma_acts"):
            for j, t in enumerate(v):
                getattr(d, k)[j] = int(t)
        else:
            setattr(d, k, v)
    return d


class _NodeOdeFn(torch.autograd.Function):

    @staticmethod
    def forward(ctx, u, plan, save, att, *wb):
        lib = _lib.load()
        u = u.contiguous()
        ws = [w.contiguous() for w in wb[0::2]]
        bs = [None if b is None else b.contiguous() for b in wb[1::2]]
        att = None if att is None else att.contiguous()
        nf = plan.n_first if plan.n_first else len(ws)
        prm = _lib.OdeParams()
        for l, (w, b) in enumerate(zip(ws, bs)):
            blk, j = (prm.first, l) if l < nf else (prm.second, l - nf)
            blk.weight[j], blk.bias[j] = w.data_ptr(), (b.data_ptr() if b is not None else None)
        prm.attention = att.data_ptr() if att is not None else None
        k, start = save if save is not None else (0, 0)
        out = torch.empty_like(u) if save is None else torch.empty((plan.n_steps // k + int(start), u.numel()), dtype=torch.float32, device=u.device)
        _lib.check(lib.ngpde_ode_forward(plan.ptr, _lib.ptr(u), C.byref(prm), int(k), int(start), _lib.ptr(out), _lib.current_stream()))
        plan.gen, plan._pending = plan.gen + 1, True
        ctx.plan, ctx.gen, ctx.token, ctx.save, ctx.nf = plan, plan.gen, plan.claim(), (int(k), int(start)), nf
# ... 34 lines not shown
```

Before: 10300 ODE-steps/s.

## Permute rows within persistent GCN tiles to balance per-wave aggregation load

Adds a host-side row placement pass that permutes the 32 rows of each tile across waves, using a cost model over forward own/foreign slot counts and backward source counts, then local swap search. The persistent forward and backward kernels gain a PLACED template path that indexes LDS halo, tile rows and mask bytes through the permutation. The aim is to cut the per-wave maximum (and SIMD-partner pair) aggregation rounds, which sets the tile's critical path. It adds extra indirection in LDS indexing, host preprocessing at plan creation, and more device tables.

```diff
diff --git a/include/ngpde.h b/include/ngpde.h
--- a/include/ngpde.h
+++ b/include/ngpde.h
@@ -350,7 +350,8 @@
        NGPDE_NODE_TILE_ROUNDS = 64 ,
        NGPDE_NODE_WIDENED = 128 ,
        NGPDE_NODE_HUB_GEOMETRY = 256 ,
-       NGPDE_NODE_OWN_FIRST = 512  };
+       NGPDE_NODE_OWN_FIRST = 512 ,
+       NGPDE_NODE_ROW_PLACEMENT = 1024  };
 int32_t ngpde_node_flags(const ngpde_node_t *plan, int32_t *flags);
 int32_t ngpde_batch_pad_host(int32_t n_members, const int64_t *sizes, int64_t *padded_offsets, int64_t *index, const int32_t *order,
                              int32_t *order_padded);
@@ -359,6 +360,7 @@
 int32_t ngpde_node_fault(ngpde_node_t *plan, ngpde_stream_t stream, int32_t *fault);
 int32_t ngpde_node_pipeline_stats(ngpde_node_t *plan, ngpde_stream_t stream, int64_t *ahead_forward, int64_t *ahead_backward,
                                   int64_t *slot_phases);
+int32_t ngpde_node_row_placement(ngpde_node_t *plan, int32_t which, void *out, size_t capacity, size_t *bytes);
 int32_t ngpde_node_gat_supported(const ngpde_graph_t *g, int32_t din, int32_t heads, int32_t c);
 int32_t ngpde_node_gat_create(const ngpde_graph_t *g, int32_t heads, int32_t c, float negative_slope, int32_t act, int32_t tableau,
                               int32_t n_steps, double dt, int32_t with_backward, ngpde_node_gat_t **out);
diff --git a/neuralgraphpde.jl_amd/_lib.py b/neuralgraphpde.jl_amd/_lib.py
--- a/neuralgraphpde.jl_amd/_lib.py
+++ b/neuralgraphpde.jl_amd/_lib.py
@@ -260,6 +260,7 @@
     "ngpde_transpose": (_i32, [_i32, _i32, _vp, _vp, _vp]),
     "ngpde_rows_scale": (_i32, [_i64, _i32, _vp, _vp, _vp, _vp]),
     "ngpde_node_pipeline_stats": (_i32, [_vp, _vp, C.POINTER(_i64), C.POINTER(_i64), C.POINTER(_i64)]),
+    "ngpde_node_row_placement": (_i32, [_vp, _i32, _vp, C.c_size_t, C.POINTER(C.c_size_t)]),
     "ngpde_node_generation": (_i32, [_vp, C.POINTER(C.c_uint64), C.POINTER(_i32)]),
     "ngpde_node_expect_generation": (_i32, [_vp, C.c_uint64]),
     "ngpde_node_profile": (_i32, [_vp, _i32, C.POINTER(_f32), C.POINTER(_i32), _vp]),
diff --git a/neuralgraphpde.jl_amd/csrc/common.h b/neuralgraphpde.jl_amd/csrc/common.h
--- a/neuralgraphpde.jl_amd/csrc/common.h
+++ b/neuralgraphpde.jl_amd/csrc/common.h
@@ -161,6 +161,14 @@
 };
 int32_t own_first_tables_build(const ngpde_graph *g, OwnFirst *of, hipStream_t stream);
 void own_first_tables_free(OwnFirst *of);
+struct RowPlacement {
+  uint8_t *perm = nullptr;
+  uint8_t *slots = nullptr;
+  int4 *sched = nullptr;
+  uint8_t *pre = nullptr;
+};
+int32_t row_placement_build(const ngpde_graph *g, RowPlacement *rp);
+void row_placement_free(RowPlacement *rp);
 
 struct NodePersist {
   int n_tiles = 0;
@@ -201,6 +209,7 @@
   hipEvent_t ev_start = nullptr, ev_stop = nullptr;
   bool no_latch = false;
   const OwnFirst *of = nullptr;
+  const RowPlacement *place = nullptr;
 };
 struct NodePersistBwd {
   const ngpde_graph *g = nullptr;
@@ -217,6 +226,7 @@
   float *ubar = nullptr;
   hipEvent_t ev_start = nullptr, ev_stop = nullptr;
   bool no_latch = false;
+  const RowPlacement *place = nullptr;
 };
 const unsigned *node_persistent_abort_word(const NodePersist *ps);
 bool node_persistent_interleave_env();
diff --git a/neuralgraphpde.jl_amd/csrc/node.hip b/neuralgraphpde.jl_amd/csrc/node.hip
--- a/neuralgraphpde.jl_amd/csrc/node.hip
+++ b/neuralgraphpde.jl_amd/csrc/node.hip
@@ -201,6 +201,8 @@
   NodePersist persist;
   OwnFirst of;
   bool has_of = false;
+  RowPlacement place;
+  bool has_place = false;
   float *pbuf = nullptr;
   bool interleave = false;
   bool pair = false;
@@ -404,6 +406,7 @@
   }
   a.interleave = p->interleave; a.pair = p->pair; a.k_tiles = p->ktiles; a.state = p->kstate;
   a.of = p->has_of ? &p->of : nullptr;
+  a.place = p->has_place ? &p->place : nullptr;
   a.ev_start = ev0; a.ev_stop = ev1;
   return launch_node_fwd_persistent(a, stream);
 }
@@ -417,6 +420,7 @@
   a.tape = p->tape; a.masks = p->masks; a.row_elems = p->row_elems; a.mask_bytes = p->mask_bytes; a.ztape = p->ztape;
   a.slab_dw1 = p->slab_dw1; a.slab_db1 = p->slab_db1; a.slab_dw2 = p->slab_dw2; a.slab_db2 = p->slab_db2;
   a.interleave = p->interleave; a.pair = p->pair; a.ubar = p->pubar; a.k_tiles = p->ktiles;
+  a.place = p->has_place ? &p->place : nullptr;
   a.ev_start = ev0; a.ev_stop = ev1;
   int32_t st;
   if ((st = launch_node_bwd_persistent(a, stream))) return st;
@@ -492,6 +496,7 @@
   if (p->kstate) (void)hipFree(p->kstate);
   node_persistent_free(&p->persist);
   own_first_tables_free(&p->of);
+  row_placement_free(&p->place);
   delete p;
   return NGPDE_OK;
 }
@@ -583,6 +588,13 @@
       p->has_of = st == NGPDE_OK;
     }
   }
+  if (st == NGPDE_OK && p->has_of && p->persistent && !p->pair && !p->ktiles) {
+    const char *nrp = std::getenv("NGPDE_NO_ROW_PLACEMENT");
+    if (!(nrp && nrp[0] == '1')) {
+      st = row_placement_build(g, &p->place);
+      p->has_place = st == NGPDE_OK && p->place.perm != nullptr;
+    }
+  }
   p->ztape_mode = p->with_bwd && !p->mask_mode && p->persistent;
   p->slots = p->mask_mode ? 2 : (p->ztape_mode ? 4 : (p->with_bwd ? (p->needs_z ? 6 : 4) : 4));
   p->mask_bytes = p->mask_mode ? fused_mask_bytes(p->n, d) : 0;
@@ -689,7 +701,8 @@
   *flags = (p->pre ? NGPDE_NODE_PRESCALED : 0) | (p->mask_mode ? NGPDE_NODE_SIGN_MASKS : 0) |
            (p->persistent ? NGPDE_NODE_PERSISTENT_FWD : 0) | (p->persistent && p->with_bwd ? NGPDE_NODE_PERSISTENT_BWD : 0) |
            (p->pair ? NGPDE_NODE_TILE_PAIRS : 0) | (p->ktiles ? NGPDE_NODE_TILE_ROUNDS : 0) | (p->du != p->d ? NGPDE_NODE_WIDENED : 0) |
-           (p->hub ? NGPDE_NODE_HUB_GEOMETRY : 0) | (p->has_of ? NGPDE_NODE_OWN_FIRST : 0);
+           (p->hub ? NGPDE_NODE_HUB_GEOMETRY : 0) | (p->has_of ? NGPDE_NODE_OWN_FIRST : 0) |
+           (p->has_place ? NGPDE_NODE_ROW_PLACEMENT : 0);
   return NGPDE_OK;
 }
 
@@ -720,6 +733,22 @@
   if (ahead_forward) *ahead_forward = f;
   if (ahead_backward) *ahead_backward = b;
   if (slot_phases) *slot_phases = (int64_t)nt * p->members * p->n_steps * p->tb.S * 2;
+  return NGPDE_OK;
+}
+
+int32_t ngpde_node_row_placement(ngpde_node_t *p, int32_t which, void *out, size_t capacity, size_t *bytes) {
+  NGPDE_RANGE();
+  NGPDE_REQUIRE(p != nullptr && bytes != nullptr, NGPDE_ERR_INVALID_ARGUMENT, "ngpde_node_row_placement: NULL argument");
+  *bytes = 0;
+  NGPDE_REQUIRE(which >= 0 && which <= 7, NGPDE_ERR_INVALID_ARGUMENT, "ngpde_node_row_placement: table %d (0 .. 7)", which);
+  if (!p->has_of || (which <= 3 && !p->has_place)) return NGPDE_OK;
+  const size_t ns = (size_t)p->g->n_sched, nt = ns / kTileRows;
+  const void *src[8] = {p->place.perm, p->place.slots, p->place.sched, p->place.pre, p->of.slots, p->of.sched, p->of.pre, p->g->by_s.sched};
+  const size_t len[8] = {ns, ns * kSlotWidth, ns * sizeof(int4), nt * 8, ns * kSlotWidth, ns * sizeof(int4), nt * 8, ns * sizeof(int4)};
+  *bytes = len[which];
+  if (!out) return NGPDE_OK;
+  NGPDE_REQUIRE(capacity >= len[which], NGPDE_ERR_INVALID_ARGUMENT, "ngpde_node_row_placement: table %d takes %zu bytes", which, len[which]);
+  NGPDE_HIP_CHECK(hipMemcpy(out, src[which], len[which], hipMemcpyDeviceToHost));
   return NGPDE_OK;
 }
 
diff --git a/neuralgraphpde.jl_amd/csrc/node_persistent.hip b/neuralgraphpde.jl_amd/csrc/node_persistent.hip
--- a/neuralgraphpde.jl_amd/csrc/node_persistent.hip
+++ b/neuralgraphpde.jl_amd/csrc/node_persistent.hip
@@ -7,6 +7,7 @@
 
 #include "common.h"
 #include "persistent_gcn_tile.h"
+#include "row_placement.h"
 #include "stamps.h"
 
 namespace ngpde {
@@ -17,6 +18,7 @@
 template <int ACT, bool TAPE, bool WGT = false, bool HUB = false>
 __global__ __launch_bounds__(kThreads, HUB ? 2 : 4) void node_fwd_persistent_kernel(const PFwdK p) {
   static_assert(!(HUB && WGT), "hub geometry: its own weight lists (HubCtx::hw), not the WGT form");
+  constexpr bool PLACED = !HUB && !WGT;
   constexpr int XH = HUB ? kHubXhF : kXhF, MF = HUB ? kHubMetaF : kMetaF;
   __shared__ __attribute__((aligned(16))) float lds[XH + 2 * kTileF + (WGT ? kWF + kSlotWF : 2 * kWF) + 2 * PD + MF + 48 + 4];
   static_assert(!HUB || sizeof(lds) <= 160 * 1024 - 64, "one workgroup per CU");
@@ -26,7 +28,7 @@
   int *s_ok = reinterpret_cast<int *>(ldsC + 48);
   typename std::conditional<HUB, HubCtx, TileCtx>::type c;
   if constexpr (HUB) hub_ctx_init(p.m, c, ldsMeta);
-  else tile_ctx_init(p.m, c, ldsMeta);
+  else tile_ctx_init<PLACED>(p.m, c, ldsMeta);
   coef_to_lds(ldsC, p.cf, 42, c.tid);
   const int act = ACT >= 0 ? ACT : p.act;
   float4 *Xh4 = reinterpret_cast<float4 *>(ldsXh);
@@ -60,7 +62,7 @@
   const size_t ev0 = (size_t)mb * p.n_steps * p.S * 2;
   float4 u = f4_sel(c.valid && ok, ld4_g(u_in, own), f4_zero());
   float4 k0 = f4_zero(), k1 = f4_zero(), k2 = f4_zero(), k3 = f4_zero(), k4 = f4_zero(), k5 = f4_zero();
-  Xh4[c.grp * PG::LPR + c.q] = u;
+  Xh4[own_halo_index<PLACED>(c)] = u;
   if constexpr (!HUB && !WGT) __syncthreads();
   for (int n = 0; n < p.n_steps && ok; ++n) {
     for (int i = 0; i < p.S && ok; ++i) {
@@ -80,11 +82,11 @@
           agg = hub_aggregate(c, sw, ldsXh, ldsZ);
         } else if constexpr (!WGT) {
           unsigned sw[8], swf[8];
-          tile_slot_words(c, sw);
-          tile_slot_words_from(c, of_pre, swf);
+          tile_slot_words<PLACED>(c, sw);
+          tile_slot_words_from<PLACED>(c, of_pre, swf);
           unsigned goff[2];
           tile_gather_offsets(c, goff);
-          const float4 self = Xh4[c.grp * PG::LPR + c.q];
+          const float4 self = Xh4[own_halo_index<PLACED>(c)];
           float4 a = tile_aggregate_rounds(c, sw, ldsXh, f4_zero(), of_pre);
           tile_wait_arrive(p.m, c, ph, s_ok, p.m.flags);
           NGPDE_PHASE_STAMP(p.m.stamps, ph, 1);
@@ -102,7 +104,7 @@
           agg = tile_aggregate_weighted(c, ldsXh);
         }
         float4 acc = f4_scale(c.ci, agg);
-        tile_row_store(ldsT, c, acc);
+        tile_row_store<PLACED>(ldsT, c, acc);
         const size_t ev = ev0 + (size_t)(n * p.S + i) * 2 + layer;
         __syncthreads();
         NGPDE_PHASE_STAMP(p.m.stamps, ph, 3);
@@ -110,26 +112,26 @@
         else mfma_rows_times_bt<PD>(ldsT, layer == 0 ? ldsW1 : ldsW2, ldsZ, c.wave_u, c.lane);
         __syncthreads();
         NGPDE_PHASE_STAMP(p.m.stamps, ph, 4);
-        const float4 z = fwd_preact(ldsZ, c, layer == 0 ? bias1 : bias2);
+        const float4 z = fwd_preact<PLACED>(ldsZ, c, layer == 0 ? bias1 : bias2);
         const uint8_t sign_bits = relu_sign_bits(z);
         float4 yv = fwd_output(c, act, z);
         if (layer == 0) {
           if (c.valid) store_sc1(p.bufB, own, yv);
-          Xh4[c.grp * PG::LPR + c.q] = yv;
+          Xh4[own_halo_index<PLACED>(c)] = yv;
         } else {
           k0 = f4_sel(i == 0, yv, k0); k1 = f4_sel(i == 1, yv, k1); k2 = f4_sel(i == 2, yv, k2);
           k3 = f4_sel(i == 3, yv, k3); k4 = f4_sel(i == 4, yv, k4); k5 = f4_sel(i == 5, yv, k5);
           const float4 v = rk_combine<false>(RkCoefInPlace{ldsC, i}, i, yv, u, k0, k1, k2, k3, k4);
           if (i == p.S - 1) u = v;
           if (c.valid) store_sc1(p.bufA, own, v);
-          Xh4[c.grp * PG::LPR + c.q] = v;
+          Xh4[own_halo_index<PLACED>(c)] = v;
         }
         NGPDE_PHASE_STAMP(p.m.stamps, ph, 5);
         tile_publish(p.m, c, ph);
         NGPDE_PHASE_STAMP(p.m.stamps, ph, 6);
-        if constexpr (TAPE && ACT == NGPDE_ACT_RELU) stu8_g(p.masks + ev * p.mask_bytes + (size_t)c.tile * kThreads, (unsigned)c.tid, sign_bits);
+        if constexpr (TAPE && ACT == NGPDE_ACT_RELU) stu8_g(p.masks + ev * p.mask_bytes + (size_t)c.tile * kThreads, mask_offset<PLACED>(c), sign_bits);
         else if (TAPE && c.valid) st4_stream_g(p.ztape + ev * p.row_elems, own, z);
-        if (TAPE && c.valid) st4_stream_g(p.tape + ev * p.row_elems, own, tile_row(ldsT, c));
+        if (TAPE && c.valid) st4_stream_g(p.tape + ev * p.row_elems, own, tile_row<PLACED>(ldsT, c));
       }
     }
   }
@@ -521,6 +523,7 @@
 __global__ __launch_bounds__(kThreads, HUB ? 2 : 4) void node_bwd_persistent_kernel(const PBwdK p) {
   static_assert(!(HUB && WGT), "hub geometry: its own weight lists (HubCtx::hw), not the WGT form");
   constexpr bool RELU = (ACT == NGPDE_ACT_RELU);
+  constexpr bool PLACED = !HUB && !WGT;
   using Aux = typename std::conditional<RELU, unsigned, float4>::type;
   constexpr int XH = HUB ? kHubXhF : kXhF, MF = HUB ? kHubMetaF : kMetaF;
   __shared__ __attribute__((aligned(16))) float lds[XH + 2 * kTileF + (WGT ? PD * PD + kWF + kSlotWF : 2 * kWF) + MF + 48 + 4];
@@ -531,7 +534,7 @@
   int *s_ok = reinterpret_cast<int *>(ldsC + 48);
   typename std::conditional<HUB, HubCtx, TileCtx>::type c;
   if constexpr (HUB) hub_ctx_init(p.m, c, ldsMeta);
-  else tile_ctx_init(p.m, c, ldsMeta);
+  else tile_ctx_init<PLACED>(p.m, c, ldsMeta);
   coef_to_lds(ldsC, p.cb, 48, c.tid);
   float4 *Xh4 = reinterpret_cast<float4 *>(ldsXh);
   if constexpr (WGT) {
@@ -562,7 +565,7 @@
 
   auto tape_row = [&](size_t ev) { return ld4_stream_g(p.tape + ev * p.row_elems, own); };
   auto mask_of = [&](size_t ev) -> Aux {
-    if constexpr (RELU) return ldu8_g(p.masks + ev * p.mask_bytes + (size_t)c.tile * kThreads, (unsigned)c.tid);
+    if constexpr (RELU) return ldu8_g(p.masks + ev * p.mask_bytes + (size_t)c.tile * kThreads, mask_offset<PLACED>(c));
     else return ld4_stream_g(p.ztape + ev * p.row_elems, own);
   };
   Aux mk_n{};
@@ -570,20 +573,20 @@
   unsigned f_next = 0;
   auto dense = [&](int ph, const float *ldsW, f32x4 (&dwl)[PG::DWT], float &dbl, float4 kbar, Aux mk, float4 xrow, float *gout, bool pf, size_t ev_n) {
     const float4 dz = adjoint_dz<RELU>(c, p.act, kbar, mk);
-    tile_row_store(ldsDZ, c, dz);
+    tile_row_store<PLACED>(ldsDZ, c, dz);
     __syncthreads();
     NGPDE_PHASE_STAMP(p.m.stamps, ph, 3);
     if (WGT && ldsW == ldsW1) mfma_rows_times_bswz64(ldsDZ, ldsW, ldsG, c.wave_u, c.lane);
     else mfma_rows_times_bt<PD>(ldsDZ, ldsW, ldsG, c.wave_u, c.lane);
     __syncthreads();
     NGPDE_PHASE_STAMP(p.m.stamps, ph, 4);
-    const float4 gv = adjoint_g_row(ldsG, c);
+    const float4 gv = adjoint_g_row<PLACED>(ldsG, c);
     if (c.valid) store_sc1(gout, own, gv);
-    adjoint_x_store(ldsX, c, xrow);
+    adjoint_x_store<PLACED>(ldsX, c, xrow);
     NGPDE_PHASE_STAMP(p.m.stamps, ph, 5);
     tile_publish(p.m, c, ph);
     NGPDE_PHASE_STAMP(p.m.stamps, ph, 6);
-    Xh4[c.grp * PG::LPR + c.q] = gv;
+    Xh4[own_halo_index<PLACED>(c)] = gv;
     if constexpr (!HUB) {
       if (c.wave_u == 0) f_next = poll_issue(p.m, c, p.m.flags);
     }
@@ -634,7 +637,7 @@
           t = tile_aggregate_weighted(c, ldsXh);
         } else {
           unsigned sw[8], goff[2];
-          tile_slot_words(c, sw);
+          tile_slot_words<PLACED>(c, sw);
           if constexpr (RELU) tile_gather_offsets(c, goff);
           if constexpr (RELU) {
             tile_wait_primed_arrive(p.m, c, ph, s_ok, p.m.flags, f_next);
@@ -647,9 +650,9 @@
           }
           NGPDE_PHASE_STAMP(p.m.stamps, ph, 2);
           float4 self;
-          if constexpr (RELU) self = Xh4[c.grp * PG::LPR + c.q];
+          if constexpr (RELU) self = Xh4[own_halo_index<PLACED>(c)];
           t = tile_aggregate_rounds_rolling(c, sw, ldsXh, f4_zero(), (c.wmax + 3) >> 2);
-          if constexpr (!RELU) self = Xh4[c.grp * PG::LPR + c.q];
+          if constexpr (!RELU) self = Xh4[own_halo_index<PLACED>(c)];
           t = f4_add(t, self);
         }
         dense(ph, ldsW1, dw1, db1, t, mk, xrow, p.g1, !last_next, ev_next);
@@ -678,7 +681,7 @@
           t = tile_aggregate_weighted(c, ldsXh);
         } else {
           unsigned sw[8], goff[2];
-          tile_slot_words(c, sw);
+          tile_slot_words<PLACED>(c, sw);
           if constexpr (RELU) tile_gather_offsets(c, goff);
           if constexpr (RELU) {
             tile_wait_primed_arrive(p.m, c, ph, s_ok, p.m.flags, f_next);
@@ -691,9 +694,9 @@
           }
           NGPDE_PHASE_STAMP(p.m.stamps, ph, 2);
           float4 self;
-          if constexpr (RELU) self = Xh4[c.grp * PG::LPR + c.q];
+          if constexpr (RELU) self = Xh4[own_halo_index<PLACED>(c)];
           t = tile_aggregate_rounds_rolling(c, sw, ldsXh, f4_zero(), (c.wmax + 3) >> 2);
-          if constexpr (!RELU) self = Xh4[c.grp * PG::LPR + c.q];
+          if constexpr (!RELU) self = Xh4[own_halo_index<PLACED>(c)];
           t = f4_add(t, self);
         }
         float4 kbar;
@@ -1669,6 +1672,82 @@
   *of = OwnFirst();
 }
 
+int32_t row_placement_build(const ngpde_graph *g, RowPlacement *rp) {
+  const Csr &ct = g->by_t, &cs = g->by_s;
+  if (!(ct.halo_ok && ct.slots && ct.sched && cs.halo_ok && cs.sched) || ct.slot_w) return NGPDE_OK;
+  const size_t ns = (size_t)g->n_sched;
+  const int nt = g->n_sched / kTileRows;
+  std::vector<uint8_t> slots(ns * kSlotWidth), o_slots(ns * kSlotWidth, (uint8_t)kHaloCap), perm((size_t)nt * kTileRows), pre((size_t)nt * 8, 0);
+  std::vector<int4> sched(ns), sched_s(ns);
+  NGPDE_HIP_CHECK(hipMemcpy(slots.data(), ct.slots, slots.size(), hipMemcpyDeviceToHost));
+  NGPDE_HIP_CHECK(hipMemcpy(sched.data(), ct.sched, ns * sizeof(int4), hipMemcpyDeviceToHost));
+  NGPDE_HIP_CHECK(hipMemcpy(sched_s.data(), cs.sched, ns * sizeof(int4), hipMemcpyDeviceToHost));
+  std::vector<PlaceRow> rows(ns);
+  for (size_t pos = 0; pos < ns; ++pos) {
+    PlaceRow &r = rows[pos];
+    r.valid = sched[pos].x >= 0;
+    const int deg = r.valid ? std::min(sched[pos].z, kSlotWidth) : 0;
+    for (int j = 0; j < deg; ++j) (slots[pos * kSlotWidth + j] < kTileRows ? r.own : r.foreign) += 1;
+    r.src = sched_s[pos].x >= 0 ? std::min(sched_s[pos].z, kSlotWidth) : 0;
+  }
+  for (size_t g4 = 0; g4 < ns; g4 += 4) {
+    int p4 = 0;
+    for (int k = 0; k < 4; ++k) p4 = std::max(p4, (rows[g4 + k].own + 3) >> 2);
+    bool fits = true;
+    for (int k = 0; k < 4; ++k) fits = fits && 4 * p4 + rows[g4 + k].foreign <= kSlotWidth;
+    for (int k = 0; k < 4; ++k) {
+      PlaceRow &r = rows[g4 + k];
+      r.keep = !fits;
+      r.lead = kSlotWidth / 4;
+      for (int j = r.own + r.foreign - 1; j >= 0; --j)
+        if (slots[(g4 + k) * kSlotWidth + j] >= kTileRows) r.lead = j >> 2;
+    }
+  }
+  for (int t = 0; t < nt; ++t) {
+    const PlaceRow *tr = &rows[(size_t)t * kTileRows];
+    uint8_t *pm = &perm[(size_t)t * kTileRows];
+    place_tile(tr, pm);
+    for (int w = 0; w < 8; ++w) {
+      const PlaceWave pw = place_wave(tr, pm + 4 * w);
+      pre[(size_t)t * 8 + w] = (uint8_t)pw.pre;
+      for (int k = 0; k < 4; ++k) {
+        const size_t pos = (size_t)t * kTileRows + pm[4 * w + k];
+        const PlaceRow &r = tr[pm[4 * w + k]];
+        const uint8_t *b = &slots[pos * kSlotWidth];
+        uint8_t *ob = &o_slots[pos * kSlotWidth];
+        if (r.keep) {
+          std::copy(b, b + kSlotWidth, ob);
+          continue;
+        }
+        const int deg = r.own + r.foreign;
+        int n = 0;
+        for (int j = 0; j < deg; ++j)
+          if (b[j] < kTileRows) ob[n++] = b[j];
+        n = 4 * std::max(pw.pre, (r.own + 3) >> 2);
+        for (int j = 0; j < deg; ++j)
+          if (b[j] >= kTileRows) ob[n++] = b[j];
+        if (r.valid) sched[pos].z = n;
+      }
+    }
+  }
+  const auto up = [](auto **dst, const auto &v) -> int32_t {
+    NGPDE_HIP_CHECK(hipMalloc((void **)dst, v.size() * sizeof(v[0])));
+    NGPDE_HIP_CHECK(hipMemcpy(*dst, v.data(), v.size() * sizeof(v[0]), hipMemcpyHostToDevice));
+    return NGPDE_OK;
+  };
+  int32_t st;
+  if ((st = up(&rp->perm, perm)) || (st = up(&rp->slots, o_slots)) || (st = up(&rp->sched, sched)) || (st = up(&rp->pre, pre))) return st;
+  return NGPDE_OK;
+}
+
+void row_placement_free(RowPlacement *rp) {
+  if (rp->perm) (void)hipFree(rp->perm);
+  if (rp->slots) (void)hipFree(rp->slots);
+  if (rp->sched) (void)hipFree(rp->sched);
+  if (rp->pre) (void)hipFree(rp->pre);
+  *rp = RowPlacement();
+}
+
 int32_t node_persistent_setup(const ngpde_graph *g, const float *coef_host, NodePersist *ps, bool pair, bool hub) {
   std::vector<int> lists;
   const int nt = g->n_sched / kTileRows;
@@ -1813,6 +1892,7 @@
   }
   const NodePersist::HubLists &L = ps.hub_lists[dir];
   m.hub_halo = L.halo; m.hub_slots = L.slots; m.hub_rows = L.rows; m.hub_info = L.info; m.hub_long = L.longs; m.hub_sched = L.sched;
+  if (!ps.hub) m.perm = nullptr;
   m.hub_w = L.w;
   if (ps.hub) m.slot_w = nullptr;
   m.flags = ps.sync; m.abort_word = sync_abort_word(ps.sync, ps.n_tiles); m.n_tiles = ps.n_tiles;
@@ -1936,6 +2016,10 @@
          : a.pair ? node_fwd_persistent2_kernel<AA, TT, true>                                                    \
          : a.interleave ? node_fwd_persistent2_kernel<AA, TT, false> : node_fwd_persistent_kernel<AA, TT>, grid);
   k.ztape = a.ztape;
+  if (a.place && a.place->perm && a.of && a.of->slots && !k.m.slot_w && !a.pair && !a.interleave) {
+    k.m.perm = a.place->perm;
+    k.m.slots = a.place->slots; k.m.sched = a.place->sched; k.m.of_pre = a.place->pre;
+  }
   if (a.tape && a.act == NGPDE_ACT_RELU) {
     NGPDE_REQUIRE(a.masks != nullptr, NGPDE_ERR_INVALID_ARGUMENT, "persistent forward with a relu tape needs the sign-bit masks");
     NGPDE_PF_LAUNCH(NGPDE_ACT_RELU, true)
@@ -2006,8 +2090,10 @@
     launch(node_bwd_persistent2_kernel<false>, grid);
   } else if (a.act != NGPDE_ACT_RELU) {
     NGPDE_REQUIRE(a.ztape != nullptr, NGPDE_ERR_INVALID_ARGUMENT, "persistent adjoint: activations other than relu need the saved pre-activations");
+    if (a.place) k.m.perm = a.place->perm;
     launch(node_bwd_persistent_kernel<-1>, grid);
   } else {
+    if (a.place) k.m.perm = a.place->perm;
     launch(node_bwd_persistent_kernel<NGPDE_ACT_RELU>, grid);
   }
   NGPDE_LAUNCH_CHECK("node_bwd_persistent_kernel");
diff --git a/neuralgraphpde.jl_amd/csrc/persistent_gcn_tile.h b/neuralgraphpde.jl_amd/csrc/persistent_gcn_tile.h
--- a/neuralgraphpde.jl_amd/csrc/persistent_gcn_tile.h
+++ b/neuralgraphpde.jl_amd/csrc/persistent_gcn_tile.h
@@ -21,12 +21,15 @@
 
 struct TileCtx {
   int tid, lane, wave_u, grp, q, tile, node, hcount, wmax, my_nbr;
+  int row;
   bool valid;
   float ci;
   const unsigned *lds_slots;
   const int *lds_hnode;
   const float *lds_w;
 };
+template <bool PLACED>
+__device__ __forceinline__ int ctx_row(const TileCtx &c) { return PLACED ? c.row : c.grp; }
 constexpr int kMetaF = kTM * 8 + 2 * kTM;
 
 struct TileMeta {
@@ -45,11 +48,15 @@
   const int2 *hub_rows;
   const int4 *hub_info;
   const int4 *hub_sched;
-  const uint8_t *hub_long;
+  union {
+    const uint8_t *hub_long;
+    const uint8_t *perm;
+  };
   const float *hub_w;
   NGPDE_STAMP_FIELD
 };
 
+template <bool PLACED = false>
 __device__ __forceinline__ void tile_ctx_init(const TileMeta &m, TileCtx &c, float *lds_meta, int tile = -1) {
   c.tid = threadIdx.x;
   c.lane = c.tid & 63;
@@ -58,7 +65,11 @@
   c.q = c.tid & 15;
   c.tile = tile >= 0 ? tile : xcd_tile(blockIdx.x, m.n_tiles);
   const size_t pos = (size_t)c.tile * kTM + c.grp;
-  const int4 sc = m.sched[pos];
+  c.row = c.grp;
+  if constexpr (PLACED) {
+    if (m.perm) c.row = (int)m.perm[pos];
+  }
+  const int4 sc = m.sched[PLACED ? (size_t)c.tile * kTM + c.row : pos];
   c.valid = sc.x >= 0;
   c.node = max(sc.x, 0);
   c.ci = c.valid ? __int_as_float(sc.w) : 0.f;
@@ -105,6 +116,7 @@
   c.lane = c.tid & 63;
   c.wave_u = __builtin_amdgcn_readfirstlane(c.tid >> 6);
   c.grp = c.tid >> 4;
+  c.row = c.grp;
   c.q = c.tid & 15;
   c.tile = tile;
   const int4 sc = reinterpret_cast<const int4 *>(base + kMetaF)[c.grp];
@@ -200,8 +212,10 @@
   return verdict != 0;
 }
 
+template <bool PLACED = false>
 __device__ __forceinline__ void tile_slot_words(const TileCtx &c, unsigned (&w)[8]) {
-  const uint4 a = reinterpret_cast<const uint4 *>(c.lds_slots)[c.grp * 2], b = reinterpret_cast<const uint4 *>(c.lds_slots)[c.grp * 2 + 1];
+  const int r = ctx_row<PLACED>(c);
+  const uint4 a = reinterpret_cast<const uint4 *>(c.lds_slots)[r * 2], b = reinterpret_cast<const uint4 *>(c.lds_slots)[r * 2 + 1];
   w[0] = a.x; w[1] = a.y; w[2] = a.z; w[3] = a.w; w[4] = b.x; w[5] = b.y; w[6] = b.z; w[7] = b.w;
 }
 
@@ -298,9 +312,10 @@
 }
 
 
+template <bool PLACED = false>
 __device__ __forceinline__ void tile_slot_words_from(const TileCtx &c, int r0, unsigned (&w)[8]) {
 #pragma unroll
-  for (int k = 0; k < 8; ++k) w[k] = c.lds_slots[c.grp * 8 + min(r0 + k, 7)];
+  for (int k = 0; k < 8; ++k) w[k] = c.lds_slots[ctx_row<PLACED>(c) * 8 + min(r0 + k, 7)];
 }
 constexpr int kHubHalo = 256;
 constexpr int kHubList = 4096;
@@ -323,6 +338,7 @@
   c.lane = c.tid & 63;
   c.wave_u = __builtin_amdgcn_readfirstlane(c.tid >> 6);
   c.grp = c.tid >> 4;
+  c.row = c.grp;
   c.q = c.tid & 15;
   c.tile = xcd_tile(blockIdx.x, m.n_tiles);
   const size_t pos = (size_t)c.tile * kTM + c.grp;
@@ -565,8 +581,14 @@
 };
 
 
-__device__ __forceinline__ float4 tile_row(const float *tile, const TileCtx &c) { return *reinterpret_cast<const float4 *>(&tile[c.grp * PG::TS + 4 * c.q]); }
-__device__ __forceinline__ void tile_row_store(float *tile, const TileCtx &c, float4 v) { *reinterpret_cast<float4 *>(&tile[c.grp * PG::TS + 4 * c.q]) = v; }
+template <bool PLACED = false>
+__device__ __forceinline__ float4 tile_row(const float *tile, const TileCtx &c) { return *reinterpret_cast<const float4 *>(&tile[ctx_row<PLACED>(c) * PG::TS + 4 * c.q]); }
+template <bool PLACED = false>
+__device__ __forceinline__ void tile_row_store(float *tile, const TileCtx &c, float4 v) { *reinterpret_cast<float4 *>(&tile[ctx_row<PLACED>(c) * PG::TS + 4 * c.q]) = v; }
+template <bool PLACED = false>
+__device__ __forceinline__ int own_halo_index(const TileCtx &c) { return ctx_row<PLACED>(c) * PG::LPR + c.q; }
+template <bool PLACED>
+__device__ __forceinline__ unsigned mask_offset(const TileCtx &c) { return PLACED ? (unsigned)own_halo_index<true>(c) : (unsigned)c.tid; }
 
 __device__ __forceinline__ unsigned row_offset(int node, int q) { return (unsigned)node * (unsigned)(PD * 4) + (unsigned)(q * 16); }
 __device__ __forceinline__ unsigned own_row_offset(const TileCtx c) { return row_offset(c.node, c.q); }
@@ -602,7 +624,8 @@
     if (valid) st4_g(out + (size_t)mb * row_elems, own, f4_nan());
 }
 
-__device__ __forceinline__ float4 fwd_preact(const float *ldsZ, const TileCtx &c, float4 bias) { return f4_add(tile_row(ldsZ, c), bias); }
+template <bool PLACED = false>
+__device__ __forceinline__ float4 fwd_preact(const float *ldsZ, const TileCtx &c, float4 bias) { return f4_add(tile_row<PLACED>(ldsZ, c), bias); }
 __device__ __forceinline__ uint8_t relu_sign_bits(float4 z) {
   return (uint8_t)((z.x > 0.f ? 1 : 0) | (z.y > 0.f ? 2 : 0) | (z.z > 0.f ? 4 : 0) | (z.w > 0.f ? 8 : 0));
 }
@@ -656,8 +679,10 @@
   }
 }
 __device__ __forceinline__ float4 adjoint_kbar_last(const float *ldsC, int S, float4 lam) { return f4_scale(ldsC[S - 1], lam); }
-__device__ __forceinline__ void adjoint_x_store(float *ldsX, const TileCtx &c, float4 xrow) { tile_row_store(ldsX, c, f4_sel(c.valid, xrow, f4_zero())); }
-__device__ __forceinline__ float4 adjoint_g_row(const float *ldsG, const TileCtx &c) { return f4_sel(c.valid, f4_scale(c.ci, tile_row(ldsG, c)), f4_zero()); }
+template <bool PLACED = false>
+__device__ __forceinline__ void adjoint_x_store(float *ldsX, const TileCtx &c, float4 xrow) { tile_row_store<PLACED>(ldsX, c, f4_sel(c.valid, xrow, f4_zero())); }
+template <bool PLACED = false>
+__device__ __forceinline__ float4 adjoint_g_row(const float *ldsG, const TileCtx &c) { return f4_sel(c.valid, f4_scale(c.ci, tile_row<PLACED>(ldsG, c)), f4_zero()); }
 
 __device__ __forceinline__ void param_grad_products(const float *tX, const float *tDZ, int wave_u, int lane, int dbc, int dbpart,
                                                     f32x4 (&dwl)[PG::DWT], float &dbl) {
diff --git a/neuralgraphpde.jl_amd/csrc/row_placement.h b/neuralgraphpde.jl_amd/csrc/row_placement.h
--- /dev/null
+++ b/neuralgraphpde.jl_amd/csrc/row_placement.h
@@ -0,0 +1,143 @@
+#pragma once
+
+#include <algorithm>
+#include <cstdint>
+
+namespace ngpde {
+
+constexpr int kPlaceRows = 32, kPlaceWaves = 8, kPlaceSlots = 32;
+constexpr int place_simd_partner(int w) { return w ^ 4; }
+
+struct PlaceRow {
+  int own = 0, foreign = 0;
+  int src = 0;
+  bool keep = false;
+  int lead = 0;
+  bool valid = false;
+};
+
+struct PlaceWave {
+  int pre = 0;
+  int fwd = 0;
+  int bwd = 0;
+};
+
+inline int place_fwd_len(const PlaceRow &r, int pre) {
+  if (!r.valid) return 0;
+  if (r.keep) return r.own + r.foreign;
+  return 4 * std::max(pre, (r.own + 3) >> 2) + r.foreign;
+}
+
+inline PlaceWave place_wave(const PlaceRow *rows, const uint8_t *p) {
+  PlaceWave w;
+  bool own_first = true;
+  int pre = 0;
+  for (int k = 0; k < 4; ++k) {
+    const PlaceRow &r = rows[p[k]];
+    if (!r.valid) continue;
+    pre = std::max(pre, (r.own + 3) >> 2);
+    w.bwd = std::max(w.bwd, (r.src + 3) >> 2);
+  }
+  for (int k = 0; k < 4; ++k) {
+    const PlaceRow &r = rows[p[k]];
+    if (r.valid && (r.keep ? r.lead < pre : 4 * pre + r.foreign > kPlaceSlots)) own_first = false;
+  }
+  w.pre = own_first ? pre : 0;
+  for (int k = 0; k < 4; ++k) w.fwd = std::max(w.fwd, (place_fwd_len(rows[p[k]], w.pre) + 3) >> 2);
+  return w;
+}
+
+struct PlaceCost {
+  int fwd_pair = 0, bwd_pair = 0;
+  int pre0 = 0;
+  int total = 0;
+  int weighed() const { return 12 * (fwd_pair + bwd_pair) + 4 * pre0 + total; }
+};
+
+inline PlaceCost place_cost(const PlaceWave *w) {
+  PlaceCost c;
+  for (int k = 0; k < kPlaceWaves; ++k) {
+    const int o = place_simd_partner(k);
+    c.fwd_pair = std::max(c.fwd_pair, (w[k].fwd - w[k].pre) + (w[o].fwd - w[o].pre));
+    c.bwd_pair = std::max(c.bwd_pair, w[k].bwd + w[o].bwd);
+    c.total += w[k].fwd + w[k].bwd;
+  }
+  c.pre0 = w[0].pre;
+  return c;
+}
+inline PlaceCost place_cost(const PlaceRow *rows, const uint8_t *perm) {
+  PlaceWave w[kPlaceWaves];
+  for (int k = 0; k < kPlaceWaves; ++k) w[k] = place_wave(rows, perm + 4 * k);
+  return place_cost(w);
+}
+
+inline void place_tile(const PlaceRow *rows, uint8_t *perm) {
+  uint8_t id[kPlaceRows], p[kPlaceRows];
+  int nv = 0;
+  bool tail_only = true;
+  for (int r = 0; r < kPlaceRows; ++r) {
+    id[r] = (uint8_t)r;
+    if (rows[r].valid) {
+      if (r != nv) tail_only = false;
+      ++nv;
+    }
+  }
+  std::copy(id, id + kPlaceRows, perm);
+  if (!tail_only || nv < 8) return;
+  static const int kOrders[3][3] = {{0, 1, 2}, {2, 0, 1}, {1, 0, 2}};
+  uint8_t bestp[kPlaceRows];
+  PlaceCost best;
+  for (int start = 0; start < 3; ++start) {
+    uint8_t s[kPlaceRows];
+    std::copy(id, id + kPlaceRows, s);
+    auto key = [&](int r, int k) {
+      const PlaceRow &x = rows[r];
+      return k == 0 ? (x.foreign + 3) >> 2 : k == 1 ? (x.own + 3) >> 2 : (x.src + 3) >> 2;
+    };
+    std::sort(s, s + nv, [&](uint8_t a, uint8_t b) {
+      for (int k = 0; k < 3; ++k)
+        if (key(a, kOrders[start][k]) != key(b, kOrders[start][k])) return key(a, kOrders[start][k]) < key(b, kOrders[start][k]);
+      return a < b;
+    });
+    if (nv == kPlaceRows) {
+      for (int c = 0; c < kPlaceWaves; ++c) {
+        const int w = c < 4 ? c : place_simd_partner(7 - c);
+        for (int k = 0; k < 4; ++k) p[4 * w + k] = s[4 * c + k];
+      }
+    } else {
+      std::copy(s, s + kPlaceRows, p);
+    }
+    PlaceWave w[kPlaceWaves];
+    for (int k = 0; k < kPlaceWaves; ++k) w[k] = place_wave(rows, p + 4 * k);
+    PlaceCost cur = place_cost(w);
+    for (int sweep = 0; sweep < 8; ++sweep) {
+      bool moved = false;
+      for (int a = 0; a < nv; ++a)
+        for (int b = (a | 3) + 1; b < nv; ++b) {
+          const PlaceWave wa = w[a >> 2], wb = w[b >> 2];
+          std::swap(p[a], p[b]);
+          w[a >> 2] = place_wave(rows, p + (a & ~3));
+          w[b >> 2] = place_wave(rows, p + (b & ~3));
+          const PlaceCost c = place_cost(w);
+          if (c.weighed() < cur.weighed()) {
+            cur = c;
+            moved = true;
+          } else {
+            std::swap(p[a], p[b]);
+            w[a >> 2] = wa;
+            w[b >> 2] = wb;
+          }
+        }
+      if (!moved) break;
+    }
+    if (start == 0 || cur.weighed() < best.weighed()) {
+      best = cur;
+      std::copy(p, p + kPlaceRows, bestp);
+    }
+  }
+  std::copy(bestp, bestp + kPlaceRows, p);
+  const PlaceCost base = place_cost(rows, id);
+  if (best.weighed() < base.weighed() && best.total <= base.total) std::copy(p, p + kPlaceRows, perm);
+}
+
+}
diff --git a/neuralgraphpde.jl_amd/plans.py b/neuralgraphpde.jl_amd/plans.py
--- a/neuralgraphpde.jl_amd/plans.py
+++ b/neuralgraphpde.jl_amd/plans.py
@@ -134,6 +134,22 @@
         _lib.check(self.lib.ngpde_node_flags(self.ptr, C.byref(f)))
         return {name for bit, name in _FLAG_NAMES if f.value & bit}
 
+    def row_placement_tables(self):
+        import numpy as np
+        shapes = (("perm", np.uint8, 32), ("slots", np.uint8, 32), ("sched", np.int32, 4), ("pre", np.uint8, 8),
+                  ("slots", np.uint8, 32), ("sched", np.int32, 4), ("pre", np.uint8, 8), ("sched", np.int32, 4))
+        got = []
+        for which, (_, dt, width) in enumerate(shapes):
+            n = C.c_size_t()
+            _lib.check(self.lib.ngpde_node_row_placement(self.ptr, which, None, 0, C.byref(n)))
+            if n.value == 0:
+                return None
+            a = np.empty(n.value // np.dtype(dt).itemsize, dtype=dt)
+            _lib.check(self.lib.ngpde_node_row_placement(self.ptr, which, a.ctypes.data_as(C.c_void_p), a.nbytes, C.byref(n)))
+            got.append(a.reshape(-1, width))
+        return dict(perm=got[0], placed=dict(slots=got[1], sched=got[2], pre=got[3]),
+                    own_first=dict(slots=got[4], sched=got[5], pre=got[6]), by_source=dict(sched=got[7]))
+
     def generation(self):
         gen, pend = C.c_uint64(), C.c_int32()
         _lib.check(self.lib.ngpde_node_generation(self.ptr, C.byref(gen), C.byref(pend)))
@@ -172,7 +188,8 @@
 
 
 _FLAG_NAMES = ((1, "prescaled"), (2, "sign_masks"), (8, "persistent_fwd"), (16, "persistent_bwd"), (32, "tile_pairs"),
-               (64, "tile_rounds"), (128, "widened"), (256, "hub_geometry"), (512, "own_first"))
+               (64, "tile_rounds"), (128, "widened"), (256, "hub_geometry"), (512, "own_first"),
+               (1024, "row_placement"))
 
 
 class _OdePlan(_ResidentPlan):
```

After: 10220 ODE-steps/s. No clear change (-0.8%).
